# insight-platform/Similari

Hardware: NVIDIA H100
Metric: pair_associations_per_sec (higher is better)
Workload: dtype f32

## Files before the change

similari_b200/csrc/engine.cu:

```cuda
#include <cuda_runtime.h>

#include <algorithm>
#include <chrono>
#include <cmath>
#include <cstdlib>
#include <cstdarg>
#include <cstdio>
#include <cstring>
#include <map>
#include <string>
#include <unordered_map>
#include <vector>

#include "../../include/similari_b200.h"
#include "sb_engine.cuh"

#include <atomic>

namespace sb {
static std::atomic<unsigned long long> g_launches{0};
void note_launch(int n) { g_launches.fetch_add((unsigned long long)n, std::memory_order_relaxed); }
unsigned long long launch_count() { return g_launches.load(std::memory_order_relaxed); }
}

// ... 22 lines not shown
  void* p = nullptr;
  size_t bytes = 0;
  int ensure(size_t need) {
    if (need <= bytes) return 0;
    size_t nb = std::max(need, bytes + bytes / 2);
    void* np = nullptr;
    cudaError_t e = cudaMalloc(&np, nb);
    if (e != cudaSuccess) return fail(SB200_ERR_CUDA, "cudaMalloc(%zu) failed: %s", nb, cudaGetErrorString(e));
    if (p) cudaFree(p);
    p = np;
    bytes = nb;
    return 0;
  }
  void release() {
    if (p) cudaFree(p);
    p = nullptr;
    bytes = 0;
  }
  template <typename T> T* as() const { return reinterpret_cast<T*>(p); }
};

struct HBuf {
  void* p = nullptr;
  void* dp = nullptr;
  size_t bytes = 0;
  int ensure(size_t need) {
    if (need <= bytes) return 0;
    size_t nb = std::max(need, bytes + bytes / 2);
    void* np = nullptr;
    cudaError_t e = cudaHostAlloc(&np, nb, cudaHostAllocMapped);
    if (e != cudaSuccess) return fail(SB200_ERR_CUDA, "cudaHostAlloc(%zu) failed: %s", nb, cudaGetErrorString(e));
    void* ndp = nullptr;
    e = cudaHostGetDevicePointer(&ndp, np, 0);
    if (e != cudaSuccess) { cudaFreeHost(np); return fail(SB200_ERR_CUDA, "cudaHostGetDevicePointer failed: %s", cudaGetErrorString(e)); }
    if (p) cudaFreeHost(p);
    p = np;
    dp = ndp;
    bytes = nb;
    return 0;
  }
  void release() {
    if (p) cudaFreeHost(p);
    p = nullptr;
    dp = nullptr;
    bytes = 0;
  }
  template <typename T> T* as() const { return reinterpret_cast<T*>(p); }
};

int make_params(const sb200_options& o, sb::Params* out) {
  sb::Params p;
  memset(&p, 0, sizeof(p));
  if (o.kind < 0 || o.kind > 3) return fail(SB200_ERR_INVALID, "unknown tracker kind %d", o.kind);
  if (o.positional_kind != SB200_POS_MAHA && o.positional_kind != SB200_POS_IOU)
    return fail(SB200_ERR_INVALID, "unknown positional metric %d", o.positional_kind);
  p.kind = o.kind;
  p.positional_kind = o.positional_kind;
  p.visual_kind = o.visual_kind;
  p.iou_threshold = o.iou_threshold;
  p.min_confidence = o.min_confidence;
  p.pos_weight = o.kalman_position_weight;
  p.vel_weight = o.kalman_velocity_weight;
  p.max_idle_epochs = o.max_idle_epochs;
  if (o.max_idle_epochs < 0) return fail(SB200_ERR_INVALID, "max_idle_epochs must be >= 0");
  if (o.n_constraints < 0 || o.n_constraints > SB200_MAX_CONSTRAINTS)
    return fail(SB200_ERR_INVALID, "at most %d spatio-temporal constraints", SB200_MAX_CONSTRAINTS);
  std::vector<std::pair<int, float>> c;
  for (int i = 0; i < o.n_constraints; ++i) {
    if (!(o.constraint_max_dist[i] > 0.0f))
      return fail(SB200_ERR_INVALID, "The distance is expected to be a positive float");
    c.emplace_back(o.constraint_epochs[i], o.constraint_max_dist[i]);
  }
  std::stable_sort(c.begin(), c.end(), [](const std::pair<int, float>& a, const std::pair<int, float>& b) { return a.first < b.first; });
  c.erase(std::unique(c.begin(), c.end(), [](const std::pair<int, float>& a, const std::pair<int, float>& b) { return a.first == b.first; }), c.end());
  p.n_constraints = (int)c.size();
  for (size_t i = 0; i < c.size(); ++i) { p.constraint_epochs[i] = c[i].first; p.constraint_max_dist[i] = c[i].second; }
  p.is_visual = o.kind == SB200_KIND_VISUAL_SORT || o.kind == SB200_KIND_BATCH_VISUAL_SORT;
  p.is_batch = o.kind == SB200_KIND_BATCH_SORT || o.kind == SB200_KIND_BATCH_VISUAL_SORT;
  if (p.is_visual) {
    if (o.visual_kind != SB200_VIS_EUCLIDEAN && o.visual_kind != SB200_VIS_COSINE)
      return fail(SB200_ERR_INVALID, "unknown visual metric %d", o.visual_kind);
    if (o.feature_dim <= 0) return fail(SB200_ERR_INVALID, "feature_dim must be > 0 for visual trackers");
    if (o.visual_max_observations < 1 || o.visual_max_observations > sb::kMaxObs)
      return fail(SB200_ERR_CAPACITY, "visual_max_observations must be in [1, %d]", sb::kMaxObs);
    p.visual_threshold = o.visual_threshold;
    p.feature_dim = o.feature_dim;
    p.d8 = (o.feature_dim + 7) / 8 * 8;
    p.max_obs = o.visual_max_observations;
    p.min_votes = o.visual_min_votes;
    p.min_track_length = o.visual_minimal_track_length;
    p.min_area = o.visual_minimal_area;
    p.min_quality_use = o.visual_minimal_quality_use;
    p.min_quality_collect = o.visual_minimal_quality_collect;
    p.min_own_use = o.visual_minimal_own_area_percentage_use;
    p.min_own_collect = o.visual_minimal_own_area_percentage_collect;
    p.use_own_area = (o.visual_minimal_own_area_percentage_collect + o.visual_minimal_own_area_percentage_use) > 0.0f;
  } else {
    p.max_obs = 1;
    p.d8 = 8;
  }
  *out = p;
  return 0;
}

}

struct sb200_tracker {
  sb200_options opts{};
  sb::Params P{};
  int device = 0;
  cudaStream_t stream = nullptr;
  bool own_stream = true;
  cudaStream_t user_stream = nullptr;
  bool has_user_stream = false;
  bool join_per_call = true;
  cudaEvent_t ev_join_req = nullptr;
  cudaEvent_t ev_user_in = nullptr, ev_user_out = nullptr;
  cudaStream_t prep_stream = nullptr;
  cudaEvent_t ev_prep_done = nullptr, ev_set_free[2]{}, ev_inputs = nullptr;
  cudaEvent_t ev_cost_done = nullptr;
  bool cost_done_valid = false;
  bool set_busy[2]{};
  bool prep_off = false;
  unsigned long long frame_seq = 0;
  float kernel_ms[2]{};
  bool tc_timed = false;
  cudaStream_t copy_stream = nullptr;
  static constexpr int kDepth = 3;
  struct Pending {
    bool active = false;
    int n_scenes = 0, total = 0;
    std::vector<int> slots, m;
    long long live_ub = 0;
    HBuf h_req;
    HBuf h_out;
    cudaEvent_t done = nullptr;
    cudaEvent_t ev[6]{}, ev_k[3]{}, ev_pos[2]{};
    bool tc_timed = false, pos_forked = false;
    int mode = 0;
  } pend[kDepth];
  int pend_head = 0, pend_count = 0;
  std::vector<int> pending_add;
  long long inflight_live_ub = 0;
  int async_rc = 0;
  std::string async_err;
  unsigned long long acc_units_mn = 0, acc_units_rows = 0, acc_frames = 0;
  double host_ms_total = 0.0, host_ms_blocked = 0.0;
  unsigned long long host_calls = 0;
  double acc_stage_ms[5]{}, acc_kernel_ms[2]{};
  unsigned long long acc_tc_frames = 0;
  cudaStream_t pos_stream = nullptr;
  bool side_off = false;
  cudaEvent_t ev_fork[2]{}, ev_join = nullptr;
  float stage_ms[5]{};
  std::unordered_map<uint64_t, int> slot_of;
  std::vector<uint64_t> scene_of_slot;
  std::vector<uint32_t> epoch;
  std::vector<int> n_tracks;
  std::vector<int> n_hidden;
  std::vector<int> arena_top;
  std::vector<uint64_t> last_req_scenes;
  std::vector<int> last_req_slots;
  int64_t revealed = 0;
  int scene_cap = 0, track_cap = 0;
  DBuf b_idc;
  int auto_waste_counter = 100, auto_waste_periodicity = 100;
  int64_t wasted_count = 0;
  sb::TrackStore ts{};
  DBuf b_id, b_epoch, b_length, b_custom, b_vt, b_pred, b_obs, b_radius, b_kst, b_vert, b_hpred, b_hobs, b_feat, b_feat_bf16, b_fnorm2, b_obs_phys,
      b_obs_hasf, b_obs_q, b_obs_n, b_feat_cnt, b_fblk, b_blk_owner, b_blk_free;
  DBuf b_ntracks, b_cur_epoch, b_scene_ids, b_nfree, b_atop;
  sb::WastedBuf wb{};
  DBuf w_count, w_id, w_scene, w_epoch, w_length, w_pred, w_obs, w_hpred, w_hobs;
  int hist_len = 1;
  struct Staging {
    DBuf boxes, feat, hasf, quality, custom, own;
    const void* key[6] = {nullptr, nullptr, nullptr, nullptr, nullptr, nullptr};
    int total = -1;
    bool pending = false;
    cudaEvent_t ev = nullptr;
    cudaEvent_t ev0 = nullptr;
    cudaEvent_t ev_read = nullptr;
    bool read_pending = false;
  } stg[2];
  int stg_last = 1;
  DBuf f_cbox2[2], f_cradius2[2], f_cconf2[2], f_cvert2[2], f_cflags2[2], f_cnorm22[2], f_cbf162[2], f_decided2[2];
  DBuf f_winner, f_cvt, f_pos, f_vis, f_scenes, f_newcount,
      f_status, f_featdst, f_apprank, f_appmeta, f_posgq, f_frameout, f_excl, f_prewin, f_own, f_ownovf, f_dyn, f_ws, f_tmeta, f_rowinfo, f_slabc, f_slabm, f_slabmask,
      f_dscene, f_maxc, f_maxcval, f_drowb, f_dcolb, f_slabk, f_scene_max, f_tiles, f_pairs, f_colmeta, f_colgeo, f_colb, f_colvalid, f_rowmeta, f_poslist, f_counters, f_visval;
  int num_sms = 132;
  DBuf o_ids, o_epochs, o_lengths, o_vt, o_pred, o_obs;
  HBuf h_small;
  bool adapt_dense = false;
  unsigned long long acc_dense_scenes = 0;
  int last_dense_scenes = 0;
  bool seen_features = false;
  int last_n_scenes = 0;

  ~sb200_tracker() {
    cudaSetDevice(device);
    DBuf* all[] = {&b_id, &b_epoch, &b_length, &b_custom, &b_vt, &b_pred, &b_obs, &b_radius, &b_kst, &b_vert, &b_hpred, &b_hobs, &w_hpred, &w_hobs, &b_feat,
                   &b_feat_bf16, &f_scene_max, &f_tiles, &f_pairs, &f_colmeta, &f_colgeo, &f_colb, &f_colvalid, &f_rowmeta, &f_poslist, &f_counters, &f_visval, &b_fnorm2, &b_obs_phys, &b_obs_hasf, &b_obs_q, &b_obs_n, &b_feat_cnt, &b_ntracks, &b_cur_epoch,
                   &b_fblk, &b_blk_owner, &b_blk_free, &b_nfree, &b_atop, &f_frameout, &f_excl, &f_prewin, &f_own, &f_ownovf, &f_dyn, &b_idc, &f_ws, &f_tmeta, &f_rowinfo, &f_slabc, &f_slabm, &f_slabmask, &f_dscene, &f_maxc, &f_maxcval, &f_drowb, &f_dcolb, &f_slabk,
                   &b_scene_ids, &w_count, &w_id, &w_scene, &w_epoch, &w_length, &w_pred, &w_obs, &f_winner, &f_cvt, &f_pos, &f_vis, &f_scenes, &f_newcount, &f_status,
                   &f_featdst, &f_apprank, &f_appmeta, &f_posgq, &o_ids, &o_epochs, &o_lengths, &o_vt, &o_pred, &o_obs};
    for (DBuf* b : all) b->release();
    for (int k = 0; k < 2; ++k) {
      f_cbox2[k].release(); f_cradius2[k].release(); f_cconf2[k].release(); f_cvert2[k].release(); f_cflags2[k].release();
      f_cnorm22[k].release(); f_cbf162[k].release(); f_decided2[k].release();
    }
    if (stream) cudaStreamSynchronize(stream);
    h_small.release();
    for (auto& g : stg) {
      g.boxes.release(); g.feat.release(); g.hasf.release(); g.quality.release(); g.custom.release(); g.own.release();
      if (g.ev) cudaEventDestroy(g.ev);
      if (g.ev0) cudaEventDestroy(g.ev0);
      if (g.ev_read) cudaEventDestroy(g.ev_read);
    }
    for (auto& q : pend) {
      q.h_req.release(); q.h_out.release();
      if (q.done) cudaEventDestroy(q.done);
      for (auto& e : q.ev) if (e) cudaEventDestroy(e);
      for (auto& e : q.ev_k) if (e) cudaEventDestroy(e);
      for (auto& e : q.ev_pos) if (e) cudaEventDestroy(e);
    }
    if (copy_stream) cudaStreamDestroy(copy_stream);
    if (pos_stream) cudaStreamDestroy(pos_stream);
    if (prep_stream) cudaStreamDestroy(prep_stream);
    for (cudaEvent_t e : {ev_user_in, ev_user_out, ev_prep_done, ev_set_free[0], ev_set_free[1], ev_inputs, ev_join_req, ev_cost_done}) if (e) cudaEventDestroy(e);
    for (auto& e : ev_fork) if (e) cudaEventDestroy(e);
    if (ev_join) cudaEventDestroy(ev_join);
    if (own_stream && stream) cudaStreamDestroy(stream);
  }

  template <typename T>
  int regrow(DBuf& b, T** field, int width, int new_scenes, int new_tracks, bool zero = false) {
    size_t row = (size_t)width * sizeof(T);
    DBuf nb;
    int rc = nb.ensure(std::max<size_t>(1, (size_t)new_scenes * new_tracks * row));
    if (rc) return rc;
    if (zero && cudaMemsetAsync(nb.p, 0, std::max<size_t>(1, (size_t)new_scenes * new_tracks * row), stream) != cudaSuccess)
      return fail(SB200_ERR_CUDA, "store regrow memset failed");
    if (b.p && scene_cap > 0 && track_cap > 0) {
      cudaError_t e = cudaMemcpy2DAsync(nb.p, (size_t)new_tracks * row, b.p, (size_t)track_cap * row,
                                        (size_t)std::min(track_cap, new_tracks) * row, (size_t)scene_cap,
                                        cudaMemcpyDeviceToDevice, stream);
      if (e != cudaSuccess) return fail(SB200_ERR_CUDA, "store regrow copy failed: %s", cudaGetErrorString(e));
      e = cudaStreamSynchronize(stream);
      if (e != cudaSuccess) return fail(SB200_ERR_CUDA, "store regrow sync failed: %s", cudaGetErrorString(e));
    }
    b.release();
    b = nb;
    *field = b.as<T>();
    return 0;
  }

  int ensure_store(int need_scenes, int need_tracks) {
    if (need_scenes <= scene_cap && need_tracks <= track_cap) return 0;
    int ns = scene_cap, nt = track_cap;
    if (need_scenes > ns) ns = std::max(need_scenes, std::max(4, ns * 2));
    if (need_tracks > nt) nt = std::max(need_tracks, std::max(64, nt * 2));
    const int K = P.max_obs;
    int rc = 0;
    if ((rc = regrow(b_id, &ts.id, 1, ns, nt))) return rc;
    if ((rc = regrow(b_epoch, &ts.epoch, 1, ns, nt))) return rc;
    if ((rc = regrow(b_length, &ts.length, 1, ns, nt))) return rc;
    if ((rc = regrow(b_custom, &ts.custom, 1, ns, nt))) return rc;
    if ((rc = regrow(b_vt, &ts.vt, 1, ns, nt))) return rc;
    if ((rc = regrow(b_pred, &ts.pred, 6, ns, nt))) return rc;
    if ((rc = regrow(b_obs, &ts.obs, 6, ns, nt))) return rc;
    if ((rc = regrow(b_radius, &ts.radius, 1, ns, nt))) return rc;
    if ((rc = regrow(b_kst, &ts.kst, sb::kStateStride, ns, nt))) return rc;
    ts.kst_stride = sb::kStateStride;
    if (P.positional_kind == SB200_POS_IOU)
      if ((rc = regrow(b_vert, &ts.vert, 8, ns, nt))) return rc;
    if (hist_len > 1) {
      if ((rc = regrow(b_hpred, &ts.hist_pred, 6 * hist_len, ns, nt, true))) return rc;
      if ((rc = regrow(b_hobs, &ts.hist_obs, 6 * hist_len, ns, nt, true))) return rc;
      ts.hist_len = hist_len;
    }
    if (P.is_visual) {
      if ((rc = regrow(b_feat, &ts.feat, K * P.d8, ns, nt))) return rc;
      {
        unsigned short* tmp = reinterpret_cast<unsigned short*>(ts.feat_bf16);
        if ((rc = regrow(b_feat_bf16, &tmp, K * P.d8, ns, nt))) return rc;
        ts.feat_bf16 = tmp;
      }
      if ((rc = regrow(b_fnorm2, &ts.fnorm2, K, ns, nt))) return rc;
      if ((rc = regrow(b_obs_phys, &ts.obs_phys, K, ns, nt))) return rc;
      if ((rc = regrow(b_obs_hasf, &ts.obs_hasf, K, ns, nt))) return rc;
      if ((rc = regrow(b_obs_q, &ts.obs_q, K, ns, nt))) return rc;
      if ((rc = regrow(b_obs_n, &ts.obs_n, 1, ns, nt))) return rc;
      if ((rc = regrow(b_feat_cnt, &ts.feat_cnt, 1, ns, nt))) return rc;
      if ((rc = regrow(b_fblk, &ts.fblk, 1, ns, nt))) return rc;
      if ((rc = regrow(b_blk_owner, &ts.blk_owner, 1, ns, nt))) return rc;
      if ((rc = regrow(b_blk_free, &ts.blk_free, 1, ns, nt))) return rc;
    }
    if (ns != scene_cap) {
      DBuf n1, n2, n3, n4, n5;
      if ((rc = n1.ensure(sizeof(int) * ns))) return rc;
      if ((rc = n2.ensure(sizeof(unsigned int) * ns))) return rc;
      if ((rc = n3.ensure(sizeof(unsigned long long) * ns))) return rc;
      if ((rc = n4.ensure(sizeof(int) * ns))) return rc;
      if ((rc = n5.ensure(sizeof(int) * ns))) return rc;
      CU(cudaMemsetAsync(n1.p, 0, sizeof(int) * ns, stream));
      CU(cudaMemsetAsync(n4.p, 0, sizeof(int) * ns, stream));
      CU(cudaMemsetAsync(n5.p, 0, sizeof(int) * ns, stream));
      if (b_ntracks.p && scene_cap > 0) {
        CU(cudaMemcpyAsync(n1.p, b_ntracks.p, sizeof(int) * scene_cap, cudaMemcpyDeviceToDevice, stream));
        CU(cudaMemcpyAsync(n4.p, b_nfree.p, sizeof(int) * scene_cap, cudaMemcpyDeviceToDevice, stream));
        CU(cudaMemcpyAsync(n5.p, b_atop.p, sizeof(int) * scene_cap, cudaMemcpyDeviceToDevice, stream));
      }
      CU(cudaStreamSynchronize(stream));
      b_ntracks.release(); b_cur_epoch.release(); b_scene_ids.release(); b_nfree.release(); b_atop.release();
      b_ntracks = n1; b_cur_epoch = n2; b_scene_ids = n3; b_nfree = n4; b_atop = n5;
      ts.n_free = b_nfree.as<int>();
      ts.arena_top = b_atop.as<int>();
    }
    scene_cap = ns;
    track_cap = nt;
    ts.track_cap = nt;
    return 0;
  }

  int slot_for(uint64_t scene_id, bool create) {
    auto it = slot_of.find(scene_id);
    if (it != slot_of.end()) return it->second;
    if (!create) return -1;
    int s = (int)scene_of_slot.size();
    slot_of[scene_id] = s;
    scene_of_slot.push_back(scene_id);
    epoch.push_back(0);
    n_tracks.push_back(0);
    n_hidden.push_back(0);
    arena_top.push_back(0);
    pending_add.push_back(0);
    return s;
  }

  int ensure_wasted(int64_t need) {
    if (need <= wb.cap) return 0;
    int64_t ncap = std::max<int64_t>(need, std::max<int64_t>(1024, (int64_t)wb.cap * 3));
    DBuf nid, nsc, nep, nle, npr, nob, nhp, nho;
    int rc;
    if ((rc = nid.ensure(8 * ncap)) || (rc = nsc.ensure(8 * ncap)) || (rc = nep.ensure(4 * ncap)) ||
        (rc = nle.ensure(4 * ncap)) || (rc = npr.ensure(24 * ncap)) || (rc = nob.ensure(24 * ncap)))
      return rc;
    const size_t hrow = (size_t)24 * hist_len;
    if (hist_len > 1 && ((rc = nhp.ensure(hrow * ncap)) || (rc = nho.ensure(hrow * ncap)))) return rc;
    if (wasted_count > 0) {
      CU(cudaMemcpyAsync(nid.p, w_id.p, 8 * wasted_count, cudaMemcpyDeviceToDevice, stream));
      CU(cudaMemcpyAsync(nsc.p, w_scene.p, 8 * wasted_count, cudaMemcpyDeviceToDevice, stream));
      CU(cudaMemcpyAsync(nep.p, w_epoch.p, 4 * wasted_count, cudaMemcpyDeviceToDevice, stream));
      CU(cudaMemcpyAsync(nle.p, w_length.p, 4 * wasted_count, cudaMemcpyDeviceToDevice, stream));
      CU(cudaMemcpyAsync(npr.p, w_pred.p, 24 * wasted_count, cudaMemcpyDeviceToDevice, stream));
      CU(cudaMemcpyAsync(nob.p, w_obs.p, 24 * wasted_count, cudaMemcpyDeviceToDevice, stream));
      if (hist_len > 1) {
        CU(cudaMemcpyAsync(nhp.p, w_hpred.p, hrow * wasted_count, cudaMemcpyDeviceToDevice, stream));
        CU(cudaMemcpyAsync(nho.p, w_hobs.p, hrow * wasted_count, cudaMemcpyDeviceToDevice, stream));
      }
      CU(cudaStreamSynchronize(stream));
    }
    w_id.release(); w_scene.release(); w_epoch.release(); w_length.release(); w_pred.release(); w_obs.release();
    w_hpred.release(); w_hobs.release();
    w_id = nid; w_scene = nsc; w_epoch = nep; w_length = nle; w_pred = npr; w_obs = nob; w_hpred = nhp; w_hobs = nho;
    wb.hist_pred = w_hpred.as<float>();
    wb.hist_obs = w_hobs.as<float>();
    if (!w_count.p) {
      if ((rc = w_count.ensure(sizeof(int)))) return rc;
      CU(cudaMemsetAsync(w_count.p, 0, sizeof(int), stream));
    }
    wb.cap = (int)ncap;
    wb.count = w_count.as<int>();
    wb.id = w_id.as<unsigned long long>();
    wb.scene = w_scene.as<unsigned long long>();
    wb.epoch = w_epoch.as<unsigned int>();
    wb.length = w_length.as<unsigned int>();
    wb.pred = w_pred.as<float>();
    wb.obs = w_obs.as<float>();
    return 0;
// ... 187 lines not shown
  auto since = [&](std::chrono::steady_clock::time_point a) { return std::chrono::duration<double, std::milli>(tnow() - a).count(); };
  if (n_scenes < 0) return fail(SB200_ERR_INVALID, "n_scenes must be >= 0");
  if (n_scenes > 0 && (!scene_ids || !det_offsets)) return fail(SB200_ERR_INVALID, "scene_ids / det_offsets are NULL");
  const int total = n_scenes > 0 ? det_offsets[n_scenes] : 0;
  if (n_scenes > 0 && det_offsets[0] != 0) return fail(SB200_ERR_INVALID, "det_offsets[0] must be 0");
  for (int s = 0; s < n_scenes; ++s)
    if (det_offsets[s + 1] < det_offsets[s]) return fail(SB200_ERR_INVALID, "det_offsets must be non-decreasing");
  if (total > 0 && !boxes) return fail(SB200_ERR_INVALID, "boxes is NULL");
  if (!P.is_visual) { features = nullptr; has_feature = nullptr; quality = nullptr; own_area = nullptr; }
  int rc = 0;
  poll();
  if (async_rc) { if ((rc = drain("error of an earlier frame"))) return rc; }
  const bool same_req = (int)last_req_scenes.size() == n_scenes && n_scenes > 0 &&
                        memcmp(last_req_scenes.data(), scene_ids, sizeof(uint64_t) * (size_t)n_scenes) == 0;
  if (!same_req && n_scenes > 0) {
    std::unordered_map<uint64_t, int> seen;
    for (int s = 0; s < n_scenes; ++s)
      if (!seen.emplace(scene_ids[s], s).second) return fail(SB200_ERR_INVALID, "scene %llu appears twice in one request", (unsigned long long)scene_ids[s]);
  }
  {
    int max_m0 = 0, max_n0 = 0;
    for (int s = 0; s < n_scenes; ++s) {
      const int m = det_offsets[s + 1] - det_offsets[s];
      int slot = -1;
      if (same_req) slot = last_req_slots[s];
      else { auto it = slot_of.find(scene_ids[s]); if (it != slot_of.end()) slot = it->second; }
      const int nub = slot >= 0 ? n_tracks[slot] + pending_add[slot] : 0;
      max_m0 = std::max(max_m0, m);
      max_n0 = std::max(max_n0, nub);
    }
    const int cap0 = P.is_visual ? kDenseVoteCap : 0;
    if (sb::voting_smem_need(max_m0, max_n0, cap0) > sb::kVotingSmemLimit) {
      if (pend_count > 0) {
        if ((rc = drain("assignment solver bound"))) return rc;
        max_n0 = 0;
        for (int s = 0; s < n_scenes; ++s) {
          auto it = slot_of.find(scene_ids[s]);
          if (it != slot_of.end()) max_n0 = std::max(max_n0, n_tracks[it->second]);
        }
      }
      if (sb::voting_smem_need(max_m0, max_n0, cap0) > sb::kVotingSmemLimit)
        return fail(SB200_ERR_CAPACITY, "scene too large for the on-chip assignment solver (m=%d, n=%d)", max_m0, max_n0);
    }
  }
  if (auto_waste_counter == 0) {
    if ((rc = drain("auto-waste tick"))) return rc;
    if ((rc = run_waste())) return rc;
    auto_waste_counter = auto_waste_periodicity;
  } else auto_waste_counter -= 1;
  if (n_scenes == 0) return wait ? drain() : 0;

  if (!same_req) {
    last_req_slots.resize(n_scenes);
    for (int s = 0; s < n_scenes; ++s) last_req_slots[s] = slot_for(scene_ids[s], true);
    last_req_scenes.assign(scene_ids, scene_ids + n_scenes);
  }
  if (pend_count == kDepth) {
    if (trace) fprintf(stderr, "[sb200] predict waits: ring of %d frames full\n", kDepth);
    absorb_oldest(true);
  }

  const int K = P.max_obs;
  std::vector<int> n_ub(n_scenes), nb_ub(n_scenes), m_of(n_scenes);
  int max_m = 0, max_n = 0, max_nb = 0, need_tracks = 0;
  long long live_ub = 0, pos_total = 0, vis_total = 0, col_total = 0, posl_total = 0, visl_total = 0, work = 0;
  auto bounds = [&]() {
    max_m = max_n = max_nb = need_tracks = 0;
    live_ub = pos_total = vis_total = col_total = work = 0;
    for (int s = 0; s < n_scenes; ++s) {
      const int slot = last_req_slots[s];
      const int m = det_offsets[s + 1] - det_offsets[s];
      m_of[s] = m;
      n_ub[s] = n_tracks[slot] + pending_add[slot];
      nb_ub[s] = P.is_visual ? arena_top[slot] + pending_add[slot] : 0;
      live_ub += n_ub[s];
      pos_total += (long long)m * n_ub[s];
      if (P.is_visual) vis_total += (long long)m * n_ub[s] * K;
      col_total += ((long long)nb_ub[s] * K + 127) / 128 * 128;
      work += (long long)m * n_ub[s] * K;
      max_m = std::max(max_m, m);
      max_n = std::max(max_n, n_ub[s]);
      max_nb = std::max(max_nb, nb_ub[s]);
      need_tracks = std::max(need_tracks, n_ub[s] + m);
    }
  };
  bounds();
  {
    const int pipe_room = kDepth * std::max(max_m, opts.max_dets_per_scene_hint);
    int hint_s = std::max((int)scene_of_slot.size(), opts.max_scenes_hint);
    if (hint_s > scene_cap || need_tracks > track_cap) {
      if ((rc = drain("track store bound"))) return rc;
      bounds();
      const int want_t = std::max(need_tracks, opts.max_tracks_per_scene_hint) + pipe_room;
      if (hint_s > scene_cap || need_tracks > track_cap)
        if ((rc = ensure_store(hint_s, std::max(want_t, track_cap + track_cap / 2)))) return rc;
    }
    if (wasted_count + inflight_live_ub + live_ub + 1 > wb.cap) {
      const long long pipe_need = inflight_live_ub + live_ub;
      if ((rc = drain("wasted buffer bound"))) return rc;
      bounds();
      const long long dets = std::max<long long>(total, (long long)std::max(opts.max_scenes_hint, n_scenes) * opts.max_dets_per_scene_hint);
      const long long ring_need = (long long)(kDepth + 1) * (live_ub + (long long)kDepth * dets);
      const long long rec_bytes = 72 + (hist_len > 1 ? 48ll * hist_len : 0);
      const long long base_need = std::max<long long>(ring_need, 2 * pipe_need);
      const long long mult = std::max<long long>(1, std::min<long long>(8, (2ll << 30) / std::max<long long>(1, base_need * rec_bytes)));
      if ((rc = ensure_wasted(2 * wasted_count + mult * base_need + 1))) return rc;
    }
    if (!b_idc.p) {
      if ((rc = b_idc.ensure(8))) return rc;
      CU(cudaMemsetAsync(b_idc.p, 0, 8, stream));
    }
  }
  Pending& q = pend[(pend_head + pend_count) % kDepth];
  if (!q.done) {
    CU(cudaEventCreateWithFlags(&q.done, cudaEventDisableTiming));
    for (auto& e : q.ev) CU(cudaEventCreate(&e));
    for (auto& e : q.ev_k) CU(cudaEventCreate(&e));
    for (auto& e : q.ev_pos) CU(cudaEventCreate(&e));
  }
  if ((rc = q.h_req.ensure(sizeof(sb::SceneReq) * (size_t)n_scenes)) ||
      (rc = q.h_out.ensure(dyn_offset(n_scenes) + sizeof(sb::FrameDyn) + 16)))
    return rc;
  bool want_tc = false, want_dense = false;
  if (P.is_visual && features != nullptr && total > 0) {
    const bool selective = P.visual_kind == SB200_VIS_EUCLIDEAN ? (P.visual_threshold < 1e18f) : (P.visual_threshold > -1.0f);
    const bool big = P.d8 >= 64 && work * P.d8 >= (1ll << 28);
    const bool dense_ok = P.n_constraints == 0;
    want_tc = selective && big;
    want_dense = big && dense_ok && (!selective || adapt_dense);
    if (want_dense) want_tc = false;
    if (const char* e = getenv("SB200_VIS_KERNEL")) {
      if (!strcmp(e, "simt")) { want_tc = false; want_dense = false; }
      else if (!strcmp(e, "tc")) { want_tc = work > 0; want_dense = false; }
      else if (!strcmp(e, "dense")) { want_dense = work > 0 && dense_ok; want_tc = work > 0 && !want_dense; }
    }
  }
  const int vote_cap = want_dense ? kDenseVoteCap : sb::kVoteVisCap;
  sb::Params Pf = P;
  Pf.vote_vis_cap = vote_cap;
  sb::SceneReq* hreq = q.h_req.as<sb::SceneReq>();
  for (int s = 0; s < n_scenes; ++s) {
    sb::SceneReq& r = hreq[s];
    r.slot = last_req_slots[s];
    r.m = m_of[s];
    r.det_base = det_offsets[s];
    r.epoch = epoch[r.slot] + 1;
    r.scene_id = scene_ids[s];
    r.pos_lbase = (int)posl_total;
    r.pos_lcap = (int)std::min<long long>((long long)r.m * 32, (long long)sb::kVotePosCap * 2);
    posl_total += r.pos_lcap;
    r.vis_lbase = (int)visl_total;
    r.vis_lcap = P.is_visual ? (int)std::min<long long>((long long)r.m * 64, (long long)vote_cap * 4) : 0;
    visl_total += r.vis_lcap;
  }
  const long long hint_dets = (long long)std::max(opts.max_scenes_hint, n_scenes) * opts.max_dets_per_scene_hint;
  const size_t T = (size_t)std::max<long long>(std::max(total, 1), hint_dets);
  const int hint_tracks = opts.max_tracks_per_scene_hint > 0 ? track_cap : 0;
  const long long hint_cols = (long long)std::max(opts.max_scenes_hint, n_scenes) * (((long long)hint_tracks * K + 127) / 128 * 128);
  const long long pos_ub = pos_total;
  {
    const long long hint_pos = hint_dets * hint_tracks;
    pos_total = std::max(pos_total, hint_pos);
    if (P.is_visual) vis_total = std::max(vis_total, hint_pos * K);
  }
  const int cset = (int)(frame_seq & 1);
  DBuf &f_cbox = f_cbox2[cset], &f_cradius = f_cradius2[cset], &f_cconf = f_cconf2[cset], &f_cvert = f_cvert2[cset],
       &f_cflags = f_cflags2[cset], &f_cnorm2 = f_cnorm22[cset], &f_cbf16 = f_cbf162[cset], &f_decided = f_decided2[cset];
  if ((rc = ENS(f_cbox, T * 24)) || (rc = ENS(f_cradius, T * 4)) || (rc = ENS(f_cconf, T * 4)) ||
      (rc = ENS(f_winner, T * 4)) || (rc = ENS(f_cvt, T)) || (rc = ENS(f_scenes, sizeof(sb::SceneDesc) * n_scenes)) ||
      (rc = ENS(f_newcount, 4 * (size_t)n_scenes)) || (rc = ENS(f_dyn, sizeof(sb::FrameDyn))) ||
      (rc = ENS(f_apprank, T * 8)) || (rc = ENS(f_appmeta, 16 * (size_t)n_scenes)) ||
      (rc = ENS(f_pos, std::max<size_t>(4, (size_t)pos_total * 4))))
    return rc;
  if (P.positional_kind == SB200_POS_IOU && (rc = ENS(f_cvert, T * 64))) return rc;
  if (P.is_visual) {
    if ((rc = ENS(f_cflags, T)) || (rc = ENS(f_cnorm2, T * 4)) || (rc = ENS(f_featdst, T * 4)) ||
        (rc = ENS(f_vis, std::max<size_t>(4, (size_t)vis_total * 4))) || (rc = ENS(f_scene_max, 4 * (size_t)n_scenes)))
      return rc;
  }
  sb::TcArgs tc;
  memset(&tc, 0, sizeof(tc));
  tc.num_sms = num_sms;
  int mstep = 0, cstep = 256;
  const long long visl_alloc = std::max(visl_total, hint_dets * 64);
  if (want_tc || want_dense) {
    tc.use_tc = true;
    tc.dense = want_dense;
    mstep = 256;
    cstep = want_dense ? (256 / K) * K : sb::vis_screen_ucols(P.d8, num_sms, n_scenes, m_of.data(), nb_ub.data(), K);
    tc.cstep = cstep;
    long long tiles_ub = 0, slabs_ub = 0, ws_ub = 0, blk_ub = 0;
    for (int s = 0; s < n_scenes; ++s) {
      const long long ct = ((long long)nb_ub[s] * K + cstep - 1) / cstep;
      tiles_ub += (long long)((m_of[s] + mstep - 1) / mstep) * ct;
      slabs_ub += ct;
      ws_ub += ct * (cstep / K) * ((m_of[s] + 127) / 128 * 128);
      blk_ub += ct * (cstep / K);
    }
    tc.n_tiles = (int)tiles_ub;
    long long tiles_alloc = tiles_ub;
    {
      const long long hs = std::max(opts.max_scenes_hint, n_scenes), hd = std::max(opts.max_dets_per_scene_hint, max_m);
      const long long ht = std::max(hint_tracks, max_nb);
      tiles_alloc = std::max(tiles_alloc, hs * ((hd + mstep - 1) / mstep) * ((ht * K + cstep - 1) / cstep + 1));
      if (f_tiles.bytes > 0 && sizeof(sb::TcTile) * (size_t)tiles_alloc > f_tiles.bytes) tiles_alloc += tiles_alloc / 2;
    }
    if ((rc = ENS(f_cbf16, T * P.d8 * 2)) || (rc = ENS(f_tiles, sizeof(sb::TcTile) * (size_t)std::max<long long>(1, tiles_alloc))) ||
        (rc = ENS(f_rowmeta, sizeof(sb::VisRowMeta) * (T + 256))))
      return rc;
    tc.rowmeta = f_rowmeta.as<sb::VisRowMeta>();
    tc.max_rows = max_nb * K;
    tc.d_tiles = f_tiles.as<sb::TcTile>();
    tc.d_n_tiles = &f_dyn.as<sb::FrameDyn>()->n_tiles;
    tc.a_rows = total;
    tc.b_rows = (long long)scene_cap * track_cap * K;
    if (!want_dense) {
      if ((rc = ENS(f_colmeta, sizeof(sb::VisColMeta) * (size_t)(std::max(col_total, hint_cols) + 256))) ||
          (rc = ENS(f_colb, 4 * (size_t)(std::max(col_total, hint_cols) + 256))) ||
          (rc = ENS(f_colvalid, (size_t)(std::max(col_total, hint_cols) + 256) / 8 + 16)) ||
          (rc = ENS(f_colgeo, sizeof(sb::VisColGeo) * (size_t)std::max<long long>(1, P.n_constraints > 0 ? std::max(col_total, hint_cols) : 1))))
        return rc;
      tc.colmeta = f_colmeta.as<sb::VisColMeta>();
      tc.colgeo = f_colgeo.as<sb::VisColGeo>();
      tc.colb = f_colb.as<float>();
      tc.colvalid = f_colvalid.as<unsigned int>();
      tc.total_cols = (int)col_total;
    } else {
      const long long hs = std::max(opts.max_scenes_hint, n_scenes), ht = hint_tracks;
      const long long hd = std::max(opts.max_dets_per_scene_hint, 0);
      ws_ub = std::max(ws_ub, hs * (ht + 256) * ((hd + 127) / 128 * 128));
      blk_ub = std::max(blk_ub, hs * (ht + 256));
      slabs_ub = std::max(slabs_ub, hs * ((ht * K + cstep - 1) / cstep + 1));
      if ((rc = ENS(f_drowb, 4 * 5 * T)) || (rc = ENS(f_dcolb, 4 * (size_t)std::max<long long>(1, blk_ub))) ||
          (rc = ENS(f_slabk, 4 * 256 * (size_t)std::max<long long>(1, slabs_ub))))
        return rc;
      if ((rc = ENS(f_ws, 4 * (size_t)std::max<long long>(1, ws_ub))) || (rc = ENS(f_tmeta, sizeof(sb::DenseTrackMeta) * (size_t)std::max<long long>(1, blk_ub))) ||
          (rc = ENS(f_rowinfo, 8 * (size_t)std::max<long long>(1, blk_ub * K))) || (rc = ENS(f_slabc, 4 * 256 * (size_t)std::max<long long>(1, slabs_ub))) ||
          (rc = ENS(f_slabm, 4 * 256 * (size_t)std::max<long long>(1, slabs_ub))) || (rc = ENS(f_slabmask, 2 * 32 * (size_t)std::max<long long>(1, slabs_ub))) ||
          (rc = ENS(f_dscene, 4 * 6 * (size_t)n_scenes + 128)) || (rc = ENS(f_maxc, sizeof(sb::VisPair) * (size_t)std::max<long long>(1, visl_alloc))) ||
          (rc = ENS(f_maxcval, 4 * (size_t)std::max<long long>(1, visl_alloc))))
        return rc;
      tc.max_blocks = max_nb;
      tc.n_slabs_ub = (int)slabs_ub;
      tc.ws = f_ws.p;
      tc.d_rowb = f_drowb.as<unsigned int>();
      tc.d_colb = f_dcolb.as<unsigned int>();
      tc.blk_ub = blk_ub;
      tc.slab_ktf = f_slabk.as<float>();
      tc.tmeta = f_tmeta.as<sb::DenseTrackMeta>();
      tc.rowinfo = f_rowinfo.as<int2>();
      tc.slab_colc = f_slabc.as<float>();
      tc.slab_cmax = f_slabm.as<float>();
      tc.slab_vmask = f_slabmask.as<unsigned int>();
      tc.slab_bmask = tc.slab_vmask + (size_t)slabs_ub * 8;
      tc.maxc_cnt = f_dscene.as<int>();
      tc.maxc_next = tc.maxc_cnt + n_scenes;
      tc.dense_bad = tc.maxc_cnt + 2 * n_scenes;
      tc.zeros = tc.maxc_cnt + 3 * n_scenes;
      tc.scene_l0 = reinterpret_cast<float*>(tc.maxc_cnt + 4 * n_scenes);
      tc.scene_cmax = tc.scene_l0 + n_scenes;
      tc.dbg_counts = reinterpret_cast<int*>(tc.scene_cmax + n_scenes) + 4;
      tc.maxc = f_maxc.as<sb::VisPair>();
      tc.maxc_val = f_maxcval.as<float>();
    }
  }
  sb::Frame f;
  memset(&f, 0, sizeof(f));
  f.total = total;
  f.pos_total = pos_ub;
  f.dyn = f_dyn.as<sb::FrameDyn>();
  f.id_counter = b_idc.as<unsigned long long>();
  f.id_add = P.is_batch ? (long long)total : -1;
  f.dense_bad = tc.dense ? tc.dense_bad : nullptr;
  f.pos_dense_all = getenv("SB200_FULL_COSTS") != nullptr || getenv("SB200_NO_FORK") != nullptr;
  bool prefetched = false;
  Staging* sin = nullptr;
  if (device_io) {
    f.in_boxes = boxes; f.in_feat = features; f.in_hasf = has_feature; f.in_quality = quality;
    f.in_custom = reinterpret_cast<const long long*>(custom_ids); f.in_own = own_area;
  } else {
    const void* key[6] = {boxes, features, features ? has_feature : nullptr, quality, custom_ids, own_area};
    int use = -1;
    for (int k = 0; k < 2; ++k)
      if (stg[k].pending && stg[k].total == total && memcmp(stg[k].key, key, sizeof(key)) == 0) use = k;
    if (use >= 0) {
      prefetched = true;
      stg[use].pending = false;
      CU(cudaStreamWaitEvent(stream, stg[use].ev, 0));
    } else {
      use = stg[0].pending ? 1 : (stg[1].pending ? 0 : 1 - stg_last);
      stg[use].pending = false;
    }
    stg_last = use;
    Staging& S = stg[use];
    sin = &S;
    if (prefetched && (S.boxes.bytes < T * 24 || (features && S.feat.bytes < T * (size_t)P.feature_dim * 4))) {
      prefetched = false;
    }
    if ((rc = ENS(S.boxes, T * 24))) return rc;
    f.in_boxes = S.boxes.as<float>();
    if (features && total > 0) {
      if ((rc = ENS(S.feat, T * (size_t)P.feature_dim * 4))) return rc;
      f.in_feat = S.feat.as<float>();
      if (has_feature) {
        if ((rc = ENS(S.hasf, T))) return rc;
        f.in_hasf = S.hasf.as<unsigned char>();
      }
    }
    if (quality && total > 0) { if ((rc = ENS(S.quality, T * 4))) return rc; f.in_quality = S.quality.as<float>(); }
    if (custom_ids && total > 0) { if ((rc = ENS(S.custom, T * 8))) return rc; f.in_custom = S.custom.as<long long>(); }
    if (own_area && total > 0) { if ((rc = ENS(S.own, T * 4))) return rc; f.in_own = S.own.as<float>(); }
  }
  f.c_box = f_cbox.as<float>(); f.c_radius = f_cradius.as<float>(); f.c_conf = f_cconf.as<float>();
  f.c_vert = f_cvert.as<double>(); f.c_flags = f_cflags.as<unsigned char>(); f.c_norm2 = f_cnorm2.as<float>();
  f.winner = f_winner.as<int>(); f.c_vt = f_cvt.as<unsigned char>(); f.pos = f_pos.as<float>(); f.vis = f_vis.as<float>();
  f.scenes = f_scenes.as<sb::SceneDesc>(); f.new_count = f_newcount.as<int>();
  f.new_count_all = f.new_count;
  f.feat_dst = P.is_visual ? f_featdst.as<int>() : nullptr;
  f.app_rank = f_apprank.as<int2>(); f.app_meta = f_appmeta.as<int4>();
  if ((rc = ENS(f_frameout, sizeof(int) * 3 * (size_t)n_scenes))) return rc;
  f.frame_out = f_frameout.as<int>();
  f.c_bf16 = tc.use_tc ? f_cbf16.p : nullptr; f.scene_max = f_scene_max.as<unsigned int>();
  const size_t n_counters = 6 * (size_t)n_scenes + 4;
  if ((rc = ENS(f_poslist, sizeof(sb::PosEntry) * (size_t)std::max<long long>(1, std::max(posl_total, hint_dets * 32)))) ||
      (rc = ENS(f_counters, sizeof(int) * n_counters)))
    return rc;
  if (P.is_visual && ((rc = ENS(f_pairs, sizeof(sb::VisPair) * (size_t)std::max<long long>(1, visl_alloc))) ||
                      (rc = ENS(f_visval, sizeof(float) * (size_t)std::max<long long>(1, visl_alloc)))))
    return rc;
  f.pos_list = f_poslist.as<sb::PosEntry>();
  f.pos_cnt = f_counters.as<int>();
  f.vis_cnt = f.pos_cnt + n_scenes;
  f.scene_mode = f.pos_cnt + 2 * n_scenes;
  f.vis_mode = f.pos_cnt + 3 * n_scenes;
  f.refine_next = f.pos_cnt + 4 * n_scenes;
  f.status = f.pos_cnt + 5 * n_scenes;
  f.dense_cnt = f.pos_cnt + 6 * n_scenes;
  if (getenv("SB200_POS_GQ") != nullptr) {
    size_t gq_cap = (size_t)std::min<long long>(std::max<long long>(1, std::max<long long>(total, hint_dets) * 24), 1ll << 26);
    if (const char* e = getenv("SB200_POS_GQ_CAP")) gq_cap = (size_t)std::max(1, atoi(e));
    if ((rc = ENS(f_posgq, 8 * gq_cap))) return rc;
    f.pos_gq = f_posgq.as<int2>();
    f.pos_gq_cnt = f.pos_cnt + 6 * n_scenes + 1;
    f.pos_gq_cap = (int)gq_cap;
  }
  f.vis_pairs = f_pairs.as<sb::VisPair>();
  f.vis_val = f_visval.as<float>();
  sb200_predict_out o{};
  if (out) o = *out;
  if (device_io) {
    f.o_ids = reinterpret_cast<unsigned long long*>(o.ids); f.o_epochs = o.epochs; f.o_lengths = o.lengths;
    f.o_vt = o.voting_types; f.o_pred = o.predicted_boxes; f.o_obs = o.observed_boxes;
  } else {
    if (o.ids) { if ((rc = ENS(o_ids, T * 8))) return rc; f.o_ids = o_ids.as<unsigned long long>(); }
    if (o.epochs) { if ((rc = ENS(o_epochs, T * 4))) return rc; f.o_epochs = o_epochs.as<unsigned int>(); }
    if (o.lengths) { if ((rc = ENS(o_lengths, T * 4))) return rc; f.o_lengths = o_lengths.as<unsigned int>(); }
    if (o.voting_types) { if ((rc = ENS(o_vt, T))) return rc; f.o_vt = o_vt.as<unsigned char>(); }
    if (o.predicted_boxes) { if ((rc = ENS(o_pred, T * 24))) return rc; f.o_pred = o_pred.as<float>(); }
    if (o.observed_boxes) { if ((rc = ENS(o_obs, T * 24))) return rc; f.o_obs = o_obs.as<float>(); }
  }
  const bool full_costs = getenv("SB200_FULL_COSTS") != nullptr || getenv("SB200_NO_FORK") != nullptr;
  const bool fork = P.is_visual && tc.use_tc && tc.n_tiles > 0 && !full_costs;
  if (fork) {
    if ((rc = ENS(f_decided, T)) || (rc = ENS(f_excl, (size_t)scene_cap * track_cap + 16)) || (rc = ENS(f_prewin, T * 4))) return rc;
    f.decided = f_decided.as<unsigned char>();
    f.excl = f_excl.as<unsigned char>();
    f.pre_winner = f_prewin.as<int>();
  }
  const bool derive_own = P.is_visual && P.use_own_area && f.in_own == nullptr && total > 0;
  if (derive_own && ((rc = ENS(f_own, T * 4)) || (rc = ENS(f_ownovf, 16 + T * sizeof(int2))))) return rc;

  for (int s = 0; s < n_scenes; ++s) epoch[last_req_slots[s]] += 1;
  if (features != nullptr && total > 0) seen_features = true;
  frame_seq += 1;
  q.active = true;
  q.n_scenes = n_scenes;
  q.total = total;
  q.slots.assign(last_req_slots.begin(), last_req_slots.end());
  q.m = m_of;
  q.live_ub = live_ub;
  q.tc_timed = false;
  q.pos_forked = false;
  q.mode = tc.dense ? 2 : (tc.use_tc ? 1 : 0);
  for (int s = 0; s < n_scenes; ++s) pending_add[last_req_slots[s]] += m_of[s];
  inflight_live_ub += live_ub;
  pend_count += 1;
  last_n_scenes = n_scenes;
  struct Rollback {
    sb200_tracker* t; Pending* q; bool armed;
    ~Rollback() {
      if (!armed) return;
      for (int s = 0; s < q->n_scenes; ++s) t->pending_add[q->slots[s]] -= q->m[s];
      t->inflight_live_ub -= q->live_ub;
      q->active = false;
      t->pend_count -= 1;
    }
  } rollback{this, &q, true};

  const double ms_setup = since(t_begin);
  if (has_user_stream) {
    if (!ev_user_in) { CU(cudaEventCreateWithFlags(&ev_user_in, cudaEventDisableTiming)); CU(cudaEventCreateWithFlags(&ev_user_out, cudaEventDisableTiming)); }
    CU(cudaEventRecord(ev_user_in, user_stream));
    CU(cudaStreamWaitEvent(stream, ev_user_in, 0));
  }
  if (!device_io && !prefetched && total > 0) {
    const size_t n = (size_t)total;
    CU(cudaMemcpyAsync(sin->boxes.p, boxes, n * 24, cudaMemcpyHostToDevice, stream));
    if (f.in_feat) {
      CU(cudaMemcpyAsync(sin->feat.p, features, n * (size_t)P.feature_dim * 4, cudaMemcpyHostToDevice, stream));
      if (f.in_hasf) CU(cudaMemcpyAsync(sin->hasf.p, has_feature, n, cudaMemcpyHostToDevice, stream));
    }
    if (f.in_quality) CU(cudaMemcpyAsync(sin->quality.p, quality, n * 4, cudaMemcpyHostToDevice, stream));
    if (f.in_custom) CU(cudaMemcpyAsync(sin->custom.p, custom_ids, n * 8, cudaMemcpyHostToDevice, stream));
    if (f.in_own) CU(cudaMemcpyAsync(sin->own.p, own_area, n * 4, cudaMemcpyHostToDevice, stream));
  }
  if (!pos_stream && !side_off) {
    static const bool off = [] { const char* e = getenv("SB200_SIDE_STREAM"); return e && e[0] == '0'; }();
    side_off = off;
    if (!side_off) {
      int lo = 0, hi = 0;
      CU(cudaDeviceGetStreamPriorityRange(&lo, &hi));
      CU(cudaStreamCreateWithPriority(&pos_stream, cudaStreamNonBlocking, hi));
      for (auto& e : ev_fork) CU(cudaEventCreateWithFlags(&e, cudaEventDisableTiming));
      CU(cudaEventCreateWithFlags(&ev_join, cudaEventDisableTiming));
    }
  }
  const bool side_ok = pos_stream != nullptr;
  if (!prep_stream && !prep_off) {
    static const bool off = [] { const char* e = getenv("SB200_PREP_AHEAD"); return e && e[0] == '0'; }();
    prep_off = off;
    if (!prep_off) {
      int lo = 0, hi = 0;
      CU(cudaDeviceGetStreamPriorityRange(&lo, &hi));
      CU(cudaStreamCreateWithPriority(&prep_stream, cudaStreamNonBlocking, lo));
      CU(cudaEventCreateWithFlags(&ev_prep_done, cudaEventDisableTiming));
      CU(cudaEventCreateWithFlags(&ev_inputs, cudaEventDisableTiming));
    }
  }
  const bool prep_ahead = prep_stream != nullptr && !derive_own && total > 0;
  const bool side_setup = side_ok && !derive_own && total > 0;
  cudaStream_t s_setup = stream;
  if (side_setup) {
    CU(cudaEventRecord(ev_fork[0], stream));
    CU(cudaStreamWaitEvent(pos_stream, ev_fork[0], 0));
    s_setup = pos_stream;
  }
  sb::launch_frame_setup(P, ts, f, reinterpret_cast<const sb::SceneReq*>(q.h_req.dp), n_scenes, b_ntracks.as<int>(), mstep,
                         cstep, tc.dense, f_tiles.as<sb::TcTile>(), f_dyn.as<sb::FrameDyn>(), f_counters.as<int>(), (int)n_counters, s_setup);
  tc.max_init_done = 1;
  if (side_setup && Pf.is_visual && tc.use_tc && !tc.dense && tc.n_tiles > 0 && max_m > 0 && max_n > 0 && f.in_feat) {
    sb::launch_vis_colmeta(Pf, ts, f, n_scenes, max_n, tc, pos_stream);
    tc.colmeta_done = 1;
  }
  if (side_setup) CU(cudaEventRecord(ev_join, pos_stream));
  CU(cudaEventRecord(q.ev[0], stream));
  if (derive_own) {
    sb::launch_own_area(f, n_scenes, max_m, f.in_boxes, f_own.as<float>(), f_ownovf.as<int>(),
                        reinterpret_cast<int2*>(f_ownovf.as<char>() + 16), stream);
    f.in_own = f_own.as<float>();
  }
  if (prep_ahead) {
    if (has_user_stream) CU(cudaStreamWaitEvent(prep_stream, ev_user_in, 0));
    if (!device_io) {
      if (prefetched) CU(cudaStreamWaitEvent(prep_stream, sin->ev, 0));
      else { CU(cudaEventRecord(ev_inputs, stream)); CU(cudaStreamWaitEvent(prep_stream, ev_inputs, 0)); }
    }
    if (set_busy[cset]) CU(cudaStreamWaitEvent(prep_stream, ev_set_free[cset], 0));
    static const bool after_cost = [] { const char* e = getenv("SB200_PREP_AFTER"); return !(e && !strcmp(e, "none")); }();
    if (after_cost && cost_done_valid) CU(cudaStreamWaitEvent(prep_stream, ev_cost_done, 0));
    sb::launch_prep(Pf, f, n_scenes, max_m, prep_stream);
    CU(cudaEventRecord(ev_prep_done, prep_stream));
    CU(cudaStreamWaitEvent(stream, ev_prep_done, 0));
  } else {
    sb::launch_prep(Pf, f, n_scenes, max_m, stream);
  }
  if (side_setup) CU(cudaStreamWaitEvent(stream, ev_join, 0));
  CU(cudaEventRecord(q.ev[1], stream));
  sb::TcArgs tcc = tc;
  if (tc.use_tc && tc.n_tiles > 0) { tcc.ev_screen0 = q.ev_k[0]; tcc.ev_screen1 = q.ev_k[1]; tcc.ev_refine1 = q.ev_k[2]; q.tc_timed = true; }
  if (!fork) {
    sb::launch_pos_cost(Pf, ts, f, n_scenes, max_m, max_n, stream);
    CU(cudaEventRecord(q.ev[2], stream));
    int vr0 = sb::launch_vis_cost(Pf, ts, f, n_scenes, max_m, max_n, tcc, stream);
    if (vr0 != 0) return fail(SB200_ERR_CUDA, "visual cost launch failed (%d)", vr0);
    if (!f.pos_dense_all) sb::launch_pos_scan_lazy(Pf, ts, f, n_scenes, max_m, max_n, 1, stream);
  } else {
    CU(cudaEventRecord(q.ev[2], stream));
    {
      int vr0 = sb::launch_vis_cost_a(Pf, ts, f, n_scenes, max_m, max_n, tcc, stream);
      if (vr0 != 0) return fail(SB200_ERR_CUDA, "visual cost launch failed (%d)", vr0);
      vr0 = sb::launch_vote_masks(Pf, ts, f, n_scenes, max_m, max_n, stream);
      if (vr0 != 0) return fail(SB200_ERR_CUDA, "voting launch failed: %s", cudaGetErrorString((cudaError_t)vr0));
    }
    CU(cudaEventRecord(q.ev_pos[0], stream));
    sb::launch_pos_scan_lazy(Pf, ts, f, n_scenes, max_m, max_n, 0, stream);
    CU(cudaEventRecord(q.ev_pos[1], stream));
    int vr1 = sb::launch_vis_cost_b(Pf, ts, f, n_scenes, max_m, max_n, tcc, stream);
    if (vr1 != 0) return fail(SB200_ERR_CUDA, "visual cost launch failed (%d)", vr1);
    sb::launch_pos_scan_lazy(Pf, ts, f, n_scenes, max_m, max_n, 1, stream);
    q.pos_forked = true;
  }
  CU(cudaEventRecord(q.ev[3], stream));
  if (prep_stream) {
    if (!ev_cost_done) CU(cudaEventCreateWithFlags(&ev_cost_done, cudaEventDisableTiming));
    CU(cudaEventRecord(ev_cost_done, stream));
    cost_done_valid = true;
  }
  int vr = sb::launch_voting(Pf, ts, f, n_scenes, max_m, max_n, stream);
  if (vr != 0) return fail(SB200_ERR_CUDA, "voting launch failed: %s", cudaGetErrorString((cudaError_t)vr));
  CU(cudaEventRecord(q.ev[4], stream));
  sb::launch_apply(Pf, ts, f, n_scenes, max_m, 0ull, b_ntracks.as<int>(), stream);
  const bool side_sweep = side_ok && Pf.is_visual && f.in_feat && total > 0;
  if (side_sweep) {
    CU(cudaEventRecord(ev_fork[1], stream));
    CU(cudaStreamWaitEvent(pos_stream, ev_fork[1], 0));
    sb::launch_frame_sweep(Pf, ts, f, n_scenes, b_ntracks.as<int>(), wb, pos_stream);
    CU(cudaEventRecord(ev_join, pos_stream));
    sb::launch_feat_store(Pf, ts, f, stream);
    CU(cudaStreamWaitEvent(stream, ev_join, 0));
  } else {
    sb::launch_feat_store(Pf, ts, f, stream);
    sb::launch_frame_sweep(Pf, ts, f, n_scenes, b_ntracks.as<int>(), wb, stream);
  }
  CU(cudaEventRecord(q.ev[5], stream));
  CU(cudaGetLastError());

  if (!device_io && total > 0) {
    if (o.ids) CU(cudaMemcpyAsync(o.ids, f.o_ids, (size_t)total * 8, cudaMemcpyDeviceToHost, stream));
    if (o.epochs) CU(cudaMemcpyAsync(o.epochs, f.o_epochs, (size_t)total * 4, cudaMemcpyDeviceToHost, stream));
    if (o.lengths) CU(cudaMemcpyAsync(o.lengths, f.o_lengths, (size_t)total * 4, cudaMemcpyDeviceToHost, stream));
    if (o.voting_types) CU(cudaMemcpyAsync(o.voting_types, f.o_vt, (size_t)total, cudaMemcpyDeviceToHost, stream));
    if (o.predicted_boxes) CU(cudaMemcpyAsync(o.predicted_boxes, f.o_pred, (size_t)total * 24, cudaMemcpyDeviceToHost, stream));
    if (o.observed_boxes) CU(cudaMemcpyAsync(o.observed_boxes, f.o_obs, (size_t)total * 24, cudaMemcpyDeviceToHost, stream));
  }
  {
    char* ho = reinterpret_cast<char*>(q.h_out.p);
    CU(cudaMemcpyAsync(ho, f.frame_out, 12 * (size_t)n_scenes, cudaMemcpyDeviceToHost, stream));
    CU(cudaMemcpyAsync(ho + 12 * (size_t)n_scenes, f.status, 4 * (size_t)n_scenes, cudaMemcpyDeviceToHost, stream));
    CU(cudaMemcpyAsync(ho + dyn_offset(n_scenes), f_dyn.p, sizeof(sb::FrameDyn), cudaMemcpyDeviceToHost, stream));
    CU(cudaMemcpyAsync(ho + dyn_offset(n_scenes) + sizeof(sb::FrameDyn), f.dense_cnt, 4, cudaMemcpyDeviceToHost, stream));
  }
  static const bool trace_dense = trace && atoi(getenv("SB200_TRACE")) >= 2;
  if (trace_dense && tc.dense && tc.n_tiles > 0) {
    int hc[8] = {0};
    int vc = 0;
    CU(cudaMemcpyAsync(hc, tc.dbg_counts, sizeof(hc), cudaMemcpyDeviceToHost, stream));
    CU(cudaStreamSynchronize(stream));
    std::vector<int> vcnt((size_t)n_scenes);
    CU(cudaMemcpy(vcnt.data(), f.vis_cnt, 4 * (size_t)n_scenes, cudaMemcpyDeviceToHost));
    long long tot = 0; int mx = 0;
    for (int v : vcnt) { tot += v; mx = std::max(mx, v); }
    (void)vc;
    fprintf(stderr, "[sb200] dense frame: fallback reasons threshold %d, max-list overflow %d, no maximum %d; max candidates %d; pairs to refine %lld (largest scene %d)\n",
            hc[0], hc[1], hc[2], hc[3], tot, mx);
  }
  CU(cudaEventRecord(q.done, stream));
  if (!ev_set_free[cset]) CU(cudaEventCreateWithFlags(&ev_set_free[cset], cudaEventDisableTiming));
  CU(cudaEventRecord(ev_set_free[cset], stream));
  set_busy[cset] = true;
  if (has_user_stream && join_per_call) {
    CU(cudaEventRecord(ev_user_out, stream));
    CU(cudaStreamWaitEvent(user_stream, ev_user_out, 0));
  }
  rollback.armed = false;
  if (sin) { CU(cudaEventRecord(sin->ev_read, stream)); sin->read_pending = true; }
  const double ms_launch = since(t_begin);
  if (wait) rc = drain();
  host_ms_total += since(t_begin);
  host_calls += 1;
  if (trace && prefetched && sin && wait) {
    float cms = 0.0f;
    if (cudaEventElapsedTime(&cms, sin->ev0, sin->ev) == cudaSuccess)
      fprintf(stderr, "[sb200] prefetch copy of this frame took %.3f ms on the copy stream\n", cms);
  }
  if (trace) fprintf(stderr, "[sb200] predict: setup %.3f ms, launched at %.3f ms, returned at %.3f ms (total dets %d, %d in flight)\n", ms_setup, ms_launch, since(t_begin), total, pend_count);
  return rc;
}

#undef ENS
extern "C" {

const char* sb200_last_error(void) { return g_err.c_str(); }
void sb200__set_error(const char* msg) { g_err = msg ? msg : ""; }

int sb200_device_count(void) {
  int n = 0;
  if (cudaGetDeviceCount(&n) != cudaSuccess) { cudaGetLastError(); return 0; }
  return n;
}

void sb200_options_default(sb200_options* o) {
  if (!o) return;
  memset(o, 0, sizeof(*o));
  o->kind = SB200_KIND_SORT;
  o->positional_kind = SB200_POS_MAHA;
  o->iou_threshold = 0.3f;
  o->min_confidence = 0.05f;
  o->max_idle_epochs = 5;
  o->history_length = 1;
  o->kalman_position_weight = 1.0f / 20.0f;
  o->kalman_velocity_weight = 1.0f / 160.0f;
  o->visual_kind = SB200_VIS_EUCLIDEAN;
  o->visual_threshold = 3.402823466e+38f;
  o->visual_max_observations = 5;
  o->visual_min_votes = 1;
  o->visual_minimal_track_length = 3;
}

int sb200_tracker_create(const sb200_options* opts, sb200_tracker** out) {
  if (!opts || !out) return fail(SB200_ERR_INVALID, "opts / out is NULL");
  *out = nullptr;
  int ndev = sb200_device_count();
  if (ndev <= 0) return fail(SB200_ERR_CUDA, "no CUDA device available (this library has no CPU execution path)");
  if (opts->device < 0 || opts->device >= ndev) return fail(SB200_ERR_INVALID, "device %d out of range (%d devices)", opts->device, ndev);
  sb::Params P;
  int rc = make_params(*opts, &P);
  if (rc) return rc;
  CU(cudaSetDevice(opts->device));
  sb200_tracker* t = new sb200_tracker();
  t->opts = *opts;
  t->P = P;
// ... 449 lines not shown
```

similari_b200/csrc/kernels_assign.cu:

```cuda
#include <algorithm>

#include "sb_engine.cuh"

namespace sb {

constexpr int VT_THREADS = 512;
constexpr int NWARPS = VT_THREADS / 32;
constexpr int kNone = -1, kSelf = -2;

struct MinPair { long long v; int y; };

__device__ __forceinline__ MinPair min_pair(MinPair a, MinPair b) {
  return (b.v < a.v || (b.v == a.v && b.y < a.y)) ? b : a;
}
__device__ __forceinline__ MinPair warp_min(MinPair a) {
#pragma unroll
  for (int o = 16; o > 0; o >>= 1) {
    MinPair b;
    b.v = __shfl_xor_sync(0xffffffffu, a.v, o);
    b.y = __shfl_xor_sync(0xffffffffu, a.y, o);
    a = min_pair(a, b);
  }
  return a;
}
// ... 742 lines not shown
    }
    for (int y = tid; y < ny; y += VT_THREADS) { s.ly[y] = 0; s.yx[y] = -1; }
    __syncthreads();

    int parity = 0;
    int root = 0;
    while (root < nrows) {
      {
        int* cand = s.alt;
        int* cfirst = s.slackx;
        for (int y = tid; y < ny; y += VT_THREADS) cfirst[y] = 0x7fffffff;
        if (tid == 0) s_misc[2] = nrows;
        __syncthreads();
        for (int r = root + tid; r < nrows; r += VT_THREADS) {
          int besty = -1;
          if (thr > 0) {
            const long long lxr = s.lx[r];
            MinPair best; best.v = lxr + s.ly[r] - thr; best.y = r;
            if (r < n_seen_rows) {
              const int m = s.row_cand[r];
              for (int q = s.row_ptr[m]; q < s.row_ptr[m + 1]; ++q) {
                const int y = nrows + s.col_rank[s.csr_n[q]];
                MinPair c; c.v = lxr + s.ly[y] - weight_i64(s.csr_v[q]); c.y = y;
                best = min_pair(best, c);
              }
            }
            if (best.v == 0 && lxr > 0) besty = best.y;
          }
          cand[r] = besty;
          if (besty >= 0) atomicMin(&cfirst[besty], r);
        }
        __syncthreads();
        for (int r = root + tid; r < nrows; r += VT_THREADS) {
          const int y = cand[r];
          if (y < 0 || cfirst[y] != r || s.yx[y] >= 0) atomicMin(&s_misc[2], r);
        }
        __syncthreads();
        const int first_fail = s_misc[2];
        for (int r = root + tid; r < first_fail; r += VT_THREADS) {
          const int y = cand[r];
          s.xy[r] = y; s.yx[y] = r;
        }
      }
      __syncthreads();
      root = s_misc[2];
      if (root >= nrows) break;
      const long long lxr = s.lx[root];
      MinPair best; best.v = 9223372036854775807LL; best.y = 0x7fffffff;
      for (int y = tid; y < ny; y += VT_THREADS) {
        long long sl = lxr + s.ly[y] - wgt(root, y);
        s.slack[y] = sl; s.slackx[y] = root; s.alt[y] = -1;
        MinPair c; c.v = sl; c.y = y;
        best = min_pair(best, c);
      }
      for (int x = tid; x < nrows; x += VT_THREADS) s.inS[x] = x == root;
      best = warp_min(best);
      if (lane == 0) s_red[parity][wid] = best;
      __syncthreads();
      int y_end = -1, x_end = -1;
      for (;;) {
        MinPair g = s_red[parity][0];
#pragma unroll
        for (int w = 1; w < NWARPS; ++w) g = min_pair(g, s_red[parity][w]);
        parity ^= 1;
        const long long delta = g.v;
        const int ystar = g.y;
        const int xstar = s.slackx[ystar];
        const int x2 = s.yx[ystar];
        for (int x = tid; x < nrows; x += VT_THREADS) {
          if (s.inS[x]) { if (delta > 0) s.lx[x] -= delta; }
          else if (x == x2) s.inS[x] = 1;
        }
        if (x2 < 0) {
          if (delta > 0)
            for (int y = tid; y < ny; y += VT_THREADS) {
              if (s.alt[y] >= 0) s.ly[y] += delta;
              else s.slack[y] -= delta;
            }
          y_end = ystar; x_end = xstar;
          break;
        }
        const long long lx2 = s.lx[x2];
        MinPair nb; nb.v = 9223372036854775807LL; nb.y = 0x7fffffff;
        for (int y = tid; y < ny; y += VT_THREADS) {
          if (s.alt[y] >= 0) { if (delta > 0) s.ly[y] += delta; continue; }
          long long sl = s.slack[y] - delta;
          if (y == ystar) { s.alt[y] = xstar; s.slack[y] = sl; continue; }
          long long a = lx2 + s.ly[y] - wgt(x2, y);
          if (sl > a) { sl = a; s.slackx[y] = x2; }
          s.slack[y] = sl;
          MinPair c; c.v = sl; c.y = y;
          nb = min_pair(nb, c);
        }
        nb = warp_min(nb);
        if (lane == 0) s_red[parity][wid] = nb;
        __syncthreads();
      }
      __syncthreads();
      if (tid == 0) {
        int y = y_end, x = x_end;
        for (;;) {
          int prec = s.xy[x];
          s.yx[y] = x;
          s.xy[x] = y;
          y = prec;
          if (y < 0) break;
          x = s.alt[y];
        }
      }
      __syncthreads();
      ++root;
    }
    for (int r = tid; r < n_seen_rows; r += VT_THREADS) {
      int y = s.xy[r];
      int m = s.row_cand[r];
      if (y >= nrows && (y - nrows) < n_seen_cols) {
        winner[m] = s.col_trk[y - nrows];
        cvt[m] = (unsigned char)1;
      }
    }
  }
  __syncthreads();
  int c = 0;
  for (int m = tid; m < M; m += VT_THREADS) c += winner[m] < 0;
#pragma unroll
  for (int o = 16; o > 0; o >>= 1) c += __shfl_xor_sync(0xffffffffu, c, o);
  if (lane == 0) s_warp[wid] = c;
  __syncthreads();
  if (tid == 0) {
    int t = 0;
    for (int w = 0; w < NWARPS; ++w) t += s_warp[w];
    f.new_count[sidx] = t;
  }
}

__device__ __forceinline__ int vis_side_mode(const Params& p, const Frame& f, const SceneDesc& sc, int s, int tc_used) {
  if (sc.m >= 65535 || sc.n >= 65535) return 1;
  if (p.is_visual) {
    if (!tc_used) return 1;
    if (f.vis_cnt[s] > sc.vis_lcap || f.vis_cnt[s] > vote_cap(p)) return 1;
    if (f.dense_bad && f.dense_bad[s]) return 1;
  }
  return 0;
}
__global__ void scene_mode_kernel(Params p, Frame f, int n_scenes, int tc_used) {
  int s = blockIdx.x * blockDim.x + threadIdx.x;
  if (s >= n_scenes) return;
  const SceneDesc sc = f.scenes[s];
  int mode = vis_side_mode(p, f, sc, s, tc_used);
  if (f.pos_cnt[s] > sc.pos_lcap || f.pos_cnt[s] > kVotePosCap) mode = 1;
  f.scene_mode[s] = mode;
  if (mode != 0 && f.dense_cnt) atomicAdd(f.dense_cnt, 1);
}
__global__ void vis_mode_kernel(Params p, Frame f, int n_scenes, int tc_used) {
  int s = blockIdx.x * blockDim.x + threadIdx.x;
  if (s >= n_scenes) return;
  f.vis_mode[s] = vis_side_mode(p, f, f.scenes[s], s, tc_used);
}

void launch_scene_mode(const Params& p, const Frame& f, int n_scenes, bool tc_used, cudaStream_t st) {
  if (n_scenes == 0) return;
  scene_mode_kernel<<<(n_scenes + 127) / 128, 128, 0, st>>>(p, f, n_scenes, tc_used ? 1 : 0);
  note_launch();
}

void launch_vis_mode(const Params& p, const Frame& f, int n_scenes, bool tc_used, cudaStream_t st) {
  if (n_scenes == 0 || !f.vis_mode) return;
  vis_mode_kernel<<<(n_scenes + 127) / 128, 128, 0, st>>>(p, f, n_scenes, tc_used ? 1 : 0);
  note_launch();
}

void launch_scene_max(const Params& p, const Frame& f, int n_scenes, bool init_only, cudaStream_t st) {
  if (n_scenes == 0 || !f.scene_max) return;
  if (init_only) {
    vis_max_init_kernel<<<(n_scenes + 255) / 256, 256, 0, st>>>(f.scene_max, n_scenes);
  } else {
    dim3 grid(32, n_scenes);
    vis_max_kernel<<<grid, 256, 0, st>>>(p, f, f.scene_max);
  }
  note_launch();
}

size_t voting_smem_need(int max_m, int max_n, int viscap) {
  return std::max(vote_smem_bytes(max_m, max_n), sparse_smem_bytes(max_m, max_n, viscap > 0 ? viscap : kVoteVisCap));
}

int launch_voting(const Params& p, const TrackStore& ts, const Frame& f, int n_scenes, int max_m, int max_n,
                  cudaStream_t st) {
  if (n_scenes == 0) return 0;
  const size_t smem_d = vote_smem_bytes(max_m, max_n);
  const size_t smem_s = sparse_smem_bytes(max_m, max_n, vote_cap(p));
  if (smem_d > kVotingSmemLimit || smem_s > kVotingSmemLimit) return -3;
  cudaError_t e;
  if (p.is_visual) {
    if ((e = cudaFuncSetAttribute(voting_sparse_kernel<true, false>, cudaFuncAttributeMaxDynamicSharedMemorySize, (int)smem_s)) != cudaSuccess) return (int)e;
    if ((e = cudaFuncSetAttribute(voting_kernel<true>, cudaFuncAttributeMaxDynamicSharedMemorySize, (int)smem_d)) != cudaSuccess) return (int)e;
    voting_sparse_kernel<true, false><<<n_scenes, VT_THREADS, smem_s, st>>>(p, ts, f);
    voting_kernel<true><<<n_scenes, VT_THREADS, smem_d, st>>>(p, f);
    note_launch(2);
  } else {
    if ((e = cudaFuncSetAttribute(voting_sparse_kernel<false, false>, cudaFuncAttributeMaxDynamicSharedMemorySize, (int)smem_s)) != cudaSuccess) return (int)e;
    if ((e = cudaFuncSetAttribute(voting_kernel<false>, cudaFuncAttributeMaxDynamicSharedMemorySize, (int)smem_d)) != cudaSuccess) return (int)e;
    voting_sparse_kernel<false, false><<<n_scenes, VT_THREADS, smem_s, st>>>(p, ts, f);
    voting_kernel<false><<<n_scenes, VT_THREADS, smem_d, st>>>(p, f);
    note_launch(2);
  }
  return 0;
}

int launch_vote_masks(const Params& p, const TrackStore& ts, const Frame& f, int n_scenes, int max_m, int max_n,
                      cudaStream_t st) {
  if (n_scenes == 0 || !p.is_visual || !f.decided || !f.excl) return 0;
  const size_t smem_s = sparse_smem_bytes(max_m, max_n, vote_cap(p));
  if (smem_s > kVotingSmemLimit) return -3;
  cudaError_t e = cudaFuncSetAttribute(voting_sparse_kernel<true, true>, cudaFuncAttributeMaxDynamicSharedMemorySize, (int)smem_s);
  if (e != cudaSuccess) return (int)e;
  voting_sparse_kernel<true, true><<<n_scenes, VT_THREADS, smem_s, st>>>(p, ts, f);
  note_launch();
  return 0;
}

}
```

similari_b200/csrc/kernels_cost.cu:

```cuda
#include <cuda_bf16.h>

#include <algorithm>
#include <cstdlib>

#include "sb_engine.cuh"

namespace sb {

__global__ void prep_kernel(Params p, Frame f) {
  int i = blockIdx.x * blockDim.x + threadIdx.x;
  if (i >= f.total) return;
  i += f.det0;
  if (f.decided) f.decided[i] = 0;
  const float* b = f.in_boxes + (size_t)i * 6;
  float xc = b[0], yc = b[1], ang = b[2], asp = b[3], h = b[4], conf = b[5];
  if (ang == 0.0f) ang = nanf("");
  float* cb = f.c_box + (size_t)i * 6;
  cb[0] = xc; cb[1] = yc; cb[2] = ang; cb[3] = asp; cb[4] = h; cb[5] = conf;
  f.c_radius[i] = box_radius(asp, h);
  f.c_conf[i] = conf < p.min_confidence ? p.min_confidence : conf;
  if (p.positional_kind == 1) box_vertices(xc, yc, ang, asp, h, f.c_vert + (size_t)i * 8);
  if (p.is_visual) {
    bool hasf = f.in_feat != nullptr && (f.in_hasf == nullptr || f.in_hasf[i] != 0);
    float q = f.in_quality ? f.in_quality[i] : 1.0f;
// ... 484 lines not shown
__device__ void vis_cost_tile(const Params& p, const TrackStore& ts, const Frame& f, int scene, int bx, int by);

__global__ void __launch_bounds__(VT) vis_cost_kernel(Params p, TrackStore ts, Frame f, int n_scenes, int tiles_x, int tiles_y) {
  if (f.dense_cnt && *f.dense_cnt == 0) return;
  const long long per_scene = (long long)tiles_x * tiles_y;
  for (int scene = 0; scene < n_scenes; ++scene) {
    if (f.scene_mode[scene] == 0) continue;
    for (long long t = blockIdx.x; t < per_scene; t += gridDim.x) {
      vis_cost_tile(p, ts, f, scene, (int)(t % tiles_x), (int)(t / tiles_x));
      __syncthreads();
    }
  }
}

__device__ void vis_cost_tile(const Params& p, const TrackStore& ts, const Frame& f, int scene, int bx, int by) {
  const SceneDesc sc = f.scenes[scene];
  const int K = p.max_obs;
  const int ncols = sc.n * K;
  const int c0 = bx * VN, m0 = by * VM;
  if (c0 >= ncols || m0 >= sc.m) return;
  __shared__ float sa[VM][VK + 1];
  __shared__ float sb_[VN][VK + 1];
  __shared__ int col_row[VN];
  __shared__ float col_norm[VN];
  __shared__ unsigned char col_ok[VN];
  __shared__ unsigned char row_ok[VM];
  __shared__ float row_norm[VM];
  const int tid = threadIdx.x;
  const bool cosine = p.visual_kind == 1;
  if (tid < VN) {
    int c = c0 + tid;
    int row = -1; float nrm = 0.0f; unsigned char ok = 0;
    if (c < ncols) {
      int n = c / K, k = c % K;
      size_t ti = (size_t)sc.slot * ts.track_cap + n;
      if (k < ts.obs_n[ti] && ts.obs_hasf[ti * K + k] && ts.feat_cnt[ti] >= p.min_track_length) {
        int phys = ts.obs_phys[ti * K + k];
        row = (int)(feat_block(ts, sc.slot, ti) * K + phys);
        nrm = cosine ? ts.fnorm2[row] : 0.0f;
        ok = 1;
      }
    }
    col_row[tid] = row; col_norm[tid] = nrm; col_ok[tid] = ok;
  }
  if (tid >= 64 && tid < 64 + VM) {
    int i = tid - 64;
    int m = m0 + i;
    unsigned char ok = 0; float nrm = 0.0f;
    if (m < sc.m) {
      int g = sc.det_base + m;
      ok = (f.c_flags[g] & 2) ? 1 : 0;
      nrm = cosine ? f.c_norm2[g] : 0.0f;
    }
    row_ok[i] = ok; row_norm[i] = nrm;
  }
  __syncthreads();
  const int tx = tid % 16, ty = tid / 16;
  float acc[4][4];
#pragma unroll
  for (int a = 0; a < 4; ++a)
#pragma unroll
    for (int b = 0; b < 4; ++b) acc[a][b] = 0.0f;
  const int D = p.feature_dim, D8 = p.d8;
  for (int k0 = 0; k0 < D8; k0 += VK) {
    for (int e = tid; e < VM * VK; e += VT) {
      int r = e / VK, c = e % VK;
      int m = m0 + r, d = k0 + c;
      float v = 0.0f;
      if (m < sc.m && d < D && row_ok[r]) v = f.in_feat[(size_t)(sc.det_base + m) * D + d];
      sa[r][c] = v;
    }
    for (int e = tid; e < VN * VK; e += VT) {
      int r = e / VK, c = e % VK;
      int d = k0 + c;
      float v = 0.0f;
      int row = col_row[r];
      if (row >= 0 && d < D8) v = ts.feat[(size_t)row * D8 + d];
      sb_[r][c] = v;
    }
    __syncthreads();
#pragma unroll
    for (int blk = 0; blk < VK / 8; ++blk) {
      float av[4][8], bv[4][8];
#pragma unroll
      for (int a = 0; a < 4; ++a)
#pragma unroll
        for (int l = 0; l < 8; ++l) av[a][l] = sa[ty * 4 + a][blk * 8 + l];
#pragma unroll
      for (int b = 0; b < 4; ++b)
#pragma unroll
        for (int l = 0; l < 8; ++l) bv[b][l] = sb_[tx * 4 + b][blk * 8 + l];
#pragma unroll
      for (int a = 0; a < 4; ++a)
#pragma unroll
        for (int b = 0; b < 4; ++b) {
          float t[8];
          if (cosine) {
#pragma unroll
            for (int l = 0; l < 8; ++l) t[l] = av[a][l] * bv[b][l];
          } else {
#pragma unroll
            for (int l = 0; l < 8; ++l) { float df = av[a][l] - bv[b][l]; t[l] = df * df; }
          }
          acc[a][b] = acc[a][b] + reduce_add8(t);
        }
    }
    __syncthreads();
  }
  float* out = f.vis + sc.vis_off;
  const float qnan = nanf("");
#pragma unroll
  for (int a = 0; a < 4; ++a) {
    int r = ty * 4 + a, m = m0 + r;
    if (m >= sc.m) continue;
    int g = sc.det_base + m;
    const float cx = f.c_box[(size_t)g * 6], cy = f.c_box[(size_t)g * 6 + 1], cr = f.c_radius[g];
#pragma unroll
    for (int b = 0; b < 4; ++b) {
      int cc = tx * 4 + b, c = c0 + cc;
      if (c >= ncols) continue;
      float v = qnan;
      if (row_ok[r] && col_ok[cc]) {
        int n = c / K;
        size_t ti = (size_t)sc.slot * ts.track_cap + n;
        const float* tb = ts.pred + ti * 6;
        if (compat_ok(p, sc.epoch, ts.epoch[ti], cx, cy, cr, tb[0], tb[1], ts.radius[ti])) {
          if (cosine) {
            float d = acc[a][b] / sqrtf(row_norm[r] * col_norm[cc]);
            if (d >= p.visual_threshold) v = 1.0f - d;
          } else {
            float d = sqrtf(acc[a][b]);
            if (d <= p.visual_threshold) v = d;
          }
        }
      }
      out[(size_t)m * ncols + c] = v;
    }
  }
}

int launch_vis_cost_a(const Params& p, const TrackStore& ts, const Frame& f, int n_scenes, int max_m, int max_n,
                      const TcArgs& tc, cudaStream_t st) {
  if (n_scenes == 0 || !p.is_visual) return 0;
  const bool any = max_m > 0 && max_n > 0 && f.in_feat != nullptr;
  const bool use_tc = tc.use_tc && any;
  if (!tc.max_init_done) launch_scene_max(p, f, n_scenes, true, st);
  if (use_tc && tc.dense) {
    int rc = launch_vis_dense(p, ts, f, n_scenes, max_m, tc, st);
    if (rc != 0) return rc;
  } else if (use_tc) {
    int rc = launch_vis_cost_tc(p, ts, f, n_scenes, max_n, tc, 0, st);
    if (rc != 0) return rc;
  }
  launch_vis_mode(p, f, n_scenes, use_tc, st);
  if (use_tc) {
    int rc = launch_vis_cost_tc(p, ts, f, n_scenes, max_n, tc, 1, st);
    if (rc != 0) return rc;
  }
  return 0;
}

int launch_vis_cost_b(const Params& p, const TrackStore& ts, const Frame& f, int n_scenes, int max_m, int max_n,
                      const TcArgs& tc, cudaStream_t st) {
  if (n_scenes == 0) return 0;
  if (!p.is_visual) {
    launch_scene_mode(p, f, n_scenes, false, st);
    return 0;
  }
  const bool any = max_m > 0 && max_n > 0 && f.in_feat != nullptr;
  const bool use_tc = tc.use_tc && any;
  launch_scene_mode(p, f, n_scenes, use_tc, st);
  if (max_m > 0 && max_n > 0) {
    const int tx = (max_n * p.max_obs + VN - 1) / VN, ty = (max_m + VM - 1) / VM;
    const long long want = (long long)tx * ty * (use_tc ? 1 : n_scenes);
    const int grid = (int)std::min<long long>(want, kNumSms * 8);
    vis_cost_kernel<<<grid, VT, 0, st>>>(p, ts, f, n_scenes, tx, ty);
    note_launch();
    launch_scene_max(p, f, n_scenes, false, st);
  }
  return 0;
}

int launch_vis_cost(const Params& p, const TrackStore& ts, const Frame& f, int n_scenes, int max_m, int max_n,
                    const TcArgs& tc, cudaStream_t st) {
  int rc = launch_vis_cost_a(p, ts, f, n_scenes, max_m, max_n, tc, st);
  if (rc != 0) return rc;
  return launch_vis_cost_b(p, ts, f, n_scenes, max_m, max_n, tc, st);
}

}
```

similari_b200/csrc/kernels_feat_dense.cu:

```cuda
#include <cuda.h>
#include <cuda_bf16.h>
#include <cuda_fp16.h>
#include <cuda_runtime.h>
#include <stdint.h>

#include <algorithm>
#include <cstdlib>
#include <cstring>

#include "sb_engine.cuh"
#include "sb_tc.cuh"

namespace sb {

constexpr float kDenseErrE = kScreenRelErr + 2e-4f;
constexpr float kDenseErrC = kScreenRelErr + 2e-4f;

constexpr int DS_STAGES = 4;
constexpr int DS_STAGE_BYTES = TC_A_BYTES + TC_B_BYTES;
constexpr int DS_CH = 16;
constexpr int DS_PITCH = DS_CH + 1;

struct DsHdr {
  int scene, m0, m, det_base;
// ... 397 lines not shown
    else v = (na + nb2 - 2.0f * dot) - 1e-4f * (na + nb2);
    best = fmaxf(best, v);
  }
  if (lane == 0) s_w[wid] = best;
  __syncthreads();
  if (tid == 0) {
    for (int w = 1; w < 8; ++w) best = fmaxf(best, s_w[w]);
    scene_l0[s] = best;
  }
}

constexpr int SEL_T = 512;
__global__ void __launch_bounds__(SEL_T) vis_dense_select_kernel(Params p, Frame f, const __half2* ws, const DenseTrackMeta* tmeta,
                                                                 const int2* rowinfo, const int* maxc_cnt, const int* max_nan,
                                                                 int* dense_bad, int* dbg_counts, const unsigned int* rowb,
                                                                 const unsigned int* colb, int fused) {
  extern __shared__ unsigned char sel_smem[];
  const int s = blockIdx.x;
  const SceneDesc sc = f.scenes[s];
  const int tid = threadIdx.x, lane = tid & 31;
  const int K = p.max_obs;
  const int nb = sc.nb, M = sc.m;
  if (M == 0 || nb == 0) return;
  const unsigned int um = f.scene_max[s];
  const float maxd = __uint_as_float((um & 0x80000000u) ? (um & 0x7fffffffu) : ~um);
  const int reason = (max_nan[s] != 0 ? 1 : 0) | (maxc_cnt[s] > sc.vis_lcap ? 2 : 0) | (!(maxd >= 0.0f) ? 4 : 0);
  if (tid == 0) {
    if (reason & 1) atomicAdd(&dbg_counts[0], 1);
    if (reason & 2) atomicAdd(&dbg_counts[1], 1);
    if (reason & 4) atomicAdd(&dbg_counts[2], 1);
    atomicAdd(&dbg_counts[3], maxc_cnt[s]);
  }
  if (reason) { if (tid == 0) dense_bad[s] = reason; return; }
  unsigned int* lcol = reinterpret_cast<unsigned int*>(sel_smem);
  short* kt = reinterpret_cast<short*>(lcol + nb);
  const int need_votes = p.min_votes > 1 ? p.min_votes : 1;
  for (int b = tid; b < nb; b += SEL_T) {
    const DenseTrackMeta tm = tmeta[sc.blk_off + b];
    const int kb = (tm.n >= 0 && tm.kt >= need_votes) ? tm.kt : 0;
    kt[b] = (short)kb;
    unsigned int u = 0x00800000u;
    if (fused && kb > 0) {
      const unsigned int cb = colb[sc.blk_off + b];
      if (cb != 0u) u = enc_ord(((float)kb * maxd * (1.0f - 2e-6f) - 1e-7f) + dec_ord(cb));
    }
    lcol[b] = u;
  }
  __syncthreads();
  const int mpad = (M + 127) / 128 * 128;
  const __half2* w0 = ws + sc.ws_off;
  const float fneg = -3.0e38f;
  for (int pass = fused ? 1 : 0; pass < 2; ++pass) {
    for (int m0 = 0; m0 < mpad; m0 += SEL_T) {
      const int m = m0 + tid;
      const bool row_ok = m < M && (f.c_flags[sc.det_base + m] & 2);
      float lrow = fneg;
      if (pass == 1 && row_ok) {
        if (!fused) lrow = f.vis_val[sc.vis_lbase + m];
        else {
          const unsigned int* rb = rowb + (size_t)(sc.det_base + m) * kDenseKClasses;
#pragma unroll
          for (int kc = 0; kc < kDenseKClasses; ++kc) {
            const unsigned int u = rb[kc];
            if (u != 0u) lrow = fmaxf(lrow, ((float)(kc + 1) * maxd * (1.0f - 2e-6f) - 1e-7f) + dec_ord(u));
          }
        }
      }
      const __half2* wrow = w0 + m;
      constexpr int UB = 8;
      for (int b0 = 0; b0 < nb; b0 += UB) {
        int kk[UB];
        float2 ee[UB];
#pragma unroll
        for (int u = 0; u < UB; ++u) {
          kk[u] = b0 + u < nb ? (int)kt[b0 + u] : 0;
          ee[u] = make_float2(0.0f, 0.0f);
          if (row_ok && kk[u] != 0) {
            const unsigned int raw = __ldcs(reinterpret_cast<const unsigned int*>(wrow + (size_t)(b0 + u) * mpad));
            const float2 v = __half22float2(*reinterpret_cast<const __half2*>(&raw));
            ee[u] = make_float2(v.x, v.y + (v.x * kHalfRel) / (float)kk[u]);
          }
        }
#pragma unroll
        for (int u = 0; u < UB; ++u) {
          const int k = kk[u], b = b0 + u;
          if (k == 0) continue;
          const float fk = (float)k, a = fk * maxd;
          const float2 e = ee[u];
          if (pass == 0) {
            float wlo = fneg;
            if (row_ok) wlo = (a * (1.0f - 2e-6f) - 1e-7f) - (e.x * (1.0f + 2e-6f) + fk * e.y);
            lrow = fmaxf(lrow, wlo);
            unsigned int uu = __float_as_uint(wlo);
            uu = (uu & 0x80000000u) ? ~uu : (uu | 0x80000000u);
            uu = __reduce_max_sync(0xffffffffu, uu);
            if (lane == 0 && uu > lcol[b]) atomicMax(&lcol[b], uu);
          } else if (row_ok) {
            float whi = (a * (1.0f + 2e-6f) + 1e-7f) - (e.x * (1.0f - 2e-6f) - fk * e.y);
            if (!(e.x < 6.0e4f)) whi = 3.0e38f;
            const unsigned int uu = lcol[b];
            const float lc = __uint_as_float((uu & 0x80000000u) ? (uu & 0x7fffffffu) : ~uu);
            if (whi >= lrow || whi >= lc) {
              const int g = sc.det_base + m;
              int cnt = 0;
              int2 ri[kMaxObs];
              for (int ph = 0; ph < K; ++ph) {
                ri[ph] = rowinfo[(size_t)sc.blk_off * K + (size_t)b * K + ph];
                cnt += ri[ph].y >= 0;
              }
              int pos = atomicAdd(&f.vis_cnt[s], cnt);
              for (int ph = 0; ph < K; ++ph) {
                if (ri[ph].y < 0) continue;
                if (pos < sc.vis_lcap) {
                  VisPair vp;
                  vp.g = g; vp.row = ri[ph].y; vp.scene = s; vp.outcol = ri[ph].x;
                  f.vis_pairs[sc.vis_lbase + pos] = vp;
                }
                ++pos;
              }
            }
          }
        }
      }
      if (pass == 0 && m < M) f.vis_val[sc.vis_lbase + m] = lrow;
    }
    __syncthreads();
  }
}

typedef CUresult (*EncodeTiledFnD)(CUtensorMap*, CUtensorMapDataType, cuuint32_t, void*, const cuuint64_t*, const cuuint64_t*,
                                   const cuuint32_t*, const cuuint32_t*, CUtensorMapInterleave, CUtensorMapSwizzle,
                                   CUtensorMapL2promotion, CUtensorMapFloatOOBfill);
static EncodeTiledFnD get_encode_d() {
  static EncodeTiledFnD fn = nullptr;
  if (!fn) {
    void* q = nullptr;
    cudaDriverEntryPointQueryResult qr;
    if (cudaGetDriverEntryPoint("cuTensorMapEncodeTiled", &q, cudaEnableDefault, &qr) == cudaSuccess && q) fn = (EncodeTiledFnD)q;
  }
  return fn;
}
static int make_map_d(CUtensorMap* m, const void* base, long long rows, int d8, int box_rows) {
  EncodeTiledFnD enc = get_encode_d();
  if (!enc) return -1;
  cuuint64_t dims[2] = {(cuuint64_t)d8, (cuuint64_t)rows};
  cuuint64_t strides[1] = {(cuuint64_t)d8 * 2};
  cuuint32_t box[2] = {(cuuint32_t)TC_BK, (cuuint32_t)box_rows};
  cuuint32_t estr[2] = {1, 1};
  CUresult r = enc(m, CU_TENSOR_MAP_DATA_TYPE_BFLOAT16, 2, (void*)base, dims, strides, box, estr, CU_TENSOR_MAP_INTERLEAVE_NONE,
                   CU_TENSOR_MAP_SWIZZLE_128B, CU_TENSOR_MAP_L2_PROMOTION_L2_256B, CU_TENSOR_MAP_FLOAT_OOB_FILL_NONE);
  return r == CUDA_SUCCESS ? 0 : -2;
}

int launch_vis_refine(const Params& p, const TrackStore& ts, const Frame& f, int n_scenes, int* nan_flag, cudaStream_t st);

int launch_vis_dense(const Params& p, const TrackStore& ts, const Frame& f, int n_scenes, int max_m, const TcArgs& tc,
                     cudaStream_t st) {
  if (n_scenes == 0) return 0;
  cudaMemsetAsync(tc.maxc_cnt, 0, (size_t)n_scenes * 4 * 4, st);
  cudaMemsetAsync(tc.dbg_counts, 0, 8 * 4, st);
  if (tc.n_tiles == 0 || max_m == 0) return 0;
  CUtensorMap mA, mB;
  if (make_map_d(&mA, f.c_bf16, tc.a_rows, p.d8, TC_BM) || make_map_d(&mB, ts.feat_bf16, tc.b_rows, p.d8, TC_BN / 2)) return -1;
  const bool cosine = p.visual_kind == 1;
  cudaMemsetAsync(tc.slab_vmask, 0, (size_t)tc.n_slabs_ub * (TC_BN / 32) * 4, st);
  cudaMemsetAsync(tc.slab_bmask, 0, (size_t)tc.n_slabs_ub * (TC_BN / 32) * 4, st);
  cudaMemsetAsync(tc.scene_cmax, 0, (size_t)n_scenes * 4, st);
  cudaMemsetAsync(tc.slab_ktf, 0, (size_t)tc.n_slabs_ub * TC_BN * 4, st);
  const bool fused = p.max_obs <= kDenseKClasses && getenv("SB200_DENSE_GENERIC") == nullptr;
  if (fused) {
    cudaMemsetAsync(tc.d_rowb, 0, (size_t)f.total * kDenseKClasses * 4, st);
    cudaMemsetAsync(tc.d_colb, 0, (size_t)tc.blk_ub * 4, st);
  }
  if (tc.max_blocks > 0) {
    dim3 grid((tc.max_blocks + 127) / 128, n_scenes);
    vis_dense_meta_kernel<<<grid, 128, 0, st>>>(p, ts, f, tc.max_blocks, tc.cstep, tc.tmeta, tc.rowinfo, tc.slab_colc, tc.slab_cmax,
                                                tc.slab_ktf, tc.slab_vmask, tc.slab_bmask, tc.scene_cmax);
    note_launch();
  }
  vis_dense_rowmeta_kernel<<<(f.total + 255) / 256, 256, 0, st>>>(p, f, tc.rowmeta);
  vis_dense_sample_kernel<<<n_scenes, 256, 0, st>>>(p, ts, f, tc.rowinfo, tc.scene_l0);
  note_launch(2);
  if (tc.ev_screen0) cudaEventRecord(tc.ev_screen0, st);
  {
    const size_t smem = sizeof(DsSmem) + 1024;
    const void* fn = nullptr;
#define SB_WSUM(KT) (cosine ? (const void*)vis_wsum_kernel<true, KT> : (const void*)vis_wsum_kernel<false, KT>)
    switch (p.max_obs) {
      case 1: fn = SB_WSUM(1); break;
      case 2: fn = SB_WSUM(2); break;
      case 3: fn = SB_WSUM(3); break;
      case 4: fn = SB_WSUM(4); break;
      case 5: fn = SB_WSUM(5); break;
      default: fn = SB_WSUM(0); break;
    }
    if (getenv("SB200_DENSE_GENERIC")) fn = SB_WSUM(0);
#undef SB_WSUM
    cudaError_t e = cudaFuncSetAttribute(fn, cudaFuncAttributeMaxDynamicSharedMemorySize, (int)smem);
    if (e != cudaSuccess) return (int)e;
    const int ncta = 2 * std::min(tc.n_tiles, tc.num_sms / 2);
    cudaLaunchConfig_t cfg;
    memset(&cfg, 0, sizeof(cfg));
    cfg.gridDim = dim3(ncta);
    cfg.blockDim = dim3(TC_THREADS);
    cfg.dynamicSmemBytes = smem;
    cfg.stream = st;
    cudaLaunchAttribute attr[1];
    attr[0].id = cudaLaunchAttributeClusterDimension;
    attr[0].val.clusterDim.x = 2; attr[0].val.clusterDim.y = 1; attr[0].val.clusterDim.z = 1;
    cfg.attrs = attr;
    cfg.numAttrs = 1;
    DenseDev dd;
    dd.ws = reinterpret_cast<__half2*>(tc.ws); dd.rowb = tc.d_rowb; dd.colb = tc.d_colb; dd.slab_ktf = tc.slab_ktf;
    dd.slab_colc = tc.slab_colc; dd.slab_cmax = tc.slab_cmax; dd.slab_vmask = tc.slab_vmask;
    dd.slab_bmask = tc.slab_bmask; dd.scene_l0 = tc.scene_l0; dd.scene_cmax = tc.scene_cmax; dd.maxc = tc.maxc;
    dd.maxc_cnt = tc.maxc_cnt; dd.rowmeta = tc.rowmeta;
    static const int dbg = getenv("SB200_DENSE_DBG") ? atoi(getenv("SB200_DENSE_DBG")) : 0;
    dd.dbg = dbg;
    const TcTile* d_tiles = tc.d_tiles;
    const int* d_n_tiles = tc.d_n_tiles;
    void* args[] = {(void*)&mA, (void*)&mB, (void*)&p, (void*)&ts, (void*)&f, (void*)&d_tiles, (void*)&d_n_tiles, (void*)&dd};
    e = cudaLaunchKernelExC(&cfg, fn, args);
    if (e != cudaSuccess) return (int)e;
    note_launch();
  }
  if (tc.ev_screen1) cudaEventRecord(tc.ev_screen1, st);
  {
    Frame fm = f;
    fm.vis_pairs = tc.maxc; fm.vis_val = tc.maxc_val; fm.vis_cnt = tc.maxc_cnt; fm.refine_next = tc.maxc_next;
    fm.vis_mode = tc.zeros;
    int rc = launch_vis_refine(p, ts, fm, n_scenes, tc.dense_bad, st);
    if (rc != 0) return rc;
  }
  {
    const size_t smem = (size_t)std::max(1, tc.max_blocks) * 6 + 64;
    if (smem > 48 * 1024) cudaFuncSetAttribute(vis_dense_select_kernel, cudaFuncAttributeMaxDynamicSharedMemorySize, (int)smem);
    vis_dense_select_kernel<<<n_scenes, SEL_T, smem, st>>>(p, f, reinterpret_cast<const __half2*>(tc.ws), tc.tmeta, tc.rowinfo,
                                                           tc.maxc_cnt, tc.dense_bad, tc.dense_bad, tc.dbg_counts, tc.d_rowb,
                                                           tc.d_colb, fused ? 1 : 0);
    note_launch();
  }
  return 0;
}

}
```

similari_b200/csrc/kernels_feat_tc.cu:

```cuda
#include <cuda.h>
#include <cuda_bf16.h>
#include <cuda_runtime.h>
#include <stdint.h>

#include <algorithm>
#include <cstdlib>
#include <cstring>

#include "sb_engine.cuh"
#include "sb_tc.cuh"

namespace sb {

constexpr int TC_STAGES = 4;
constexpr int TC_STAGE_BYTES = TC_A_BYTES + TC_B_BYTES;

struct TcHdr { int scene, m0, ncols_left, m, det_base, col0, epoch, vis_lbase, vis_lcap, pad; };
struct TcSmem {
  unsigned char stage[TC_STAGES][TC_STAGE_BYTES];
  VisColMeta meta[4][TC_BN];
  VisRowMeta rowm[4][TC_BM];
  float colb[4][TC_BN];
  unsigned int colvalid[4][TC_BN / 32];
  TcHdr hdr[4];
// ... 56 lines not shown
          h.scene = tl.scene; h.m0 = m0; h.ncols_left = sc.nb * K - tl.c0; h.m = sc.m; h.det_base = sc.det_base;
          h.col0 = sc.col_off + tl.c0; h.epoch = (int)sc.epoch; h.vis_lbase = sc.vis_lbase; h.vis_lcap = sc.vis_lcap; h.pad = 0;
          S.hdr[g] = h;
          mbar_expect_tx(&S.meta_full[g], (uint32_t)(sizeof(VisColMeta) * TC_BN + sizeof(VisRowMeta) * TC_BM +
                                                    4 * TC_BN + TC_BN / 8));
          bulk_load(S.meta[g], colmeta + h.col0, (uint32_t)(sizeof(VisColMeta) * TC_BN), &S.meta_full[g]);
          bulk_load(S.rowm[g], rowmeta + rowA, (uint32_t)(sizeof(VisRowMeta) * TC_BM), &S.meta_full[g]);
          bulk_load(S.colb[g], colb + h.col0, 4 * TC_BN, &S.meta_full[g]);
          bulk_load(S.colvalid[g], colvalid + (h.col0 >> 5), TC_BN / 8, &S.meta_full[g]);
        }
        for (int kb = 0; kb < KB; ++kb) {
          mbar_wait(&S.empty_bar[stage], phase ^ 1);
          unsigned char* base = stage_base + stage * TC_STAGE_BYTES;
          mbar_expect_tx(&S.full_bar[stage], TC_STAGE_BYTES);
          tma_load_2d(base, &mapA, kb * TC_BK, rowA, &S.full_bar[stage]);
          tma_load_2d_mc(base + TC_A_BYTES + crank * (TC_B_BYTES / 2), &mapB, kb * TC_BK, rowB + (int)crank * (TC_BN / 2),
                         &S.full_bar[stage], (uint16_t)0x3);
          if (++stage == TC_STAGES) { stage = 0; phase ^= 1; }
        }
      }
    }
  } else {
    asm volatile("setmaxnreg.inc.sync.aligned.u32 232;");
    const int wg = (warp >> 2) - 1;
    const int rr[2] = {wg * TC_WG_ROWS + (warp & 3) * 16 + (lane >> 2), wg * TC_WG_ROWS + (warp & 3) * 16 + (lane >> 2) + 8};
    const int q2 = 2 * (lane & 3);
    const bool geo = p.n_constraints > 0;
    int stage = 0;
    uint32_t phase = 0;
    int it = 0;
    for (int t = cta_first; t < n_tiles; t += cta_step, ++it) {
      float acc[128];
      tc_consume_tile<2, TC_STAGES, TC_STAGE_BYTES>(acc, stage_base, S.full_bar, S.empty_bar, KB, wg, stage, phase);
      const int ms = it & 3;
      mbar_wait(&S.meta_full[ms], (it >> 2) & 1);
      const VisColMeta* gmeta = S.meta[ms];
      const TcHdr h = S.hdr[ms];
      const float* gcolb = S.colb[ms];
      float rowk[2];
      bool row_ok[2];
      int g[2];
#pragma unroll
      for (int hr = 0; hr < 2; ++hr) {
        const VisRowMeta rm = S.rowm[ms][rr[hr]];
        const int m = h.m0 + rr[hr];
        row_ok[hr] = m < h.m && rm.ok;
        g[hr] = h.det_base + m;
        rowk[hr] = rm.rowk;
      }
      unsigned int keep[4] = {0u, 0u, 0u, 0u};
#pragma unroll
      for (int j = 0; j < TC_BN / 8; ++j) {
        const int c0 = 8 * j + q2;
        const float2 cb = *reinterpret_cast<const float2*>(gcolb + c0);
        const unsigned int vw = S.colvalid[ms][c0 >> 5] >> (c0 & 31);
#pragma unroll
        for (int e = 0; e < 4; ++e) {
          const int hr = e >> 1, cl = e & 1;
          const float b = COSINE ? rowk[hr] * (cl ? cb.y : cb.x) : rowk[hr] + (cl ? cb.y : cb.x);
          const bool k = !(acc[4 * j + e] < b) && ((vw >> cl) & 1u) && c0 + cl < h.ncols_left && row_ok[hr];
          if (k) keep[j >> 3] |= 1u << (((4 * j) & 31) + e);
        }
      }
      if (geo) {
        float cx[2], cy[2], cr[2];
#pragma unroll
        for (int hr = 0; hr < 2; ++hr) {
          cx[hr] = 0.0f; cy[hr] = 0.0f; cr[hr] = 0.0f;
          if (row_ok[hr]) { cx[hr] = f.c_box[(size_t)g[hr] * 6]; cy[hr] = f.c_box[(size_t)g[hr] * 6 + 1]; cr[hr] = f.c_radius[g[hr]]; }
        }
#pragma unroll
        for (int w = 0; w < 4; ++w) {
          unsigned int kk = keep[w];
          while (kk) {
            const int b = __ffs(kk) - 1;
            kk &= kk - 1;
            const int i = w * 32 + b, hr = (i >> 1) & 1;
            const int col = 8 * (i >> 2) + q2 + (i & 1);
            const VisColGeo cg = colgeo[h.col0 + col];
            if (!compat_ok(p, (unsigned int)h.epoch, cg.tep, cx[hr], cy[hr], cr[hr], cg.tx, cg.ty, cg.tr)) keep[w] &= ~(1u << b);
          }
        }
      }
      int cnt = 0;
#pragma unroll
      for (int w = 0; w < 4; ++w) cnt += __popc(keep[w]);
      if (__any_sync(0xffffffffu, cnt != 0)) {
        int incl = cnt;
#pragma unroll
        for (int o = 1; o < 32; o <<= 1) {
          int tt = __shfl_up_sync(0xffffffffu, incl, o);
          if (lane >= o) incl += tt;
        }
        const int total = __shfl_sync(0xffffffffu, incl, 31);
        int base = 0;
        if (lane == 31) base = atomicAdd(&f.vis_cnt[h.scene], total);
        base = __shfl_sync(0xffffffffu, base, 31);
        int pos = base + incl - cnt;
#pragma unroll
        for (int hr = 0; hr < 2; ++hr) {
#pragma unroll
          for (int w = 0; w < 4; ++w) {
            unsigned int kk = keep[w] & (hr ? 0xccccccccu : 0x33333333u);
            while (kk) {
              const int b = __ffs(kk) - 1;
              kk &= kk - 1;
              if (pos < h.vis_lcap) {
                const int i = w * 32 + b;
                const VisColMeta cm = gmeta[8 * (i >> 2) + q2 + (i & 1)];
                VisPair vp;
                vp.g = g[hr]; vp.row = cm.row; vp.scene = h.scene; vp.outcol = cm.outcol;
                f.vis_pairs[h.vis_lbase + pos] = vp;
              }
              ++pos;
            }
          }
        }
      }
      __syncwarp();
      if (lane == 0) mbar_arrive(&S.meta_empty[ms]);
    }
  }
  __syncthreads();
  cluster_sync_all();
}

constexpr int SA_BN = 128;
constexpr int SA_KMAX = 8;
constexpr int SA_A_BLOCK = TC_BM * TC_BK * 2;
constexpr int SA_B_STAGE = SA_BN * TC_BK * 2;
constexpr int SA_STAGES = 5;
constexpr int SA_SLABS = 4;
struct SaHdr { int scene, m0, ncols, m, det_base, col0, epoch, vis_lbase, vis_lcap, unit, last, pad; };
struct SaSmem {
  unsigned char a[SA_KMAX][SA_A_BLOCK];
  unsigned char b[SA_STAGES][SA_B_STAGE];
  VisColMeta meta[SA_SLABS][SA_BN];
  float colb[SA_SLABS][SA_BN];
  unsigned int colvalid[SA_SLABS][SA_BN / 32];
  SaHdr hdr[SA_SLABS];
  unsigned long long a_full[SA_KMAX];
  unsigned long long a_empty;
  unsigned long long full_bar[SA_STAGES];
  unsigned long long empty_bar[SA_STAGES];
  unsigned long long meta_full[SA_SLABS];
  unsigned long long meta_empty[SA_SLABS];
};
static_assert(sizeof(SaSmem) + 1024 <= 227 * 1024, "A-stationary screen kernel exceeds the shared memory of an SM");
constexpr int kScreenStationaryMaxD8 = SA_KMAX * TC_BK;

template <bool COSINE>
__global__ void __launch_bounds__(TC_THREADS, 1)
vis_screen_sa_kernel(const __grid_constant__ CUtensorMap mapA, const __grid_constant__ CUtensorMap mapB, Params p,
                     TrackStore ts, Frame f, const TcTile* units, int n_units_host, const int* n_units_dev, int ucols,
                     const VisColMeta* colmeta, const VisColGeo* colgeo, const VisRowMeta* rowmeta, const float* colb,
                     const unsigned int* colvalid) {
  const int n_units = n_units_dev ? *n_units_dev : n_units_host;
  extern __shared__ unsigned char smem_raw_[];
  SaSmem& S = *reinterpret_cast<SaSmem*>(smem_raw_ + ((1024u - (smem_u32(smem_raw_) & 1023u)) & 1023u));
  const int warp = threadIdx.x >> 5, lane = threadIdx.x & 31;
  const int K = p.max_obs;
  const int KB = (p.d8 + TC_BK - 1) / TC_BK;
  const uint32_t crank = cluster_rank();
  if (threadIdx.x == 0) {
    for (int kb = 0; kb < SA_KMAX; ++kb) mbar_init(&S.a_full[kb], 1);
    mbar_init(&S.a_empty, 2);
    for (int s = 0; s < SA_STAGES; ++s) { mbar_init(&S.full_bar[s], 1); mbar_init(&S.empty_bar[s], 2); }
    for (int b = 0; b < SA_SLABS; ++b) { mbar_init(&S.meta_full[b], 1); mbar_init(&S.meta_empty[b], 4); }
    asm volatile("fence.mbarrier_init.release.cluster;" ::: "memory");
  }
  __syncthreads();
  cluster_sync_all();

  if (warp < 4) {
    asm volatile("setmaxnreg.dec.sync.aligned.u32 40;");
    if (warp == 0 && lane == 0) {
      asm volatile("prefetch.tensormap [%0];" ::"l"((uint64_t)&mapA) : "memory");
      asm volatile("prefetch.tensormap [%0];" ::"l"((uint64_t)&mapB) : "memory");
      int seq = 0, gk = 0, unit = 0;
      for (int u = (int)(blockIdx.x >> 1); u < n_units; u += (int)(gridDim.x >> 1), ++unit) {
        const TcTile tl = units[u];
        const SceneDesc sc = f.scenes[tl.scene];
        const int m0 = tl.m0 + (int)crank * TC_BM;
        const int rowA = sc.det_base + m0;
        const int cols = min(ucols, sc.nb * K - tl.c0);
        const int nct = (cols + SA_BN - 1) / SA_BN;
        const int rowB = sc.slot * ts.track_cap * K + tl.c0;
        if (unit > 0) mbar_wait(&S.a_empty, (unit - 1) & 1);
        if (nct == 1) mbar_arrive(&S.a_empty);
        for (int ct = 0; ct < nct; ++ct, ++seq) {
          const int g = seq % SA_SLABS;
          mbar_wait(&S.meta_empty[g], ((seq / SA_SLABS) & 1) ^ 1);
          SaHdr h;
          h.scene = tl.scene; h.m0 = m0; h.ncols = min(SA_BN, cols - ct * SA_BN); h.m = sc.m; h.det_base = sc.det_base;
          h.col0 = sc.col_off + tl.c0 + ct * SA_BN; h.epoch = (int)sc.epoch; h.vis_lbase = sc.vis_lbase;
          h.vis_lcap = sc.vis_lcap; h.unit = unit; h.last = ct + 2 >= nct; h.pad = 0;
          S.hdr[g] = h;
          mbar_expect_tx(&S.meta_full[g], (uint32_t)(sizeof(VisColMeta) * SA_BN + 4 * SA_BN + SA_BN / 8));
          bulk_load(S.meta[g], colmeta + h.col0, (uint32_t)(sizeof(VisColMeta) * SA_BN), &S.meta_full[g]);
          bulk_load(S.colb[g], colb + h.col0, 4 * SA_BN, &S.meta_full[g]);
          bulk_load(S.colvalid[g], colvalid + (h.col0 >> 5), SA_BN / 8, &S.meta_full[g]);
          for (int kb = 0; kb < KB; ++kb, ++gk) {
            if (ct == 0) {
              mbar_expect_tx(&S.a_full[kb], SA_A_BLOCK);
              tma_load_2d(S.a[kb], &mapA, kb * TC_BK, rowA, &S.a_full[kb]);
            }
            const int s = gk % SA_STAGES;
            mbar_wait(&S.empty_bar[s], ((gk / SA_STAGES) & 1) ^ 1);
            mbar_expect_tx(&S.full_bar[s], SA_B_STAGE);
            tma_load_2d_mc(S.b[s] + crank * (SA_B_STAGE / 2), &mapB, kb * TC_BK, rowB + ct * SA_BN + (int)crank * (SA_BN / 2),
                           &S.full_bar[s], (uint16_t)0x3);
          }
        }
      }
      for (int e = 0; e < 2; ++e, ++seq) {
        const int g = seq % SA_SLABS;
        mbar_wait(&S.meta_empty[g], ((seq / SA_SLABS) & 1) ^ 1);
        S.hdr[g].scene = -1 - e;
        mbar_arrive(&S.meta_full[g]);
      }
    }
  } else {
    asm volatile("setmaxnreg.inc.sync.aligned.u32 232;");
    const int wg = (warp >> 2) - 1;
    const int rr[2] = {(warp & 3) * 16 + (lane >> 2), (warp & 3) * 16 + (lane >> 2) + 8};
    const int q2 = 2 * (lane & 3);
    const bool geo = p.n_constraints > 0;
    const bool elected = (threadIdx.x & 127) == 0;
    for (int pos = wg;; pos += 2) {
      const int ms = pos % SA_SLABS;
      mbar_wait(&S.meta_full[ms], (pos / SA_SLABS) & 1);
      const SaHdr h = S.hdr[ms];
      if (pos > 0) wg2_bar_sync(1 + (pos & 1));
      if (h.scene < 0) {
        if (h.scene == -1) wg2_bar_arrive(1 + ((pos + 1) & 1));
        break;
      }
      float rowk[2][2];
      bool row_ok[2][2];
#pragma unroll
      for (int hh = 0; hh < 2; ++hh)
#pragma unroll
        for (int hr = 0; hr < 2; ++hr) {
          const int m = h.m0 + 64 * hh + rr[hr];
          const VisRowMeta rm = rowmeta[h.det_base + m];
          rowk[hh][hr] = rm.rowk;
          row_ok[hh][hr] = m < h.m && rm.ok;
        }

      float acc[128];
      {
        const int g0 = pos * KB;
        int stage = g0 % SA_STAGES;
        uint32_t phase = (g0 / SA_STAGES) & 1;
        int prev = -1;
        auto release = [&](int s) {
          if (elected)
            for (uint32_t r = 0; r < 2; ++r) mbar_arrive_cluster(cluster_addr(&S.empty_bar[s], r));
        };
        for (int kb = 0; kb < KB; ++kb) {
          mbar_wait(&S.a_full[kb], (uint32_t)h.unit & 1u);
          mbar_wait(&S.full_bar[stage], phase);
          const uint32_t a0 = smem_u32(S.a[kb]);
          const uint32_t b0 = smem_u32(S.b[stage]);
          wgmma_fence();
#pragma unroll
          for (int k = 0; k < TC_BK / 16; ++k) {
            const uint32_t acc_on = (kb | k) != 0 ? 1u : 0u;
            wgmma_bf16_m64n128(acc, wgmma_desc(a0 + k * 32), wgmma_desc(b0 + k * 32), acc_on);
            wgmma_bf16_m64n128(acc + 64, wgmma_desc(a0 + 64 * 128 + k * 32), wgmma_desc(b0 + k * 32), acc_on);
          }
          wgmma_commit();
          wgmma_wait<1>();
          if (prev >= 0) release(prev);
          prev = stage;
          if (++stage == SA_STAGES) { stage = 0; phase ^= 1; }
        }
        wg2_bar_arrive(1 + ((pos + 1) & 1));
        wgmma_wait<0>();
        wgmma_fence_acc(acc);
        release(prev);
        if (h.last && elected) mbar_arrive(&S.a_empty);
      }

      const VisColMeta* gmeta = S.meta[ms];
      const float* gcolb = S.colb[ms];
      unsigned int colm[2] = {0u, 0u};
#pragma unroll
      for (int j = 0; j < SA_BN / 8; ++j) {
        const int c0 = 8 * j + q2;
        unsigned int m2 = (S.colvalid[ms][c0 >> 5] >> (c0 & 31)) & 3u;
        m2 &= (c0 < h.ncols ? 1u : 0u) | (c0 + 1 < h.ncols ? 2u : 0u);
        colm[j >> 3] |= (m2 | (m2 << 2)) << ((4 * j) & 31);
      }
      unsigned int keep[4];
#pragma unroll
      for (int hh = 0; hh < 2; ++hh) {
        const unsigned int rowm = (row_ok[hh][0] ? 0x33333333u : 0u) | (row_ok[hh][1] ? 0xccccccccu : 0u);
        keep[2 * hh] = 0u;
        keep[2 * hh + 1] = 0u;
#pragma unroll
        for (int j = 0; j < SA_BN / 8; ++j) {
          const float2 cb = *reinterpret_cast<const float2*>(gcolb + 8 * j + q2);
#pragma unroll
          for (int e = 0; e < 4; ++e) {
            const float rk = rowk[hh][e >> 1], c = (e & 1) ? cb.y : cb.x;
            const float b = COSINE ? rk * c : rk + c;
            if (!(acc[64 * hh + 4 * j + e] < b)) keep[2 * hh + (j >> 3)] |= 1u << ((4 * j + e) & 31);
          }
        }
        keep[2 * hh] &= colm[0] & rowm;
        keep[2 * hh + 1] &= colm[1] & rowm;
      }
      if (geo) {
        float cx[2][2], cy[2][2], cr[2][2];
#pragma unroll
        for (int hh = 0; hh < 2; ++hh)
#pragma unroll
          for (int hr = 0; hr < 2; ++hr) {
            cx[hh][hr] = 0.0f; cy[hh][hr] = 0.0f; cr[hh][hr] = 0.0f;
            if (row_ok[hh][hr]) {
              const size_t g = (size_t)h.det_base + h.m0 + 64 * hh + rr[hr];
              cx[hh][hr] = f.c_box[g * 6]; cy[hh][hr] = f.c_box[g * 6 + 1]; cr[hh][hr] = f.c_radius[g];
            }
          }
#pragma unroll
        for (int w = 0; w < 4; ++w) {
          unsigned int kk = keep[w];
          while (kk) {
            const int b = __ffs(kk) - 1;
            kk &= kk - 1;
            const int i = (w & 1) * 32 + b, hh = w >> 1;
            const bool r8 = (i >> 1) & 1;
            const int col = 8 * (i >> 2) + q2 + (i & 1);
            const VisColGeo cg = colgeo[h.col0 + col];
            if (!compat_ok(p, (unsigned int)h.epoch, cg.tep, r8 ? cx[hh][1] : cx[hh][0], r8 ? cy[hh][1] : cy[hh][0],
                           r8 ? cr[hh][1] : cr[hh][0], cg.tx, cg.ty, cg.tr))
              keep[w] &= ~(1u << b);
          }
        }
      }
      int cnt = 0;
#pragma unroll
      for (int w = 0; w < 4; ++w) cnt += __popc(keep[w]);
      if (__any_sync(0xffffffffu, cnt != 0)) {
        int incl = cnt;
#pragma unroll
        for (int o = 1; o < 32; o <<= 1) {
          int tt = __shfl_up_sync(0xffffffffu, incl, o);
          if (lane >= o) incl += tt;
        }
        const int total = __shfl_sync(0xffffffffu, incl, 31);
        int base = 0;
        if (lane == 31) base = atomicAdd(&f.vis_cnt[h.scene], total);
        base = __shfl_sync(0xffffffffu, base, 31);
        int at = base + incl - cnt;
#pragma unroll
        for (int hh = 0; hh < 2; ++hh) {
#pragma unroll
          for (int hr = 0; hr < 2; ++hr) {
            const int g = h.det_base + h.m0 + 64 * hh + rr[hr];
#pragma unroll
            for (int w = 0; w < 2; ++w) {
              unsigned int kk = keep[2 * hh + w] & (hr ? 0xccccccccu : 0x33333333u);
              while (kk) {
                const int b = __ffs(kk) - 1;
                kk &= kk - 1;
                if (at < h.vis_lcap) {
                  const int i = w * 32 + b;
                  const VisColMeta cm = gmeta[8 * (i >> 2) + q2 + (i & 1)];
                  VisPair vp;
                  vp.g = g; vp.row = cm.row; vp.scene = h.scene; vp.outcol = cm.outcol;
                  f.vis_pairs[h.vis_lbase + at] = vp;
                }
                ++at;
              }
            }
          }
        }
      }
      __syncwarp();
      if (lane == 0) mbar_arrive(&S.meta_empty[ms]);
    }
  }
  __syncthreads();
  cluster_sync_all();
}

__device__ __forceinline__ float reduce_add8_tc(const float* t) {
  float q0 = t[0] + t[4], q1 = t[1] + t[5], q2 = t[2] + t[6], q3 = t[3] + t[7];
  float d0 = q0 + q2, d1 = q1 + q3;
  return d0 + d1;
}

constexpr int RF_WARPS = 4;
constexpr int RF_SEG = 64;
constexpr int RF_PITCH = RF_SEG + 1;

template <bool TAIL>
__device__ __forceinline__ void refine_load_a(const float* __restrict__ a, int blk, int D, float* av) {
  if (!TAIL) {
    const float4 a0 = *reinterpret_cast<const float4*>(a + blk * 8);
    const float4 a1 = *reinterpret_cast<const float4*>(a + blk * 8 + 4);
    av[0] = a0.x; av[1] = a0.y; av[2] = a0.z; av[3] = a0.w; av[4] = a1.x; av[5] = a1.y; av[6] = a1.z; av[7] = a1.w;
  } else {
#pragma unroll
    for (int l = 0; l < 8; ++l) av[l] = blk * 8 + l < D ? a[blk * 8 + l] : 0.0f;
  }
}
template <bool COSINE>
__device__ __forceinline__ float refine_block_sum(const float* av, const float* __restrict__ b, int blk) {
  const float4 b0 = *reinterpret_cast<const float4*>(b + blk * 8);
  const float4 b1 = *reinterpret_cast<const float4*>(b + blk * 8 + 4);
  const float bb[8] = {b0.x, b0.y, b0.z, b0.w, b1.x, b1.y, b1.z, b1.w};
  float t[8];
#pragma unroll
  for (int l = 0; l < 8; ++l) {
    if (COSINE) t[l] = av[l] * bb[l];
    else { const float df = av[l] - bb[l]; t[l] = df * df; }
  }
  return reduce_add8_tc(t);
}

template <bool COSINE, bool TAIL, int RP>
__global__ void __launch_bounds__(RF_WARPS * 32, RP == 32 ? 6 : 8) vis_refine_kernel(Params p, TrackStore ts, Frame f, int* nan_flag) {
  __shared__ float s_bs[RF_WARPS][RP][RF_PITCH];
  const int scene = blockIdx.y;
  if (f.vis_mode[scene] != 0) return;
  const SceneDesc sc = f.scenes[scene];
  const int lane = threadIdx.x & 31, w = threadIdx.x >> 5;
  const int n_pairs = min(f.vis_cnt[scene], sc.vis_lcap);
  const int nblk = p.d8 / 8;
  const int D = p.feature_dim;
  float (*bs)[RF_PITCH] = s_bs[w];
  float vmax = nanf("");
  for (;;) {
    int i0 = 0;
    if (lane == 0) i0 = atomicAdd(f.refine_next + scene, RP);
    i0 = __shfl_sync(0xffffffffu, i0, 0);
    if (i0 >= n_pairs) break;
    const int npair = min(RP, n_pairs - i0);
    VisPair mine;
    mine.g = 0; mine.row = 0; mine.scene = 0; mine.outcol = 0;
    if (lane < npair) mine = f.vis_pairs[sc.vis_lbase + i0 + lane];
    float acc = 0.0f;
    for (int seg0 = 0; seg0 < nblk; seg0 += RF_SEG) {
      const int segn = min(RF_SEG, nblk - seg0);
      int g_prev = -1;
      float av[RF_SEG / 32][8];
#pragma unroll 4
      for (int pp = 0; pp < npair; ++pp) {
        const int g = __shfl_sync(0xffffffffu, mine.g, pp);
        const int row = __shfl_sync(0xffffffffu, mine.row, pp);
        const float* b = ts.feat + (size_t)row * p.d8;
        if (g != g_prev) {
          const float* a = f.in_feat + (size_t)g * D;
#pragma unroll
          for (int h = 0; h < RF_SEG / 32; ++h)
            if (h * 32 + lane < segn) refine_load_a<TAIL>(a, seg0 + h * 32 + lane, D, av[h]);
          g_prev = g;
        }
#pragma unroll
        for (int h = 0; h < RF_SEG / 32; ++h) {
          const int j = h * 32 + lane;
          if (j < segn) bs[pp][j] = refine_block_sum<COSINE>(av[h], b, seg0 + j);
        }
      }
      __syncwarp();
      if (lane < npair)
        for (int j = 0; j < segn; ++j) acc = acc + bs[lane][j];
      __syncwarp();
    }
    if (lane < npair) {
      float v = nanf("");
      if (COSINE) {
        const float d = acc / sqrtf(f.c_norm2[mine.g] * ts.fnorm2[mine.row]);
        if (d >= p.visual_threshold) v = 1.0f - d;
      } else {
        const float d = sqrtf(acc);
        if (d <= p.visual_threshold) v = d;
      }
      f.vis_val[sc.vis_lbase + i0 + lane] = v;
      if (!is_nan(v) && !(v <= vmax)) vmax = v;
      if (nan_flag && is_nan(v)) nan_flag[scene] = 1;
    }
  }
  unsigned int u = 0u;
  if (!is_nan(vmax)) {
    u = __float_as_uint(vmax);
    u = (u & 0x80000000u) ? ~u : (u | 0x80000000u);
  }
#pragma unroll
  for (int o = 16; o > 0; o >>= 1) u = max(u, __shfl_xor_sync(0xffffffffu, u, o));
  if (lane == 0 && u != 0u) atomicMax(f.scene_max + scene, u);
}

constexpr int RA_WARPS = 6;
constexpr int RA_STAGES = 3;
constexpr int RA_PAIRS = 2;
constexpr int RA_SEGF = RF_SEG * 8;
constexpr int RA_STAGE_FLOATS = RA_PAIRS * 2 * RA_SEGF;

__device__ __forceinline__ void cp_async16(void* smem_dst, const void* gsrc) {
  asm volatile("cp.async.cg.shared.global [%0], [%1], 16;" ::"r"(smem_u32(smem_dst)), "l"(gsrc) : "memory");
}
__device__ __forceinline__ void cp_async_commit() { asm volatile("cp.async.commit_group;" ::: "memory"); }
template <int N>
__device__ __forceinline__ void cp_async_wait() { asm volatile("cp.async.wait_group %0;" ::"n"(N) : "memory"); }

template <bool COSINE>
__global__ void __launch_bounds__(RA_WARPS * 32) vis_refine_async_kernel(Params p, TrackStore ts, Frame f, int* nan_flag) {
  extern __shared__ __align__(16) unsigned char ra_smem[];
  const int scene = blockIdx.y;
  if (f.vis_mode[scene] != 0) return;
  const SceneDesc sc = f.scenes[scene];
  const int lane = threadIdx.x & 31, w = threadIdx.x >> 5;
  float* stage0 = reinterpret_cast<float*>(ra_smem) + (size_t)w * (RA_STAGES * RA_STAGE_FLOATS + 32 * RF_PITCH);
  float (*bs)[RF_PITCH] = reinterpret_cast<float (*)[RF_PITCH]>(stage0 + RA_STAGES * RA_STAGE_FLOATS);
  const int n_pairs = min(f.vis_cnt[scene], sc.vis_lcap);
  const int nblk = p.d8 / 8;
  const int D = p.feature_dim;
  float vmax = nanf("");
  for (;;) {
    int i0 = 0;
    if (lane == 0) i0 = atomicAdd(f.refine_next + scene, 32);
    i0 = __shfl_sync(0xffffffffu, i0, 0);
    if (i0 >= n_pairs) break;
    const int npair = min(32, n_pairs - i0);
    VisPair mine;
    mine.g = 0; mine.row = 0; mine.scene = 0; mine.outcol = 0;
    if (lane < npair) mine = f.vis_pairs[sc.vis_lbase + i0 + lane];
    float acc = 0.0f;
    const int nst = (npair + RA_PAIRS - 1) / RA_PAIRS;
    for (int seg0 = 0; seg0 < nblk; seg0 += RF_SEG) {
      const int segn = min(RF_SEG, nblk - seg0);
      const int nchunk = segn * 2;
      auto issue = [&](int st) {
        if (st < nst) {
          float* dst = stage0 + (st % RA_STAGES) * RA_STAGE_FLOATS;
#pragma unroll
          for (int pi = 0; pi < RA_PAIRS; ++pi) {
            const int pp = st * RA_PAIRS + pi;
            const int g = __shfl_sync(0xffffffffu, mine.g, pp & 31);
            const int row = __shfl_sync(0xffffffffu, mine.row, pp & 31);
            if (pp < npair) {
              const float* a = f.in_feat + (size_t)g * D + seg0 * 8;
              const float* b = ts.feat + (size_t)row * p.d8 + seg0 * 8;
              float* da = dst + (pi * 2) * RA_SEGF;
              float* db = da + RA_SEGF;
#pragma unroll
              for (int c = 0; c < RA_SEGF / 4 / 32; ++c) {
                const int q = c * 32 + lane;
                if (q < nchunk) {
                  const int pos = ((q & 1) * RF_SEG + (q >> 1)) * 4;
                  cp_async16(da + pos, a + q * 4);
                  cp_async16(db + pos, b + q * 4);
                }
              }
            }
          }
        }
        cp_async_commit();
      };
      issue(0);
      issue(1);
      for (int st = 0; st < nst; ++st) {
        issue(st + 2);
        cp_async_wait<2>();
        __syncwarp();
        const float* src = stage0 + (st % RA_STAGES) * RA_STAGE_FLOATS;
#pragma unroll
        for (int pi = 0; pi < RA_PAIRS; ++pi) {
          const int pp = st * RA_PAIRS + pi;
          if (pp < npair) {
            const float* sa = src + (pi * 2) * RA_SEGF;
            const float* sb2 = sa + RA_SEGF;
#pragma unroll
            for (int h = 0; h < RF_SEG / 32; ++h) {
              const int j = h * 32 + lane;
              if (j < segn) {
                const float4 a0 = *reinterpret_cast<const float4*>(sa + j * 4);
                const float4 a1 = *reinterpret_cast<const float4*>(sa + (RF_SEG + j) * 4);
                const float4 b0 = *reinterpret_cast<const float4*>(sb2 + j * 4);
                const float4 b1 = *reinterpret_cast<const float4*>(sb2 + (RF_SEG + j) * 4);
                const float av[8] = {a0.x, a0.y, a0.z, a0.w, a1.x, a1.y, a1.z, a1.w};
                const float bv[8] = {b0.x, b0.y, b0.z, b0.w, b1.x, b1.y, b1.z, b1.w};
                float t[8];
#pragma unroll
                for (int l = 0; l < 8; ++l) {
                  if (COSINE) t[l] = av[l] * bv[l];
                  else { const float df = av[l] - bv[l]; t[l] = df * df; }
                }
                bs[pp][j] = reduce_add8_tc(t);
              }
            }
          }
        }
        __syncwarp();
      }
      cp_async_wait<0>();
      if (lane < npair)
        for (int j = 0; j < segn; ++j) acc = acc + bs[lane][j];
      __syncwarp();
    }
    if (lane < npair) {
      float v = nanf("");
      if (COSINE) {
        const float d = acc / sqrtf(f.c_norm2[mine.g] * ts.fnorm2[mine.row]);
        if (d >= p.visual_threshold) v = 1.0f - d;
      } else {
        const float d = sqrtf(acc);
        if (d <= p.visual_threshold) v = d;
      }
      f.vis_val[sc.vis_lbase + i0 + lane] = v;
      if (!is_nan(v) && !(v <= vmax)) vmax = v;
      if (nan_flag && is_nan(v)) nan_flag[scene] = 1;
    }
  }
  unsigned int u = 0u;
  if (!is_nan(vmax)) {
    u = __float_as_uint(vmax);
    u = (u & 0x80000000u) ? ~u : (u | 0x80000000u);
  }
#pragma unroll
  for (int o = 16; o > 0; o >>= 1) u = max(u, __shfl_xor_sync(0xffffffffu, u, o));
  if (lane == 0 && u != 0u) atomicMax(f.scene_max + scene, u);
}

__global__ void vis_fill_none_kernel(Params p, Frame f) {
  const int scene = blockIdx.y;
  if (f.scene_mode[scene] != 0) return;
  const SceneDesc sc = f.scenes[scene];
  const long long cnt = (long long)sc.m * sc.n * p.max_obs;
  float* out = f.vis + sc.vis_off;
  const float qnan = nanf("");
  for (long long i = (long long)blockIdx.x * blockDim.x + threadIdx.x; i < cnt; i += (long long)gridDim.x * blockDim.x) out[i] = qnan;
}
__global__ void vis_scatter_kernel(Params p, Frame f) {
  const int scene = blockIdx.y;
  if (f.scene_mode[scene] != 0) return;
  const SceneDesc sc = f.scenes[scene];
  const int n_pairs = min(f.vis_cnt[scene], sc.vis_lcap);
  float* out = f.vis + sc.vis_off;
  for (int i = blockIdx.x * blockDim.x + threadIdx.x; i < n_pairs; i += gridDim.x * blockDim.x) {
    const VisPair vp = f.vis_pairs[sc.vis_lbase + i];
    out[(size_t)(vp.g - sc.det_base) * (sc.n * p.max_obs) + vp.outcol] = f.vis_val[sc.vis_lbase + i];
  }
}
void launch_vis_densify(const Params& p, const Frame& f, int n_scenes, cudaStream_t st) {
  if (n_scenes == 0) return;
  dim3 grid(64, n_scenes);
  vis_fill_none_kernel<<<grid, 256, 0, st>>>(p, f);
  vis_scatter_kernel<<<grid, 256, 0, st>>>(p, f);
  note_launch(2);
}

__global__ void to_bf16_kernel(const float* src, int src_pitch, int d, int d8, long long rows, __nv_bfloat16* dst) {
  long long i = (long long)blockIdx.x * blockDim.x + threadIdx.x;
  if (i >= rows * d8) return;
  long long r = i / d8;
  int c = (int)(i - r * d8);
  float x = c < d ? src[r * src_pitch + c] : 0.0f;
  dst[i] = __float2bfloat16_rn(x);
}

void launch_to_bf16(const float* src, int src_pitch, int d, int d8, long long rows, void* dst, cudaStream_t st) {
  if (rows == 0) return;
  long long n = rows * d8;
  to_bf16_kernel<<<(unsigned)((n + 255) / 256), 256, 0, st>>>(src, src_pitch, d, d8, rows, (__nv_bfloat16*)dst);
  note_launch();
}

typedef CUresult (*EncodeTiledFn)(CUtensorMap*, CUtensorMapDataType, cuuint32_t, void*, const cuuint64_t*, const cuuint64_t*,
                                  const cuuint32_t*, const cuuint32_t*, CUtensorMapInterleave, CUtensorMapSwizzle,
                                  CUtensorMapL2promotion, CUtensorMapFloatOOBfill);

static EncodeTiledFn get_encode() {
  static EncodeTiledFn fn = nullptr;
  if (!fn) {
    void* p = nullptr;
    cudaDriverEntryPointQueryResult qr;
    if (cudaGetDriverEntryPoint("cuTensorMapEncodeTiled", &p, cudaEnableDefault, &qr) == cudaSuccess && p) fn = (EncodeTiledFn)p;
  }
  return fn;
}

static int make_map(CUtensorMap* m, const void* base, long long rows, int d8, int box_rows) {
  EncodeTiledFn enc = get_encode();
  if (!enc) return -1;
  cuuint64_t dims[2] = {(cuuint64_t)d8, (cuuint64_t)rows};
  cuuint64_t strides[1] = {(cuuint64_t)d8 * 2};
  cuuint32_t box[2] = {(cuuint32_t)TC_BK, (cuuint32_t)box_rows};
  cuuint32_t estr[2] = {1, 1};
  CUresult r = enc(m, CU_TENSOR_MAP_DATA_TYPE_BFLOAT16, 2, (void*)base, dims, strides, box, estr, CU_TENSOR_MAP_INTERLEAVE_NONE,
                   CU_TENSOR_MAP_SWIZZLE_128B, CU_TENSOR_MAP_L2_PROMOTION_L2_256B, CU_TENSOR_MAP_FLOAT_OOB_FILL_NONE);
  return r == CUDA_SUCCESS ? 0 : -2;
}

__global__ void vis_meta_kernel(Params p, TrackStore ts, Frame f, int n_scenes, int max_rows, VisColMeta* colmeta,
                                VisColGeo* colgeo, float* colb, unsigned int* colvalid) {
  const int s = blockIdx.y;
  const SceneDesc sc = f.scenes[s];
  const int K = p.max_obs;
  const int prow = blockIdx.x * blockDim.x + threadIdx.x;
  const bool in = prow < sc.nb * K && prow < max_rows;
  VisColMeta cm;
  cm.colb = 0.0f; cm.colc = 0.0f; cm.outcol = -1; cm.row = -1;
  if (in) {
    const int b = prow / K, ph = prow - b * K;
    const size_t sbase = (size_t)sc.slot * ts.track_cap;
    const int n = ts.blk_owner ? ts.blk_owner[sbase + b] : b;
    const size_t ti = sbase + (n >= 0 ? n : 0);
    const size_t frow = (sbase + b) * K + ph;
    unsigned int tep = 0u;
    if (n >= 0) {
      const int on = ts.obs_n[ti];
      int k_of = -1, live_mask = 0;
      for (int k = 0; k < K; ++k) {
        if (k < on && ts.obs_hasf[ti * K + k]) {
          int pp = ts.obs_phys[ti * K + k];
          live_mask |= 1 << pp;
          if (pp == ph) k_of = k;
        }
      }
      tep = ts.epoch[ti];
      if (k_of >= 0) {
        const unsigned int delta = sc.epoch > tep ? sc.epoch - tep : tep - sc.epoch;
        cm.outcol = n * K + k_of;
        const bool valid = (ts.feat_cnt[ti] >= p.min_track_length) && ((unsigned int)p.max_idle_epochs >= delta);
        const float nb = ts.fnorm2[frow];
        cm.colb = p.visual_kind == 1 ? sqrtf(nb) : 0.5f * nb * (1.0f - 1e-5f - kScreenRelErr);
        cm.row = valid ? (int)frow : -1;
      } else {
        int dead_rank = 0;
        for (int pp = 0; pp < ph; ++pp) dead_rank += ((live_mask >> pp) & 1) ? 0 : 1;
        int seen = 0;
        for (int k = 0; k < K; ++k) {
          bool lv = k < on && ts.obs_hasf[ti * K + k];
          if (!lv) { if (seen == dead_rank) { cm.outcol = n * K + k; break; } ++seen; }
        }
      }
    }
    colmeta[sc.col_off + prow] = cm;
    colb[sc.col_off + prow] = cm.colb;
    if (p.n_constraints > 0) {
      VisColGeo cg;
      cg.tx = 0.0f; cg.ty = 0.0f; cg.tr = 0.0f; cg.tep = tep;
      if (n >= 0) { const float* tb = ts.pred + ti * 6; cg.tx = tb[0]; cg.ty = tb[1]; cg.tr = ts.radius[ti]; }
      colgeo[sc.col_off + prow] = cg;
    }
  }
  const unsigned int vb = __ballot_sync(0xffffffffu, cm.row >= 0);
  if ((threadIdx.x & 31) == 0 && vb != 0) colvalid[(sc.col_off + prow) >> 5] = vb;
  else if ((threadIdx.x & 31) == 0 && in) colvalid[(sc.col_off + prow) >> 5] = 0u;
}

__global__ void vis_rowmeta_kernel(Params p, Frame f, VisRowMeta* rowmeta) {
  int g = blockIdx.x * blockDim.x + threadIdx.x;
  if (g >= f.total) return;
  g += f.det0;
  const float na = f.c_norm2[g];
  VisRowMeta rm;
  rm.ok = (f.c_flags[g] & 2) ? 1 : 0;
  const float thr = p.visual_threshold;
  if (p.visual_kind == 1) rm.rowk = (thr - 1e-5f - kScreenRelErr) * sqrtf(na);
  else rm.rowk = 0.5f * (na * (1.0f - 1e-5f - kScreenRelErr) - thr * thr * (1.0f + 1e-5f));
  rowmeta[g] = rm;
}

int launch_vis_refine(const Params& p, const TrackStore& ts, const Frame& f, int n_scenes, int* nan_flag, cudaStream_t st) {
  if (n_scenes == 0) return 0;
  dim3 grid(16, n_scenes);
  const bool tail = p.feature_dim != p.d8 || (reinterpret_cast<uintptr_t>(f.in_feat) & 15) != 0;
  static const bool async_copy = getenv("SB200_REFINE") != nullptr && !strcmp(getenv("SB200_REFINE"), "async");
  if (!tail && async_copy) {
    const size_t smem = (size_t)RA_WARPS * (RA_STAGES * RA_STAGE_FLOATS + 32 * RF_PITCH) * sizeof(float);
    const void* fn = p.visual_kind == 1 ? (const void*)vis_refine_async_kernel<true> : (const void*)vis_refine_async_kernel<false>;
    cudaError_t e = cudaFuncSetAttribute(fn, cudaFuncAttributeMaxDynamicSharedMemorySize, (int)smem);
    if (e != cudaSuccess) return (int)e;
    dim3 grid2(8, n_scenes);
    if (p.visual_kind == 1) vis_refine_async_kernel<true><<<grid2, RA_WARPS * 32, smem, st>>>(p, ts, f, nan_flag);
    else vis_refine_async_kernel<false><<<grid2, RA_WARPS * 32, smem, st>>>(p, ts, f, nan_flag);
    note_launch();
    return 0;
  }
  static const bool rp16 = !(getenv("SB200_REFINE_PAIRS") != nullptr && atoi(getenv("SB200_REFINE_PAIRS")) == 32);
#define SB_RF(C, T)                                                                        \
  do {                                                                                     \
    if (rp16) vis_refine_kernel<C, T, 16><<<grid, RF_WARPS * 32, 0, st>>>(p, ts, f, nan_flag); \
    else vis_refine_kernel<C, T, 32><<<grid, RF_WARPS * 32, 0, st>>>(p, ts, f, nan_flag);      \
  } while (0)
  if (p.visual_kind == 1) {
    if (tail) SB_RF(true, true); else SB_RF(true, false);
  } else {
    if (tail) SB_RF(false, true); else SB_RF(false, false);
  }
#undef SB_RF
  note_launch();
  return 0;
}

void launch_vis_colmeta(const Params& p, const TrackStore& ts, const Frame& f, int n_scenes, int max_n, const TcArgs& tc,
                        cudaStream_t st) {
  const int max_rows = tc.max_rows > 0 ? tc.max_rows : max_n * p.max_obs;
  if (tc.n_tiles == 0 || max_rows <= 0) return;
  dim3 grid((max_rows + 255) / 256, n_scenes);
  vis_meta_kernel<<<grid, 256, 0, st>>>(p, ts, f, n_scenes, max_rows, tc.colmeta, tc.colgeo, tc.colb, tc.colvalid);
  note_launch();
}

int vis_screen_ucols(int d8, int num_sms, int n_scenes, const int* m, const int* nb, int K) {
  if (d8 > kScreenStationaryMaxD8) return TC_BN;
  long long pairs = 0, pair_tiles = 0;
  int max_ct = 1;
  for (int s = 0; s < n_scenes; ++s) {
    const int ct = (nb[s] * K + SA_BN - 1) / SA_BN, rp = (m[s] + 2 * TC_BM - 1) / (2 * TC_BM);
    pairs += rp;
    pair_tiles += (long long)rp * ct;
    max_ct = std::max(max_ct, ct);
  }
  const long long units = 2ll * std::max(1, num_sms / 2);
  if (pairs >= units) return max_ct * SA_BN;
  const long long per = (pair_tiles + units - 1) / units;
  return (int)std::max<long long>(2, std::min<long long>(per, max_ct)) * SA_BN;
}

int launch_vis_cost_tc(const Params& p, const TrackStore& ts, const Frame& f, int n_scenes, int max_n, const TcArgs& tc,
                       int phase, cudaStream_t st) {
  if (tc.n_tiles == 0) return 0;
  if (phase == 1) {
    int rc = launch_vis_refine(p, ts, f, n_scenes, nullptr, st);
    if (tc.ev_refine1) cudaEventRecord(tc.ev_refine1, st);
    return rc;
  }
  const bool stationary = p.d8 <= kScreenStationaryMaxD8;
  CUtensorMap mA, mB;
  if (make_map(&mA, f.c_bf16, tc.a_rows, p.d8, TC_BM) ||
      make_map(&mB, ts.feat_bf16, tc.b_rows, p.d8, stationary ? SA_BN / 2 : TC_BN / 2))
    return -1;
  const size_t smem = (stationary ? sizeof(SaSmem) : sizeof(TcSmem)) + 1024;
  const bool cosine = p.visual_kind == 1;
  cudaError_t e = cudaSuccess;
  const void* fn = stationary ? (cosine ? (const void*)vis_screen_sa_kernel<true> : (const void*)vis_screen_sa_kernel<false>)
                              : (cosine ? (const void*)vis_screen_kernel<true> : (const void*)vis_screen_kernel<false>);
  e = cudaFuncSetAttribute(fn, cudaFuncAttributeMaxDynamicSharedMemorySize, (int)smem);
  if (e != cudaSuccess) return (int)e;
  if (!tc.colmeta_done) launch_vis_colmeta(p, ts, f, n_scenes, max_n, tc, st);
  vis_rowmeta_kernel<<<(f.total + 255) / 256, 256, 0, st>>>(p, f, tc.rowmeta);
  note_launch();
  if (tc.ev_screen0) cudaEventRecord(tc.ev_screen0, st);
  {
    const int ncta = 2 * std::min(tc.n_tiles, tc.num_sms / 2);
    cudaLaunchConfig_t cfg;
    memset(&cfg, 0, sizeof(cfg));
    cfg.gridDim = dim3(ncta);
    cfg.blockDim = dim3(TC_THREADS);
    cfg.dynamicSmemBytes = smem;
    cfg.stream = st;
    cudaLaunchAttribute attr[1];
    attr[0].id = cudaLaunchAttributeClusterDimension;
    attr[0].val.clusterDim.x = 2; attr[0].val.clusterDim.y = 1; attr[0].val.clusterDim.z = 1;
    cfg.attrs = attr;
    cfg.numAttrs = 1;
    const TcTile* d_tiles = tc.d_tiles;
    int n_tiles = tc.n_tiles;
    const int* d_n_tiles = tc.d_n_tiles;
    const VisColMeta* cmeta = tc.colmeta;
    const VisColGeo* cgeo = tc.colgeo;
    const VisRowMeta* rmeta = tc.rowmeta;
    const float* cb = tc.colb;
    const unsigned int* cv = tc.colvalid;
    int ucols = tc.cstep;
    void* args[] = {(void*)&mA, (void*)&mB, (void*)&p, (void*)&ts, (void*)&f, (void*)&d_tiles, (void*)&n_tiles,
                    (void*)&d_n_tiles, (void*)&cmeta, (void*)&cgeo, (void*)&rmeta, (void*)&cb, (void*)&cv};
    void* args_sa[] = {(void*)&mA, (void*)&mB, (void*)&p, (void*)&ts, (void*)&f, (void*)&d_tiles, (void*)&n_tiles,
                       (void*)&d_n_tiles, (void*)&ucols, (void*)&cmeta, (void*)&cgeo, (void*)&rmeta, (void*)&cb, (void*)&cv};
    e = cudaLaunchKernelExC(&cfg, fn, stationary ? args_sa : args);
    if (e != cudaSuccess) return (int)e;
    note_launch();
  }
  if (tc.ev_screen1) cudaEventRecord(tc.ev_screen1, st);
  return 0;
}

}
```

similari_b200/csrc/kernels_state.cu:

```cuda
#include <cuda_bf16.h>

#include <algorithm>

#include "sb_engine.cuh"

namespace sb {

constexpr int AT = 512;

__device__ __forceinline__ void write_box(float* dst, const Box& b) {
  dst[0] = b.xc; dst[1] = b.yc; dst[2] = b.angle; dst[3] = b.aspect; dst[4] = b.height; dst[5] = b.conf;
}
__device__ __forceinline__ void write_box_row(float* dst, const Box& b) {
  float2* d2 = reinterpret_cast<float2*>(dst);
  d2[0] = make_float2(b.xc, b.yc); d2[1] = make_float2(b.angle, b.aspect); d2[2] = make_float2(b.height, b.conf);
}

__global__ void __launch_bounds__(AT) apply_rank_kernel(Params p, TrackStore ts, Frame f, int n_scenes, int* n_tracks) {
  __shared__ int s_warp[AT / 32];
  __shared__ int s_carry;
  __shared__ int s_newbefore;
  const int sidx = blockIdx.x;
  const SceneDesc sc = f.scenes[sidx];
  const int tid = threadIdx.x, lane = tid & 31, wid = tid >> 5;
// ... 379 lines not shown
    s_wbase = seen > 0 ? atomicAdd(wb.count, seen) : 0;
  }
  __syncthreads();
  const int wcount = s_wcount;
  if (frame_out && tid == 0) {
    frame_out[blockIdx.x * 3] = n - wcount;
    frame_out[blockIdx.x * 3 + 1] = arena ? ts.arena_top[slot] : 0;
    frame_out[blockIdx.x * 3 + 2] = wcount;
  }
  if (wcount == 0) return;
  const int first = s_first;
  const int nfree0 = arena ? ts.n_free[slot] : 0;
  for (int j = first + tid; j < n; j += WT) {
    const int d = s_dst[j];
    if (d >= 0) continue;
    const int wrank = -1 - d;
    const int o = s_wbase + wrank;
    if (o < wb.cap) {
      wb.id[o] = ts.id[base + j]; wb.scene[o] = scene_id; wb.epoch[o] = ts.epoch[base + j];
      wb.length[o] = ts.length[base + j];
      for (int c = 0; c < 6; ++c) { wb.pred[(size_t)o * 6 + c] = ts.pred[(base + j) * 6 + c]; wb.obs[(size_t)o * 6 + c] = ts.obs[(base + j) * 6 + c]; }
      if (ts.hist_len > 1) {
        const int hw = ts.hist_len * 6;
        const int hv = (int)min((unsigned int)ts.hist_len, ts.length[base + j]) * 6;
        for (int c = 0; c < hv; ++c) {
          wb.hist_pred[(size_t)o * hw + c] = ts.hist_pred[(base + j) * hw + c];
          wb.hist_obs[(size_t)o * hw + c] = ts.hist_obs[(base + j) * hw + c];
        }
      }
    }
    if (arena) {
      const int b = ts.fblk[base + j];
      ts.blk_free[base + nfree0 + wrank] = b;
      ts.blk_owner[base + b] = -1;
    }
  }
  __syncthreads();
  for (int j0 = first; j0 < n; j0 += WT) {
    const int j = j0 + tid;
    int d = -1;
    unsigned long long v_id = 0; unsigned int v_ep = 0, v_len = 0; long long v_cu = 0; signed char v_vt = 0; float v_r = 0.0f;
    unsigned char v_on = 0, v_fc = 0, v_ph[kMaxObs], v_hf[kMaxObs]; float v_q[kMaxObs]; int v_fb = 0;
    if (j < n) {
      d = s_dst[j];
      if (d >= 0 && d != j) {
        const size_t t = base + j;
        v_id = ts.id[t]; v_ep = ts.epoch[t]; v_len = ts.length[t]; v_cu = ts.custom[t]; v_vt = ts.vt[t]; v_r = ts.radius[t];
        if (p.is_visual) {
          v_on = ts.obs_n[t]; v_fc = ts.feat_cnt[t];
          if (arena) v_fb = ts.fblk[t];
          for (int k = 0; k < K; ++k) {
            const bool have = k < (int)v_on;
            v_ph[k] = have ? ts.obs_phys[t * K + k] : (unsigned char)0; v_hf[k] = have ? ts.obs_hasf[t * K + k] : (unsigned char)0;
            v_q[k] = have ? ts.obs_q[t * K + k] : 0.0f;
          }
        }
      } else d = -1;
    }
    __syncthreads();
    if (d >= 0) {
      const size_t t = base + d;
      ts.id[t] = v_id; ts.epoch[t] = v_ep; ts.length[t] = v_len; ts.custom[t] = v_cu; ts.vt[t] = v_vt; ts.radius[t] = v_r;
      if (p.is_visual) {
        ts.obs_n[t] = v_on; ts.feat_cnt[t] = v_fc;
        if (arena) ts.fblk[t] = v_fb;
        for (int k = 0; k < K; ++k) { ts.obs_phys[t * K + k] = v_ph[k]; ts.obs_hasf[t * K + k] = v_hf[k]; ts.obs_q[t * K + k] = v_q[k]; }
      }
    }
    __syncthreads();
  }
  compact_rows(ts.pred, base, 6, s_dst, first, n);
  compact_rows(ts.obs, base, 6, s_dst, first, n);
  compact_rows(ts.kst, base, ts.kst_stride, s_dst, first, n);
  if (p.positional_kind == 1) compact_rows(ts.vert, base, 8, s_dst, first, n);
  if (ts.hist_len > 1) {
    compact_rows(ts.hist_pred, base, ts.hist_len * 6, s_dst, first, n);
    compact_rows(ts.hist_obs, base, ts.hist_len * 6, s_dst, first, n);
  }
  const int kept = n - wcount;
  if (arena) {
    for (int j = first + tid; j < kept; j += WT) ts.blk_owner[base + ts.fblk[base + j]] = j;
    if (tid == 0) ts.n_free[slot] = nfree0 + wcount;
  }
  if (tid == 0) n_tracks[slot] = kept;
}

static void launch_waste_kernel(const Params& p, const TrackStore& ts, int n_ctas, const unsigned int* d_cur_epoch,
                                const unsigned long long* d_scene_ids, int* d_n_tracks, const WastedBuf& wb,
                                const SceneDesc* scenes, int* frame_out, unsigned long long* id_counter, long long id_add,
                                const int* new_count, cudaStream_t st) {
  const size_t smem = (size_t)std::max(1, ts.track_cap) * sizeof(int);
  if (smem > 48 * 1024) cudaFuncSetAttribute(waste_kernel, cudaFuncAttributeMaxDynamicSharedMemorySize, (int)smem);
  waste_kernel<<<n_ctas, WT, smem, st>>>(p, ts, d_cur_epoch, d_scene_ids, d_n_tracks, wb, scenes, frame_out, id_counter,
                                         id_add, new_count, n_ctas);
  note_launch();
}

void launch_waste(const Params& p, const TrackStore& ts, int n_slots, const unsigned int* d_cur_epoch,
                  const unsigned long long* d_scene_ids, int* d_n_tracks, const WastedBuf& wb, int max_n,
                  cudaStream_t st) {
  (void)max_n;
  if (n_slots == 0) return;
  launch_waste_kernel(p, ts, n_slots, d_cur_epoch, d_scene_ids, d_n_tracks, wb, nullptr, nullptr, nullptr, 0, nullptr, st);
}

void launch_frame_sweep(const Params& p, const TrackStore& ts, const Frame& f, int n_scenes, int* d_n_tracks,
                        const WastedBuf& wb, cudaStream_t st) {
  if (n_scenes == 0) return;
  launch_waste_kernel(p, ts, n_scenes, nullptr, nullptr, d_n_tracks, wb, f.scenes, f.frame_out, f.id_counter, f.id_add,
                      f.new_count, st);
}

__global__ void kalman_ops_kernel(int op, float pw, float vw, const float* in30, const float* boxes, int n, float* out30) {
  int i = blockIdx.x * blockDim.x + threadIdx.x;
  if (i >= n) return;
  float a[kStateFloats], b[kStateFloats];
  Box bx{};
  if (boxes) { const float* q = boxes + (size_t)i * 6; bx = Box{q[0], q[1], q[2], q[3], q[4], q[5]}; }
  if (op == 0) kalman_initiate(pw, vw, bx, b);
  else {
    for (int k = 0; k < kStateFloats; ++k) a[k] = in30[(size_t)i * kStateFloats + k];
    if (op == 1) kalman_predict(pw, vw, a, b);
    else kalman_update(pw, a, bx, b);
  }
  for (int k = 0; k < kStateFloats; ++k) out30[(size_t)i * kStateFloats + k] = b[k];
}

void launch_kalman_ops(int op, float pw, float vw, const float* in30, const float* boxes, int n, float* out30,
                       cudaStream_t st) {
  if (n == 0) return;
  kalman_ops_kernel<<<(n + 127) / 128, 128, 0, st>>>(op, pw, vw, in30, boxes, n, out30);
  note_launch();
}

__global__ void pull_kernel(unsigned int* __restrict__ dst, const unsigned int* __restrict__ src, size_t n4, size_t n1) {
  const size_t i = (size_t)blockIdx.x * blockDim.x + threadIdx.x;
  if (i < n4) reinterpret_cast<uint4*>(dst)[i] = reinterpret_cast<const uint4*>(src)[i];
  if (i < n1) dst[n4 * 4 + i] = src[n4 * 4 + i];
}

void launch_pull(void* dst, const void* src, size_t bytes, cudaStream_t st) {
  if (bytes == 0) return;
  const size_t words = bytes / 4, n4 = words / 4, n1 = words - n4 * 4;
  const size_t threads = n4 > n1 ? n4 : n1;
  pull_kernel<<<(unsigned int)((threads + 255) / 256), 256, 0, st>>>(reinterpret_cast<unsigned int*>(dst),
                                                                    reinterpret_cast<const unsigned int*>(src), n4, n1);
  note_launch();
}

constexpr int FS_T = 1024;

__global__ void __launch_bounds__(FS_T) frame_setup_kernel(Params p, TrackStore ts, Frame f, const SceneReq* req, int n_scenes,
                                                           const int* n_tracks, int mstep, int cstep, int dense_i,
                                                           TcTile* tiles, FrameDyn* dyn, int* zero, int n_zero) {
  constexpr int NQ = 6;
  __shared__ long long s_w[NQ][FS_T / 32];
  __shared__ long long s_carry[NQ];
  __shared__ unsigned long long s_red[3][FS_T / 32];
  __shared__ int s_maxn, s_maxrows;
  const int tid = threadIdx.x, lane = tid & 31, wid = tid >> 5;
  for (int i = tid; i < n_zero; i += FS_T) zero[i] = 0;
  if (f.scene_max) for (int i = tid; i < n_scenes; i += FS_T) f.scene_max[i] = ~__float_as_uint(-1.0f);
  if (tid < NQ) s_carry[tid] = 0;
  if (tid == 0) { s_maxn = 0; s_maxrows = 0; }
  const bool dense = dense_i != 0;
  __syncthreads();
  const int K = p.max_obs;
  unsigned long long u_mn = 0, u_rows = 0, live = 0;
  for (int base = 0; base < n_scenes; base += FS_T) {
    const int s = base + tid;
    SceneReq r;
    r.slot = 0; r.m = 0; r.det_base = 0; r.epoch = 0; r.scene_id = 0; r.pos_lbase = r.pos_lcap = r.vis_lbase = r.vis_lcap = 0;
    int n = 0, nb = 0, rows = 0;
    long long v[NQ] = {0, 0, 0, 0, 0, 0};
    int ctiles = 0;
    if (s < n_scenes) {
      r = req[s];
      n = n_tracks[r.slot];
      nb = (p.is_visual && ts.arena_top) ? ts.arena_top[r.slot] : 0;
      rows = nb * K;
      v[0] = (long long)r.m * n;
      v[1] = p.is_visual ? (long long)r.m * n * K : 0;
      ctiles = (rows + cstep - 1) / cstep;
      v[2] = dense ? (long long)ctiles * 256 : ((long long)rows + 127) / 128 * 128;
      v[3] = mstep > 0 ? (long long)((r.m + mstep - 1) / mstep) * ctiles : 0;
      const int nbpad = dense ? ctiles * (cstep / (K > 0 ? K : 1)) : nb;
      v[4] = dense ? (long long)nbpad * ((r.m + 127) / 128 * 128) : 0;
      v[5] = nbpad;
      u_mn += (unsigned long long)v[0];
      u_rows += (unsigned long long)r.m * (unsigned long long)rows;
      live += (unsigned long long)n;
      atomicMax(&s_maxn, n);
      atomicMax(&s_maxrows, rows);
    }
    long long x[NQ];
#pragma unroll
    for (int q = 0; q < NQ; ++q) {
      x[q] = v[q];
#pragma unroll
      for (int o = 1; o < 32; o <<= 1) {
        const long long t = __shfl_up_sync(0xffffffffu, x[q], o);
        if (lane >= o) x[q] += t;
      }
      if (lane == 31) s_w[q][wid] = x[q];
    }
    __syncthreads();
    long long ex[NQ];
#pragma unroll
    for (int q = 0; q < NQ; ++q) {
      long long woff = 0;
      for (int w = 0; w < wid; ++w) woff += s_w[q][w];
      ex[q] = s_carry[q] + woff + x[q] - v[q];
    }
    __syncthreads();
    if (tid == FS_T - 1) {
#pragma unroll
      for (int q = 0; q < NQ; ++q) s_carry[q] = ex[q] + v[q];
    }
    if (s < n_scenes) {
      SceneDesc d;
      d.slot = r.slot; d.m = r.m; d.n = n; d.det_base = r.det_base;
      d.pos_off = ex[0]; d.vis_off = ex[1];
      d.epoch = r.epoch; d.col_off = (int)ex[2]; d.scene_id = r.scene_id;
      d.pos_lbase = r.pos_lbase; d.pos_lcap = r.pos_lcap; d.vis_lbase = r.vis_lbase; d.vis_lcap = r.vis_lcap;
      d.nb = nb; d.pad0 = 0;
      d.ws_off = ex[4]; d.blk_off = (int)ex[5]; d.slab_off = dense ? (int)(ex[2] / 256) : 0;
      f.scenes[s] = d;
      if (mstep > 0 && tiles) {
        int k = (int)ex[3];
        for (int m0 = 0; m0 < r.m; m0 += mstep)
          for (int j = 0; j < ctiles; ++j) { TcTile t; t.scene = s; t.m0 = m0; t.c0 = j * cstep; t.pad = j; tiles[k++] = t; }
      }
    }
    __syncthreads();
  }
#pragma unroll
  for (int o = 16; o > 0; o >>= 1) {
    u_mn += __shfl_xor_sync(0xffffffffu, u_mn, o);
    u_rows += __shfl_xor_sync(0xffffffffu, u_rows, o);
    live += __shfl_xor_sync(0xffffffffu, live, o);
  }
  if (lane == 0) { s_red[0][wid] = u_mn; s_red[1][wid] = u_rows; s_red[2][wid] = live; }
  __syncthreads();
  if (tid == 0) {
    unsigned long long a = 0, b = 0, c = 0;
    for (int w = 0; w < FS_T / 32; ++w) { a += s_red[0][w]; b += s_red[1][w]; c += s_red[2][w]; }
    FrameDyn d;
    d.n_tiles = (int)s_carry[3]; d.total_cols = (int)s_carry[2]; d.max_rows = s_maxrows; d.max_n = s_maxn;
    d.pos_total = s_carry[0]; d.vis_total = s_carry[1];
    d.units_mn = a; d.units_rows = b; d.live_total = (long long)c;
    d.ws_total = s_carry[4]; d.blk_total = (int)s_carry[5]; d.dense_scenes = 0;
    *dyn = d;
  }
}

void launch_frame_setup(const Params& p, const TrackStore& ts, const Frame& f, const SceneReq* req, int n_scenes,
                        const int* d_n_tracks, int mstep, int cstep, bool dense, TcTile* tiles, FrameDyn* dyn, int* zero,
                        int n_zero, cudaStream_t st) {
  frame_setup_kernel<<<1, FS_T, 0, st>>>(p, ts, f, req, n_scenes, d_n_tracks, mstep, cstep > 0 ? cstep : 256, dense ? 1 : 0, tiles,
                                         dyn, zero, n_zero);
  note_launch();
}

}
```

similari_b200/csrc/sb_engine.cuh:

```cuda
#pragma once
#include <cuda_runtime.h>
#include <stdint.h>

#include "sb_math.cuh"

namespace sb {

constexpr int kMaxConstraints = 8;
constexpr int kNumSms = 132;
constexpr int kMaxObs = 8;
constexpr int kStateStride = 32;
constexpr int kMaxHist = 64;

struct Params {
  int kind, positional_kind, visual_kind;
  float iou_threshold, min_confidence, pos_weight, vel_weight;
  int max_idle_epochs;
  int n_constraints;
  int constraint_epochs[kMaxConstraints];
  float constraint_max_dist[kMaxConstraints];
  float visual_threshold;
  int feature_dim, d8, max_obs, min_votes, min_track_length;
  int vote_vis_cap;
  float min_area, min_quality_use, min_quality_collect, min_own_use, min_own_collect;
  bool is_visual, is_batch, use_own_area;
};

struct SceneDesc {
  int slot;
  int m;
  int n;
  int det_base;
  long long pos_off;
  long long vis_off;
  unsigned int epoch;
  int col_off;
  unsigned long long scene_id;
  int pos_lbase, pos_lcap;
  int vis_lbase, vis_lcap;
  int nb;
  int pad0;
  long long ws_off;
  int blk_off;
  int slab_off;
};

struct SceneReq {
  int slot, m, det_base;
  unsigned int epoch;
  unsigned long long scene_id;
  int pos_lbase, pos_lcap, vis_lbase, vis_lcap;
};
struct FrameDyn {
  int n_tiles;
  int total_cols;
  int max_rows;
  int max_n;
  long long pos_total;
  long long vis_total;
  unsigned long long units_mn;
  unsigned long long units_rows;
  long long live_total;
  long long ws_total;
  int blk_total;
  int dense_scenes;
};

struct VisPair { int g, row, scene, outcol; };
struct PosEntry { unsigned short m, n; float v; };
constexpr int kVotePosCap = 3072;
constexpr int kVoteVisCap = 4096;

struct TrackStore {
  int track_cap;
  unsigned long long* id;
  unsigned int* epoch;
  unsigned int* length;
  long long* custom;
  signed char* vt;
  float* pred;
  float* obs;
  float* radius;
  float* kst;
  int kst_stride;
  double* vert;
  int hist_len;
  float* hist_pred;
  float* hist_obs;
  float* feat;
  void* feat_bf16;
  float* fnorm2;
  unsigned char* obs_phys;
  unsigned char* obs_hasf;
  float* obs_q;
  unsigned char* obs_n;
  unsigned char* feat_cnt;
  int* fblk;
  int* blk_owner;
  int* blk_free;
  int* n_free;
  int* arena_top;
};

__device__ __forceinline__ size_t feat_block(const TrackStore& ts, int slot, size_t ti) {
  return ts.fblk ? (size_t)slot * ts.track_cap + (size_t)ts.fblk[ti] : ti;
}

struct Frame {
  int total;
  int det0;
  int scene0;
  const int* new_count_all;
  long long pos_fill_off;
  const float* in_boxes;
  const float* in_feat;
  const unsigned char* in_hasf;
  const float* in_quality;
  const long long* in_custom;
  const float* in_own;
  float* c_box;
  float* c_radius;
  float* c_conf;
  double* c_vert;
  unsigned char* c_flags;
  float* c_norm2;
  void* c_bf16;
  unsigned int* scene_max;
  int* winner;
  unsigned char* c_vt;
  float* pos;
  bool pos_dense_all;
  long long pos_total;
  float* vis;
  SceneDesc* scenes;
  int* new_count;
  int* status;
  int* feat_dst;
  int2* app_rank;
  int4* app_meta;
  int* frame_out;
  const FrameDyn* dyn;
  unsigned long long* id_counter;
  long long id_add;
  PosEntry* pos_list;
  int* pos_cnt;
  VisPair* vis_pairs;
  float* vis_val;
  int* vis_cnt;
  int* scene_mode;
  int* vis_mode;
  unsigned char* decided;
  unsigned char* excl;
  int* pre_winner;
  int* dense_cnt;
  int2* pos_gq;
  int* pos_gq_cnt;
  int pos_gq_cap;
  int* refine_next;
  const int* dense_bad;
  unsigned long long* o_ids;
  unsigned int* o_epochs;
  unsigned int* o_lengths;
  unsigned char* o_vt;
  float* o_pred;
  float* o_obs;
};

struct TcTile { int scene, m0, c0, pad; };
struct VisColMeta {
  float colb;
  float colc;
  int outcol;
  int row;
};
struct VisColGeo { float tx, ty, tr; unsigned int tep; };
struct VisRowMeta { float rowk; int ok, pad0, pad1; };
struct DenseTrackMeta { int n; int kt; float cmax; int pad; };

void launch_prep(const Params& p, const Frame& f, int n_scenes, int max_m, cudaStream_t st);
void launch_own_area(const Frame& f, int n_scenes, int max_m, const float* d_boxes, float* d_out, int* d_ovf_cnt,
                     int2* d_ovf, cudaStream_t st);
void launch_pull(void* dst, const void* src, size_t bytes, cudaStream_t st);
void launch_frame_setup(const Params& p, const TrackStore& ts, const Frame& f, const SceneReq* req, int n_scenes,
                        const int* d_n_tracks, int mstep, int cstep, bool dense, TcTile* tiles, FrameDyn* dyn, int* zero,
                        int n_zero, cudaStream_t st);
void note_launch(int n = 1);
unsigned long long launch_count();
void launch_pos_cost(const Params& p, const TrackStore& ts, const Frame& f, int n_scenes, int max_m, int max_n,
                     cudaStream_t st);
struct TcArgs {
  int max_init_done;
  int colmeta_done;
  bool use_tc;
  const TcTile* d_tiles;
  int n_tiles;
  const int* d_n_tiles;
  long long a_rows, b_rows;
  int num_sms;
  cudaEvent_t ev_screen0, ev_screen1, ev_refine1;
  VisColMeta* colmeta;
  VisColGeo* colgeo;
  float* colb;
  unsigned int* colvalid;
  VisRowMeta* rowmeta;
  int total_cols;
  int max_rows;
  bool dense;
  int cstep;
  int max_blocks;
  int n_slabs_ub;
  void* ws;
  unsigned int* d_rowb;
  unsigned int* d_colb;
  long long blk_ub;
  float* slab_ktf;
  DenseTrackMeta* tmeta;
  int2* rowinfo;
  float* slab_colc;
  float* slab_cmax;
  unsigned int* slab_vmask;
  unsigned int* slab_bmask;
  float* scene_l0;
  float* scene_cmax;
  VisPair* maxc;
  float* maxc_val;
  int* maxc_cnt;
  int* maxc_next;
  int* dense_bad;
  int* zeros;
  int* dbg_counts;
};
int launch_vis_cost(const Params& p, const TrackStore& ts, const Frame& f, int n_scenes, int max_m, int max_n,
                    const TcArgs& tc, cudaStream_t st);
int launch_vis_dense(const Params& p, const TrackStore& ts, const Frame& f, int n_scenes, int max_m, const TcArgs& tc,
                     cudaStream_t st);
int launch_vis_cost_a(const Params& p, const TrackStore& ts, const Frame& f, int n_scenes, int max_m, int max_n,
                      const TcArgs& tc, cudaStream_t st);
int launch_vis_cost_b(const Params& p, const TrackStore& ts, const Frame& f, int n_scenes, int max_m, int max_n,
                      const TcArgs& tc, cudaStream_t st);
void launch_pos_fill(const Params& p, const Frame& f, int n_scenes, int max_m, int max_n, cudaStream_t st);
void launch_pos_scan(const Params& p, const TrackStore& ts, const Frame& f, int n_scenes, int max_m, int max_n,
                     cudaStream_t st);
void launch_pos_scan_lazy(const Params& p, const TrackStore& ts, const Frame& f, int n_scenes, int max_m, int max_n,
                          int pass, cudaStream_t st);
int launch_vote_masks(const Params& p, const TrackStore& ts, const Frame& f, int n_scenes, int max_m, int max_n,
                      cudaStream_t st);
void launch_vis_colmeta(const Params& p, const TrackStore& ts, const Frame& f, int n_scenes, int max_n, const TcArgs& tc,
                        cudaStream_t st);
int vis_screen_ucols(int d8, int num_sms, int n_scenes, const int* m, const int* nb, int K);
int launch_vis_cost_tc(const Params& p, const TrackStore& ts, const Frame& f, int n_scenes, int max_n, const TcArgs& tc,
                       int phase, cudaStream_t st);
void launch_vis_densify(const Params& p, const Frame& f, int n_scenes, cudaStream_t st);
void launch_to_bf16(const float* src, int src_pitch, int d, int d8, long long rows, void* dst, cudaStream_t st);
void launch_scene_max(const Params& p, const Frame& f, int n_scenes, bool init_only, cudaStream_t st);
void launch_scene_mode(const Params& p, const Frame& f, int n_scenes, bool tc_used, cudaStream_t st);
void launch_vis_mode(const Params& p, const Frame& f, int n_scenes, bool tc_used, cudaStream_t st);
size_t voting_smem_need(int max_m, int max_n, int viscap = 0);
constexpr size_t kVotingSmemLimit = 220 * 1024;
int launch_voting(const Params& p, const TrackStore& ts, const Frame& f, int n_scenes, int max_m, int max_n,
                  cudaStream_t st);
void launch_apply(const Params& p, const TrackStore& ts, const Frame& f, int n_scenes, int max_m,
                  unsigned long long id_base, int* d_n_tracks, cudaStream_t st);
bool launch_feat_store(const Params& p, const TrackStore& ts, const Frame& f, cudaStream_t st);
struct WastedBuf {
  int cap;
  int* count;
  unsigned long long* id;
  unsigned long long* scene;
  unsigned int* epoch;
  unsigned int* length;
  float* pred;
  float* obs;
  float* hist_pred;
  float* hist_obs;
};
void launch_waste(const Params& p, const TrackStore& ts, int n_slots, const unsigned int* d_cur_epoch,
                  const unsigned long long* d_scene_ids, int* d_n_tracks, const WastedBuf& wb, int max_n,
                  cudaStream_t st);
void launch_frame_sweep(const Params& p, const TrackStore& ts, const Frame& f, int n_scenes, int* d_n_tracks,
                        const WastedBuf& wb, cudaStream_t st);

void launch_kalman_ops(int op, float pw, float vw, const float* in30, const float* boxes, int n, float* out30,
                       cudaStream_t st);

__device__ __forceinline__ bool compat_ok(const Params& p, unsigned int cand_epoch, unsigned int trk_epoch, float cx,
                                          float cy, float cr, float tx, float ty, float tr) {
  unsigned int delta = cand_epoch > trk_epoch ? cand_epoch - trk_epoch : trk_epoch - cand_epoch;
  if ((unsigned int)p.max_idle_epochs < delta) return false;
  for (int i = 0; i < p.n_constraints; ++i) {
    if ((unsigned int)p.constraint_epochs[i] >= delta) {
      float d = dist_in_2r(cx, cy, cr, tx, ty, tr);
      return d <= p.constraint_max_dist[i];
    }
  }
  return true;
}

}
```

Before: 53.37 billion.

## Split TC screen into scene waves overlapped with refine on a side stream

Plans the tensor-core screening pass as several waves of scenes, each launched with a limited cluster count. After each wave an event releases the vis-mode and refine kernels for that wave's scenes onto a separate low-priority stream. The refine kernel becomes persistent over a scene range and uses a warp-ballot scene picker, so refine work runs on the SMs the screen leaves idle instead of waiting for the whole screen to finish. The prep-after-cost default also flips so prep no longer waits for cost by default. The extra launches, events and SM partitioning may add overhead or starve the screen kernel.

```diff
diff --git a/similari_b200/csrc/engine.cu b/similari_b200/csrc/engine.cu
--- a/similari_b200/csrc/engine.cu
+++ b/similari_b200/csrc/engine.cu
@@ -198,6 +198,10 @@
   cudaStream_t pos_stream = nullptr;
   bool side_off = false;
   cudaEvent_t ev_fork[2]{}, ev_join = nullptr;
+  cudaStream_t refine_stream = nullptr;
+  std::vector<cudaEvent_t> ev_wave;
+  cudaEvent_t ev_refined = nullptr;
+  std::vector<int> wave_scene;
   float stage_ms[5]{};
   std::unordered_map<uint64_t, int> slot_of;
   std::vector<uint64_t> scene_of_slot;
@@ -233,7 +237,7 @@
   DBuf f_cbox2[2], f_cradius2[2], f_cconf2[2], f_cvert2[2], f_cflags2[2], f_cnorm22[2], f_cbf162[2], f_decided2[2];
   DBuf f_winner, f_cvt, f_pos, f_vis, f_scenes, f_newcount,
       f_status, f_featdst, f_apprank, f_appmeta, f_posgq, f_frameout, f_excl, f_prewin, f_own, f_ownovf, f_dyn, f_ws, f_tmeta, f_rowinfo, f_slabc, f_slabm, f_slabmask,
-      f_dscene, f_maxc, f_maxcval, f_drowb, f_dcolb, f_slabk, f_scene_max, f_tiles, f_pairs, f_colmeta, f_colgeo, f_colb, f_colvalid, f_rowmeta, f_poslist, f_counters, f_visval;
+      f_dscene, f_maxc, f_maxcval, f_drowb, f_dcolb, f_slabk, f_scene_max, f_tiles, f_pairs, f_colmeta, f_colgeo, f_colb, f_colvalid, f_rowmeta, f_poslist, f_counters, f_visval, f_waves;
   int num_sms = 132;
   DBuf o_ids, o_epochs, o_lengths, o_vt, o_pred, o_obs;
   HBuf h_small;
@@ -247,7 +251,7 @@
     cudaSetDevice(device);
     DBuf* all[] = {&b_id, &b_epoch, &b_length, &b_custom, &b_vt, &b_pred, &b_obs, &b_radius, &b_kst, &b_vert, &b_hpred, &b_hobs, &w_hpred, &w_hobs, &b_feat,
                    &b_feat_bf16, &f_scene_max, &f_tiles, &f_pairs, &f_colmeta, &f_colgeo, &f_colb, &f_colvalid, &f_rowmeta, &f_poslist, &f_counters, &f_visval, &b_fnorm2, &b_obs_phys, &b_obs_hasf, &b_obs_q, &b_obs_n, &b_feat_cnt, &b_ntracks, &b_cur_epoch,
-                   &b_fblk, &b_blk_owner, &b_blk_free, &b_nfree, &b_atop, &f_frameout, &f_excl, &f_prewin, &f_own, &f_ownovf, &f_dyn, &b_idc, &f_ws, &f_tmeta, &f_rowinfo, &f_slabc, &f_slabm, &f_slabmask, &f_dscene, &f_maxc, &f_maxcval, &f_drowb, &f_dcolb, &f_slabk,
+                   &b_fblk, &b_blk_owner, &b_blk_free, &b_nfree, &b_atop, &f_frameout, &f_excl, &f_prewin, &f_own, &f_ownovf, &f_dyn, &b_idc, &f_ws, &f_tmeta, &f_rowinfo, &f_slabc, &f_slabm, &f_slabmask, &f_dscene, &f_maxc, &f_maxcval, &f_drowb, &f_dcolb, &f_slabk, &f_waves,
                    &b_scene_ids, &w_count, &w_id, &w_scene, &w_epoch, &w_length, &w_pred, &w_obs, &f_winner, &f_cvt, &f_pos, &f_vis, &f_scenes, &f_newcount, &f_status,
                    &f_featdst, &f_apprank, &f_appmeta, &f_posgq, &o_ids, &o_epochs, &o_lengths, &o_vt, &o_pred, &o_obs};
     for (DBuf* b : all) b->release();
@@ -272,6 +276,9 @@
     }
     if (copy_stream) cudaStreamDestroy(copy_stream);
     if (pos_stream) cudaStreamDestroy(pos_stream);
+    if (refine_stream) cudaStreamDestroy(refine_stream);
+    for (cudaEvent_t e : ev_wave) cudaEventDestroy(e);
+    if (ev_refined) cudaEventDestroy(ev_refined);
     if (prep_stream) cudaStreamDestroy(prep_stream);
     for (cudaEvent_t e : {ev_user_in, ev_user_out, ev_prep_done, ev_set_free[0], ev_set_free[1], ev_inputs, ev_join_req, ev_cost_done}) if (e) cudaEventDestroy(e);
     for (auto& e : ev_fork) if (e) cudaEventDestroy(e);
@@ -765,6 +772,7 @@
     r.vis_lbase = (int)visl_total;
     r.vis_lcap = P.is_visual ? (int)std::min<long long>((long long)r.m * 64, (long long)vote_cap * 4) : 0;
     visl_total += r.vis_lcap;
+    r.wave = -1;
   }
   const long long hint_dets = (long long)std::max(opts.max_scenes_hint, n_scenes) * opts.max_dets_per_scene_hint;
   const size_t T = (size_t)std::max<long long>(std::max(total, 1), hint_dets);
@@ -811,6 +819,13 @@
       blk_ub += ct * (cstep / K);
     }
     tc.n_tiles = (int)tiles_ub;
+    if (!want_dense && tiles_ub > 0) {
+      int wc = 0, wr = 0;
+      if (const char* e = getenv("SB200_SCREEN_WAVES")) { if (sscanf(e, "%d,%d", &wc, &wr) != 2) wc = wr = 0; }
+      tc.n_waves = sb::plan_screen_waves(P.d8, num_sms, n_scenes, m_of.data(), nb_ub.data(), K, cstep, wc, wr, wave_scene,
+                                         &tc.wave_last_clusters);
+      tc.wave_clusters = wc;
+    }
     long long tiles_alloc = tiles_ub;
     {
       const long long hs = std::max(opts.max_scenes_hint, n_scenes), hd = std::max(opts.max_dets_per_scene_hint, max_m);
@@ -827,6 +842,26 @@
     tc.d_n_tiles = &f_dyn.as<sb::FrameDyn>()->n_tiles;
     tc.a_rows = total;
     tc.b_rows = (long long)scene_cap * track_cap * K;
+    if (tc.n_waves > 0) {
+      if ((rc = ENS(f_waves, sizeof(int) * ((size_t)tc.n_waves + 1)))) return rc;
+      if (!refine_stream) {
+        int lo = 0, hi = 0;
+        CU(cudaDeviceGetStreamPriorityRange(&lo, &hi));
+        CU(cudaStreamCreateWithPriority(&refine_stream, cudaStreamNonBlocking, lo));
+        CU(cudaEventCreateWithFlags(&ev_refined, cudaEventDisableTiming));
+      }
+      while ((int)ev_wave.size() < tc.n_waves) {
+        cudaEvent_t e = nullptr;
+        CU(cudaEventCreateWithFlags(&e, cudaEventDisableTiming));
+        ev_wave.push_back(e);
+      }
+      for (int w = 0; w < tc.n_waves; ++w) hreq[wave_scene[w]].wave = w;
+      tc.wave_scene = wave_scene.data();
+      tc.d_wave_unit = f_waves.as<int>();
+      tc.refine_stream = refine_stream;
+      tc.ev_wave = ev_wave.data();
+      tc.ev_refined = ev_refined;
+    }
     if (!want_dense) {
       if ((rc = ENS(f_colmeta, sizeof(sb::VisColMeta) * (size_t)(std::max(col_total, hint_cols) + 256))) ||
           (rc = ENS(f_colb, 4 * (size_t)(std::max(col_total, hint_cols) + 256))) ||
@@ -1059,7 +1094,8 @@
     s_setup = pos_stream;
   }
   sb::launch_frame_setup(P, ts, f, reinterpret_cast<const sb::SceneReq*>(q.h_req.dp), n_scenes, b_ntracks.as<int>(), mstep,
-                         cstep, tc.dense, f_tiles.as<sb::TcTile>(), f_dyn.as<sb::FrameDyn>(), f_counters.as<int>(), (int)n_counters, s_setup);
+                         cstep, tc.dense, f_tiles.as<sb::TcTile>(), f_dyn.as<sb::FrameDyn>(), f_counters.as<int>(), (int)n_counters,
+                         tc.n_waves > 0 ? f_waves.as<int>() : nullptr, tc.n_waves, s_setup);
   tc.max_init_done = 1;
   if (side_setup && Pf.is_visual && tc.use_tc && !tc.dense && tc.n_tiles > 0 && max_m > 0 && max_n > 0 && f.in_feat) {
     sb::launch_vis_colmeta(Pf, ts, f, n_scenes, max_n, tc, pos_stream);
@@ -1079,7 +1115,7 @@
       else { CU(cudaEventRecord(ev_inputs, stream)); CU(cudaStreamWaitEvent(prep_stream, ev_inputs, 0)); }
     }
     if (set_busy[cset]) CU(cudaStreamWaitEvent(prep_stream, ev_set_free[cset], 0));
-    static const bool after_cost = [] { const char* e = getenv("SB200_PREP_AFTER"); return !(e && !strcmp(e, "none")); }();
+    static const bool after_cost = [] { const char* e = getenv("SB200_PREP_AFTER"); return e && !strcmp(e, "cost"); }();
     if (after_cost && cost_done_valid) CU(cudaStreamWaitEvent(prep_stream, ev_cost_done, 0));
     sb::launch_prep(Pf, f, n_scenes, max_m, prep_stream);
     CU(cudaEventRecord(ev_prep_done, prep_stream));
diff --git a/similari_b200/csrc/kernels_assign.cu b/similari_b200/csrc/kernels_assign.cu
--- a/similari_b200/csrc/kernels_assign.cu
+++ b/similari_b200/csrc/kernels_assign.cu
@@ -918,9 +918,9 @@
   f.scene_mode[s] = mode;
   if (mode != 0 && f.dense_cnt) atomicAdd(f.dense_cnt, 1);
 }
-__global__ void vis_mode_kernel(Params p, Frame f, int n_scenes, int tc_used) {
-  int s = blockIdx.x * blockDim.x + threadIdx.x;
-  if (s >= n_scenes) return;
+__global__ void vis_mode_kernel(Params p, Frame f, int s0, int s1, int tc_used) {
+  int s = s0 + blockIdx.x * blockDim.x + threadIdx.x;
+  if (s >= s1) return;
   f.vis_mode[s] = vis_side_mode(p, f, f.scenes[s], s, tc_used);
 }
 
@@ -930,9 +930,9 @@
   note_launch();
 }
 
-void launch_vis_mode(const Params& p, const Frame& f, int n_scenes, bool tc_used, cudaStream_t st) {
-  if (n_scenes == 0 || !f.vis_mode) return;
-  vis_mode_kernel<<<(n_scenes + 127) / 128, 128, 0, st>>>(p, f, n_scenes, tc_used ? 1 : 0);
+void launch_vis_mode(const Params& p, const Frame& f, int s0, int s1, bool tc_used, cudaStream_t st) {
+  if (s1 <= s0 || !f.vis_mode) return;
+  vis_mode_kernel<<<(s1 - s0 + 127) / 128, 128, 0, st>>>(p, f, s0, s1, tc_used ? 1 : 0);
   note_launch();
 }
 
diff --git a/similari_b200/csrc/kernels_cost.cu b/similari_b200/csrc/kernels_cost.cu
--- a/similari_b200/csrc/kernels_cost.cu
+++ b/similari_b200/csrc/kernels_cost.cu
@@ -660,7 +660,7 @@
     int rc = launch_vis_cost_tc(p, ts, f, n_scenes, max_n, tc, 0, st);
     if (rc != 0) return rc;
   }
-  launch_vis_mode(p, f, n_scenes, use_tc, st);
+  if (!(use_tc && !tc.dense && tc.n_waves > 0)) launch_vis_mode(p, f, 0, n_scenes, use_tc, st);
   if (use_tc) {
     int rc = launch_vis_cost_tc(p, ts, f, n_scenes, max_n, tc, 1, st);
     if (rc != 0) return rc;
diff --git a/similari_b200/csrc/kernels_feat_dense.cu b/similari_b200/csrc/kernels_feat_dense.cu
--- a/similari_b200/csrc/kernels_feat_dense.cu
+++ b/similari_b200/csrc/kernels_feat_dense.cu
@@ -573,7 +573,6 @@
   return r == CUDA_SUCCESS ? 0 : -2;
 }
 
-int launch_vis_refine(const Params& p, const TrackStore& ts, const Frame& f, int n_scenes, int* nan_flag, cudaStream_t st);
 
 int launch_vis_dense(const Params& p, const TrackStore& ts, const Frame& f, int n_scenes, int max_m, const TcArgs& tc,
                      cudaStream_t st) {
@@ -650,7 +649,7 @@
     Frame fm = f;
     fm.vis_pairs = tc.maxc; fm.vis_val = tc.maxc_val; fm.vis_cnt = tc.maxc_cnt; fm.refine_next = tc.maxc_next;
     fm.vis_mode = tc.zeros;
-    int rc = launch_vis_refine(p, ts, fm, n_scenes, tc.dense_bad, st);
+    int rc = launch_vis_refine(p, ts, fm, 0, n_scenes, 0, tc.dense_bad, st);
     if (rc != 0) return rc;
   }
   {
diff --git a/similari_b200/csrc/kernels_feat_tc.cu b/similari_b200/csrc/kernels_feat_tc.cu
--- a/similari_b200/csrc/kernels_feat_tc.cu
+++ b/similari_b200/csrc/kernels_feat_tc.cu
@@ -232,10 +232,11 @@
 template <bool COSINE>
 __global__ void __launch_bounds__(TC_THREADS, 1)
 vis_screen_sa_kernel(const __grid_constant__ CUtensorMap mapA, const __grid_constant__ CUtensorMap mapB, Params p,
-                     TrackStore ts, Frame f, const TcTile* units, int n_units_host, const int* n_units_dev, int ucols,
-                     const VisColMeta* colmeta, const VisColGeo* colgeo, const VisRowMeta* rowmeta, const float* colb,
-                     const unsigned int* colvalid) {
-  const int n_units = n_units_dev ? *n_units_dev : n_units_host;
+                     TrackStore ts, Frame f, const TcTile* units, int n_units_host, const int* n_units_dev, const int* wave,
+                     int ucols, const VisColMeta* colmeta, const VisColGeo* colgeo, const VisRowMeta* rowmeta,
+                     const float* colb, const unsigned int* colvalid) {
+  const int unit_begin = wave ? wave[0] : 0;
+  const int unit_end = wave ? wave[1] : (n_units_dev ? *n_units_dev : n_units_host);
   extern __shared__ unsigned char smem_raw_[];
   SaSmem& S = *reinterpret_cast<SaSmem*>(smem_raw_ + ((1024u - (smem_u32(smem_raw_) & 1023u)) & 1023u));
   const int warp = threadIdx.x >> 5, lane = threadIdx.x & 31;
@@ -258,7 +259,7 @@
       asm volatile("prefetch.tensormap [%0];" ::"l"((uint64_t)&mapA) : "memory");
       asm volatile("prefetch.tensormap [%0];" ::"l"((uint64_t)&mapB) : "memory");
       int seq = 0, gk = 0, unit = 0;
-      for (int u = (int)(blockIdx.x >> 1); u < n_units; u += (int)(gridDim.x >> 1), ++unit) {
+      for (int u = unit_begin + (int)(blockIdx.x >> 1); u < unit_end; u += (int)(gridDim.x >> 1), ++unit) {
         const TcTile tl = units[u];
         const SceneDesc sc = f.scenes[tl.scene];
         const int m0 = tl.m0 + (int)crank * TC_BM;
@@ -502,77 +503,99 @@
   return reduce_add8_tc(t);
 }
 
+__device__ __forceinline__ int refine_next_scene(const Frame& f, int s_first, int n_sc, int gw, int lane, int& base) {
+  for (; base < n_sc; base += 32) {
+    const int c = base + lane;
+    int scene = -1;
+    bool open = false;
+    if (c < n_sc) {
+      scene = s_first + (gw + c) % n_sc;
+      open = f.vis_mode[scene] == 0 && __ldcg(f.refine_next + scene) < min(f.vis_cnt[scene], f.scenes[scene].vis_lcap);
+    }
+    const unsigned int ob = __ballot_sync(0xffffffffu, open);
+    if (ob != 0u) {
+      const int pick = __ffs(ob) - 1;
+      base += pick + 1;
+      return __shfl_sync(0xffffffffu, scene, pick);
+    }
+  }
+  return -1;
+}
+
 template <bool COSINE, bool TAIL, int RP>
-__global__ void __launch_bounds__(RF_WARPS * 32, RP == 32 ? 6 : 8) vis_refine_kernel(Params p, TrackStore ts, Frame f, int* nan_flag) {
+__global__ void __launch_bounds__(RF_WARPS * 32, RP == 32 ? 6 : 8)
+vis_refine_kernel(Params p, TrackStore ts, Frame f, int s0, int n_sc, int* nan_flag) {
   __shared__ float s_bs[RF_WARPS][RP][RF_PITCH];
-  const int scene = blockIdx.y;
-  if (f.vis_mode[scene] != 0) return;
-  const SceneDesc sc = f.scenes[scene];
   const int lane = threadIdx.x & 31, w = threadIdx.x >> 5;
-  const int n_pairs = min(f.vis_cnt[scene], sc.vis_lcap);
   const int nblk = p.d8 / 8;
   const int D = p.feature_dim;
   float (*bs)[RF_PITCH] = s_bs[w];
-  float vmax = nanf("");
-  for (;;) {
-    int i0 = 0;
-    if (lane == 0) i0 = atomicAdd(f.refine_next + scene, RP);
-    i0 = __shfl_sync(0xffffffffu, i0, 0);
-    if (i0 >= n_pairs) break;
-    const int npair = min(RP, n_pairs - i0);
-    VisPair mine;
-    mine.g = 0; mine.row = 0; mine.scene = 0; mine.outcol = 0;
-    if (lane < npair) mine = f.vis_pairs[sc.vis_lbase + i0 + lane];
-    float acc = 0.0f;
-    for (int seg0 = 0; seg0 < nblk; seg0 += RF_SEG) {
-      const int segn = min(RF_SEG, nblk - seg0);
-      int g_prev = -1;
-      float av[RF_SEG / 32][8];
+  const int gw = (int)blockIdx.x * RF_WARPS + w;
+  int base = 0;
+  for (int scene; (scene = refine_next_scene(f, s0 + (int)blockIdx.y, n_sc, gw, lane, base)) >= 0;) {
+    const SceneDesc sc = f.scenes[scene];
+    const int n_pairs = min(f.vis_cnt[scene], sc.vis_lcap);
+    float vmax = nanf("");
+    for (;;) {
+      int i0 = 0;
+      if (lane == 0) i0 = atomicAdd(f.refine_next + scene, RP);
+      i0 = __shfl_sync(0xffffffffu, i0, 0);
+      if (i0 >= n_pairs) break;
+      const int npair = min(RP, n_pairs - i0);
+      VisPair mine;
+      mine.g = 0; mine.row = 0; mine.scene = 0; mine.outcol = 0;
+      if (lane < npair) mine = f.vis_pairs[sc.vis_lbase + i0 + lane];
+      float acc = 0.0f;
+      for (int seg0 = 0; seg0 < nblk; seg0 += RF_SEG) {
+        const int segn = min(RF_SEG, nblk - seg0);
+        int g_prev = -1;
+        float av[RF_SEG / 32][8];
 #pragma unroll 4
-      for (int pp = 0; pp < npair; ++pp) {
-        const int g = __shfl_sync(0xffffffffu, mine.g, pp);
-        const int row = __shfl_sync(0xffffffffu, mine.row, pp);
-        const float* b = ts.feat + (size_t)row * p.d8;
-        if (g != g_prev) {
-          const float* a = f.in_feat + (size_t)g * D;
-#pragma unroll
-          for (int h = 0; h < RF_SEG / 32; ++h)
-            if (h * 32 + lane < segn) refine_load_a<TAIL>(a, seg0 + h * 32 + lane, D, av[h]);
-          g_prev = g;
-        }
-#pragma unroll
-        for (int h = 0; h < RF_SEG / 32; ++h) {
-          const int j = h * 32 + lane;
-          if (j < segn) bs[pp][j] = refine_block_sum<COSINE>(av[h], b, seg0 + j);
-        }
-      }
-      __syncwarp();
-      if (lane < npair)
-        for (int j = 0; j < segn; ++j) acc = acc + bs[lane][j];
-      __syncwarp();
-    }
-    if (lane < npair) {
-      float v = nanf("");
-      if (COSINE) {
-        const float d = acc / sqrtf(f.c_norm2[mine.g] * ts.fnorm2[mine.row]);
-        if (d >= p.visual_threshold) v = 1.0f - d;
-      } else {
-        const float d = sqrtf(acc);
-        if (d <= p.visual_threshold) v = d;
-      }
-      f.vis_val[sc.vis_lbase + i0 + lane] = v;
-      if (!is_nan(v) && !(v <= vmax)) vmax = v;
-      if (nan_flag && is_nan(v)) nan_flag[scene] = 1;
-    }
-  }
-  unsigned int u = 0u;
-  if (!is_nan(vmax)) {
-    u = __float_as_uint(vmax);
-    u = (u & 0x80000000u) ? ~u : (u | 0x80000000u);
-  }
-#pragma unroll
-  for (int o = 16; o > 0; o >>= 1) u = max(u, __shfl_xor_sync(0xffffffffu, u, o));
-  if (lane == 0 && u != 0u) atomicMax(f.scene_max + scene, u);
+        for (int pp = 0; pp < npair; ++pp) {
+          const int g = __shfl_sync(0xffffffffu, mine.g, pp);
+          const int row = __shfl_sync(0xffffffffu, mine.row, pp);
+          const float* b = ts.feat + (size_t)row * p.d8;
+          if (g != g_prev) {
+            const float* a = f.in_feat + (size_t)g * D;
+#pragma unroll
+            for (int h = 0; h < RF_SEG / 32; ++h)
+              if (h * 32 + lane < segn) refine_load_a<TAIL>(a, seg0 + h * 32 + lane, D, av[h]);
+            g_prev = g;
+          }
+#pragma unroll
+          for (int h = 0; h < RF_SEG / 32; ++h) {
+            const int j = h * 32 + lane;
+            if (j < segn) bs[pp][j] = refine_block_sum<COSINE>(av[h], b, seg0 + j);
+          }
+        }
+        __syncwarp();
+        if (lane < npair)
+          for (int j = 0; j < segn; ++j) acc = acc + bs[lane][j];
+        __syncwarp();
+      }
+      if (lane < npair) {
+        float v = nanf("");
+        if (COSINE) {
+          const float d = acc / sqrtf(f.c_norm2[mine.g] * ts.fnorm2[mine.row]);
+          if (d >= p.visual_threshold) v = 1.0f - d;
+        } else {
+          const float d = sqrtf(acc);
+          if (d <= p.visual_threshold) v = d;
+        }
+        f.vis_val[sc.vis_lbase + i0 + lane] = v;
+        if (!is_nan(v) && !(v <= vmax)) vmax = v;
+        if (nan_flag && is_nan(v)) nan_flag[scene] = 1;
+      }
+    }
+    unsigned int u = 0u;
+    if (!is_nan(vmax)) {
+      u = __float_as_uint(vmax);
+      u = (u & 0x80000000u) ? ~u : (u | 0x80000000u);
+    }
+#pragma unroll
+    for (int o = 16; o > 0; o >>= 1) u = max(u, __shfl_xor_sync(0xffffffffu, u, o));
+    if (lane == 0 && u != 0u) atomicMax(f.scene_max + scene, u);
+  }
 }
 
 constexpr int RA_WARPS = 6;
@@ -589,122 +612,125 @@
 __device__ __forceinline__ void cp_async_wait() { asm volatile("cp.async.wait_group %0;" ::"n"(N) : "memory"); }
 
 template <bool COSINE>
-__global__ void __launch_bounds__(RA_WARPS * 32) vis_refine_async_kernel(Params p, TrackStore ts, Frame f, int* nan_flag) {
+__global__ void __launch_bounds__(RA_WARPS * 32)
+vis_refine_async_kernel(Params p, TrackStore ts, Frame f, int s0, int n_sc, int* nan_flag) {
   extern __shared__ __align__(16) unsigned char ra_smem[];
-  const int scene = blockIdx.y;
-  if (f.vis_mode[scene] != 0) return;
-  const SceneDesc sc = f.scenes[scene];
   const int lane = threadIdx.x & 31, w = threadIdx.x >> 5;
   float* stage0 = reinterpret_cast<float*>(ra_smem) + (size_t)w * (RA_STAGES * RA_STAGE_FLOATS + 32 * RF_PITCH);
   float (*bs)[RF_PITCH] = reinterpret_cast<float (*)[RF_PITCH]>(stage0 + RA_STAGES * RA_STAGE_FLOATS);
-  const int n_pairs = min(f.vis_cnt[scene], sc.vis_lcap);
   const int nblk = p.d8 / 8;
   const int D = p.feature_dim;
-  float vmax = nanf("");
-  for (;;) {
-    int i0 = 0;
-    if (lane == 0) i0 = atomicAdd(f.refine_next + scene, 32);
-    i0 = __shfl_sync(0xffffffffu, i0, 0);
-    if (i0 >= n_pairs) break;
-    const int npair = min(32, n_pairs - i0);
-    VisPair mine;
-    mine.g = 0; mine.row = 0; mine.scene = 0; mine.outcol = 0;
-    if (lane < npair) mine = f.vis_pairs[sc.vis_lbase + i0 + lane];
-    float acc = 0.0f;
-    const int nst = (npair + RA_PAIRS - 1) / RA_PAIRS;
-    for (int seg0 = 0; seg0 < nblk; seg0 += RF_SEG) {
-      const int segn = min(RF_SEG, nblk - seg0);
-      const int nchunk = segn * 2;
-      auto issue = [&](int st) {
-        if (st < nst) {
-          float* dst = stage0 + (st % RA_STAGES) * RA_STAGE_FLOATS;
-#pragma unroll
-          for (int pi = 0; pi < RA_PAIRS; ++pi) {
-            const int pp = st * RA_PAIRS + pi;
-            const int g = __shfl_sync(0xffffffffu, mine.g, pp & 31);
-            const int row = __shfl_sync(0xffffffffu, mine.row, pp & 31);
-            if (pp < npair) {
-              const float* a = f.in_feat + (size_t)g * D + seg0 * 8;
-              const float* b = ts.feat + (size_t)row * p.d8 + seg0 * 8;
-              float* da = dst + (pi * 2) * RA_SEGF;
-              float* db = da + RA_SEGF;
-#pragma unroll
-              for (int c = 0; c < RA_SEGF / 4 / 32; ++c) {
-                const int q = c * 32 + lane;
-                if (q < nchunk) {
-                  const int pos = ((q & 1) * RF_SEG + (q >> 1)) * 4;
-                  cp_async16(da + pos, a + q * 4);
-                  cp_async16(db + pos, b + q * 4);
+  const int gw = (int)blockIdx.x * RA_WARPS + w;
+  int base = 0;
+  for (int scene; (scene = refine_next_scene(f, s0 + (int)blockIdx.y, n_sc, gw, lane, base)) >= 0;) {
+    const SceneDesc sc = f.scenes[scene];
+    const int n_pairs = min(f.vis_cnt[scene], sc.vis_lcap);
+    float vmax = nanf("");
+    for (;;) {
+      int i0 = 0;
+      if (lane == 0) i0 = atomicAdd(f.refine_next + scene, 32);
+      i0 = __shfl_sync(0xffffffffu, i0, 0);
+      if (i0 >= n_pairs) break;
+      const int npair = min(32, n_pairs - i0);
+      VisPair mine;
+      mine.g = 0; mine.row = 0; mine.scene = 0; mine.outcol = 0;
+      if (lane < npair) mine = f.vis_pairs[sc.vis_lbase + i0 + lane];
+      float acc = 0.0f;
+      const int nst = (npair + RA_PAIRS - 1) / RA_PAIRS;
+      for (int seg0 = 0; seg0 < nblk; seg0 += RF_SEG) {
+        const int segn = min(RF_SEG, nblk - seg0);
+        const int nchunk = segn * 2;
+        auto issue = [&](int st) {
+          if (st < nst) {
+            float* dst = stage0 + (st % RA_STAGES) * RA_STAGE_FLOATS;
+#pragma unroll
+            for (int pi = 0; pi < RA_PAIRS; ++pi) {
+              const int pp = st * RA_PAIRS + pi;
+              const int g = __shfl_sync(0xffffffffu, mine.g, pp & 31);
+              const int row = __shfl_sync(0xffffffffu, mine.row, pp & 31);
+              if (pp < npair) {
+                const float* a = f.in_feat + (size_t)g * D + seg0 * 8;
+                const float* b = ts.feat + (size_t)row * p.d8 + seg0 * 8;
+                float* da = dst + (pi * 2) * RA_SEGF;
+                float* db = da + RA_SEGF;
+#pragma unroll
+                for (int c = 0; c < RA_SEGF / 4 / 32; ++c) {
+                  const int q = c * 32 + lane;
+                  if (q < nchunk) {
+                    const int pos = ((q & 1) * RF_SEG + (q >> 1)) * 4;
+                    cp_async16(da + pos, a + q * 4);
+                    cp_async16(db + pos, b + q * 4);
+                  }
                 }
               }
             }
           }
-        }
-        cp_async_commit();
-      };
-      issue(0);
-      issue(1);
-      for (int st = 0; st < nst; ++st) {
-        issue(st + 2);
-        cp_async_wait<2>();
-        __syncwarp();
-        const float* src = stage0 + (st % RA_STAGES) * RA_STAGE_FLOATS;
-#pragma unroll
-        for (int pi = 0; pi < RA_PAIRS; ++pi) {
-          const int pp = st * RA_PAIRS + pi;
-          if (pp < npair) {
-            const float* sa = src + (pi * 2) * RA_SEGF;
-            const float* sb2 = sa + RA_SEGF;
-#pragma unroll
-            for (int h = 0; h < RF_SEG / 32; ++h) {
-              const int j = h * 32 + lane;
-              if (j < segn) {
-                const float4 a0 = *reinterpret_cast<const float4*>(sa + j * 4);
-                const float4 a1 = *reinterpret_cast<const float4*>(sa + (RF_SEG + j) * 4);
-                const float4 b0 = *reinterpret_cast<const float4*>(sb2 + j * 4);
-                const float4 b1 = *reinterpret_cast<const float4*>(sb2 + (RF_SEG + j) * 4);
-                const float av[8] = {a0.x, a0.y, a0.z, a0.w, a1.x, a1.y, a1.z, a1.w};
-                const float bv[8] = {b0.x, b0.y, b0.z, b0.w, b1.x, b1.y, b1.z, b1.w};
-                float t[8];
-#pragma unroll
-                for (int l = 0; l < 8; ++l) {
-                  if (COSINE) t[l] = av[l] * bv[l];
-                  else { const float df = av[l] - bv[l]; t[l] = df * df; }
+          cp_async_commit();
+        };
+        issue(0);
+        issue(1);
+        for (int st = 0; st < nst; ++st) {
+          issue(st + 2);
+          cp_async_wait<2>();
+          __syncwarp();
+          const float* src = stage0 + (st % RA_STAGES) * RA_STAGE_FLOATS;
+#pragma unroll
+          for (int pi = 0; pi < RA_PAIRS; ++pi) {
+            const int pp = st * RA_PAIRS + pi;
+            if (pp < npair) {
+              const float* sa = src + (pi * 2) * RA_SEGF;
+              const float* sb2 = sa + RA_SEGF;
+#pragma unroll
+              for (int h = 0; h < RF_SEG / 32; ++h) {
+                const int j = h * 32 + lane;
+                if (j < segn) {
+                  const float4 a0 = *reinterpret_cast<const float4*>(sa + j * 4);
+                  const float4 a1 = *reinterpret_cast<const float4*>(sa + (RF_SEG + j) * 4);
+                  const float4 b0 = *reinterpret_cast<const float4*>(sb2 + j * 4);
+                  const float4 b1 = *reinterpret_cast<const float4*>(sb2 + (RF_SEG + j) * 4);
+                  const float av[8] = {a0.x, a0.y, a0.z, a0.w, a1.x, a1.y, a1.z, a1.w};
+                  const float bv[8] = {b0.x, b0.y, b0.z, b0.w, b1.x, b1.y, b1.z, b1.w};
+                  float t[8];
+#pragma unroll
+                  for (int l = 0; l < 8; ++l) {
+                    if (COSINE) t[l] = av[l] * bv[l];
+                    else { const float df = av[l] - bv[l]; t[l] = df * df; }
+                  }
+                  bs[pp][j] = reduce_add8_tc(t);
                 }
-                bs[pp][j] = reduce_add8_tc(t);
               }
             }
           }
-        }
+          __syncwarp();
+        }
+        cp_async_wait<0>();
+        if (lane < npair)
+          for (int j = 0; j < segn; ++j) acc = acc + bs[lane][j];
         __syncwarp();
       }
-      cp_async_wait<0>();
-      if (lane < npair)
-        for (int j = 0; j < segn; ++j) acc = acc + bs[lane][j];
-      __syncwarp();
-    }
-    if (lane < npair) {
-      float v = nanf("");
-      if (COSINE) {
-        const float d = acc / sqrtf(f.c_norm2[mine.g] * ts.fnorm2[mine.row]);
-        if (d >= p.visual_threshold) v = 1.0f - d;
-      } else {
-        const float d = sqrtf(acc);
-        if (d <= p.visual_threshold) v = d;
-      }
-      f.vis_val[sc.vis_lbase + i0 + lane] = v;
-      if (!is_nan(v) && !(v <= vmax)) vmax = v;
-      if (nan_flag && is_nan(v)) nan_flag[scene] = 1;
-    }
-  }
-  unsigned int u = 0u;
-  if (!is_nan(vmax)) {
-    u = __float_as_uint(vmax);
-    u = (u & 0x80000000u) ? ~u : (u | 0x80000000u);
-  }
-#pragma unroll
-  for (int o = 16; o > 0; o >>= 1) u = max(u, __shfl_xor_sync(0xffffffffu, u, o));
-  if (lane == 0 && u != 0u) atomicMax(f.scene_max + scene, u);
+      if (lane < npair) {
+        float v = nanf("");
+        if (COSINE) {
+          const float d = acc / sqrtf(f.c_norm2[mine.g] * ts.fnorm2[mine.row]);
+          if (d >= p.visual_threshold) v = 1.0f - d;
+        } else {
+          const float d = sqrtf(acc);
+          if (d <= p.visual_threshold) v = d;
+        }
+        f.vis_val[sc.vis_lbase + i0 + lane] = v;
+        if (!is_nan(v) && !(v <= vmax)) vmax = v;
+        if (nan_flag && is_nan(v)) nan_flag[scene] = 1;
+      }
+    }
+    unsigned int u = 0u;
+    if (!is_nan(vmax)) {
+      u = __float_as_uint(vmax);
+      u = (u & 0x80000000u) ? ~u : (u | 0x80000000u);
+    }
+#pragma unroll
+    for (int o = 16; o > 0; o >>= 1) u = max(u, __shfl_xor_sync(0xffffffffu, u, o));
+    if (lane == 0 && u != 0u) atomicMax(f.scene_max + scene, u);
+  }
 }
 
 __global__ void vis_fill_none_kernel(Params p, Frame f) {
@@ -848,34 +874,39 @@
   rowmeta[g] = rm;
 }
 
-int launch_vis_refine(const Params& p, const TrackStore& ts, const Frame& f, int n_scenes, int* nan_flag, cudaStream_t st) {
-  if (n_scenes == 0) return 0;
-  dim3 grid(16, n_scenes);
+int launch_vis_refine(const Params& p, const TrackStore& ts, const Frame& f, int s0, int s1, int n_sms, int* nan_flag,
+                      cudaStream_t st) {
+  if (s1 <= s0) return 0;
   const bool tail = p.feature_dim != p.d8 || (reinterpret_cast<uintptr_t>(f.in_feat) & 15) != 0;
   static const bool async_copy = getenv("SB200_REFINE") != nullptr && !strcmp(getenv("SB200_REFINE"), "async");
-  if (!tail && async_copy) {
-    const size_t smem = (size_t)RA_WARPS * (RA_STAGES * RA_STAGE_FLOATS + 32 * RF_PITCH) * sizeof(float);
-    const void* fn = p.visual_kind == 1 ? (const void*)vis_refine_async_kernel<true> : (const void*)vis_refine_async_kernel<false>;
-    cudaError_t e = cudaFuncSetAttribute(fn, cudaFuncAttributeMaxDynamicSharedMemorySize, (int)smem);
+  static const bool rp16 = !(getenv("SB200_REFINE_PAIRS") != nullptr && atoi(getenv("SB200_REFINE_PAIRS")) == 32);
+  const bool cosine = p.visual_kind == 1;
+  const bool use_async = !tail && async_copy;
+  const size_t smem = use_async ? (size_t)RA_WARPS * (RA_STAGES * RA_STAGE_FLOATS + 32 * RF_PITCH) * sizeof(float) : 0;
+  const void* fn;
+  if (use_async) fn = cosine ? (const void*)vis_refine_async_kernel<true> : (const void*)vis_refine_async_kernel<false>;
+  else if (rp16) fn = cosine ? (tail ? (const void*)vis_refine_kernel<true, true, 16> : (const void*)vis_refine_kernel<true, false, 16>)
+                             : (tail ? (const void*)vis_refine_kernel<false, true, 16> : (const void*)vis_refine_kernel<false, false, 16>);
+  else fn = cosine ? (tail ? (const void*)vis_refine_kernel<true, true, 32> : (const void*)vis_refine_kernel<true, false, 32>)
+                   : (tail ? (const void*)vis_refine_kernel<false, true, 32> : (const void*)vis_refine_kernel<false, false, 32>);
+  const int threads = (use_async ? RA_WARPS : RF_WARPS) * 32;
+  cudaError_t e = cudaSuccess;
+  if (use_async) {
+    e = cudaFuncSetAttribute(fn, cudaFuncAttributeMaxDynamicSharedMemorySize, (int)smem);
     if (e != cudaSuccess) return (int)e;
-    dim3 grid2(8, n_scenes);
-    if (p.visual_kind == 1) vis_refine_async_kernel<true><<<grid2, RA_WARPS * 32, smem, st>>>(p, ts, f, nan_flag);
-    else vis_refine_async_kernel<false><<<grid2, RA_WARPS * 32, smem, st>>>(p, ts, f, nan_flag);
-    note_launch();
-    return 0;
-  }
-  static const bool rp16 = !(getenv("SB200_REFINE_PAIRS") != nullptr && atoi(getenv("SB200_REFINE_PAIRS")) == 32);
-#define SB_RF(C, T)                                                                        \
-  do {                                                                                     \
-    if (rp16) vis_refine_kernel<C, T, 16><<<grid, RF_WARPS * 32, 0, st>>>(p, ts, f, nan_flag); \
-    else vis_refine_kernel<C, T, 32><<<grid, RF_WARPS * 32, 0, st>>>(p, ts, f, nan_flag);      \
-  } while (0)
-  if (p.visual_kind == 1) {
-    if (tail) SB_RF(true, true); else SB_RF(true, false);
-  } else {
-    if (tail) SB_RF(false, true); else SB_RF(false, false);
-  }
-#undef SB_RF
+  }
+  dim3 grid(use_async ? 8 : 16, s1 - s0);
+  int n_sc = 1;
+  if (n_sms > 0) {
+    int per_sm = 0;
+    e = cudaOccupancyMaxActiveBlocksPerMultiprocessor(&per_sm, fn, threads, smem);
+    if (e != cudaSuccess) return (int)e;
+    grid = dim3(std::max(1, per_sm) * n_sms, 1);
+    n_sc = s1 - s0;
+  }
+  void* args[] = {(void*)&p, (void*)&ts, (void*)&f, (void*)&s0, (void*)&n_sc, (void*)&nan_flag};
+  e = cudaLaunchKernel(fn, grid, dim3(threads), args, smem, st);
+  if (e != cudaSuccess) return (int)e;
   note_launch();
   return 0;
 }
@@ -905,11 +936,64 @@
   return (int)std::max<long long>(2, std::min<long long>(per, max_ct)) * SA_BN;
 }
 
+int plan_screen_waves(int d8, int num_sms, int n_scenes, const int* m, const int* nb, int K, int cstep, int clusters,
+                      int rounds, std::vector<int>& wave_scene, int* last_clusters) {
+  wave_scene.clear();
+  if (d8 > kScreenStationaryMaxD8 || clusters < 1 || rounds < 1 || 2 * clusters >= num_sms) return 0;
+  const long long cap = (long long)clusters * rounds;
+  long long in_wave = 0;
+  for (int s = 0; s < n_scenes; ++s) {
+    const long long ub = (long long)((m[s] + 2 * TC_BM - 1) / (2 * TC_BM)) * (((long long)nb[s] * K + cstep - 1) / cstep);
+    if (wave_scene.empty() || (in_wave > 0 && in_wave + ub > cap)) { wave_scene.push_back(s); in_wave = 0; }
+    in_wave += ub;
+  }
+  const int n_waves = (int)wave_scene.size();
+  if (n_waves < 2) { wave_scene.clear(); return 0; }
+  wave_scene.push_back(n_scenes);
+  *last_clusters = (int)std::max<long long>(1, std::min<long long>(in_wave, num_sms / 2));
+  return n_waves;
+}
+
+static int launch_screen(const CUtensorMap& mA, const CUtensorMap& mB, const Params& p, const TrackStore& ts,
+                         const Frame& f, const TcArgs& tc, const void* fn, bool stationary, size_t smem, int clusters,
+                         const int* wave, cudaStream_t st) {
+  cudaLaunchConfig_t cfg;
+  memset(&cfg, 0, sizeof(cfg));
+  cfg.gridDim = dim3(2 * clusters);
+  cfg.blockDim = dim3(TC_THREADS);
+  cfg.dynamicSmemBytes = smem;
+  cfg.stream = st;
+  cudaLaunchAttribute attr[1];
+  attr[0].id = cudaLaunchAttributeClusterDimension;
+  attr[0].val.clusterDim.x = 2; attr[0].val.clusterDim.y = 1; attr[0].val.clusterDim.z = 1;
+  cfg.attrs = attr;
+  cfg.numAttrs = 1;
+  const TcTile* d_tiles = tc.d_tiles;
+  int n_tiles = tc.n_tiles;
+  const int* d_n_tiles = tc.d_n_tiles;
+  const VisColMeta* cmeta = tc.colmeta;
+  const VisColGeo* cgeo = tc.colgeo;
+  const VisRowMeta* rmeta = tc.rowmeta;
+  const float* cb = tc.colb;
+  const unsigned int* cv = tc.colvalid;
+  int ucols = tc.cstep;
+  void* args[] = {(void*)&mA, (void*)&mB, (void*)&p, (void*)&ts, (void*)&f, (void*)&d_tiles, (void*)&n_tiles,
+                  (void*)&d_n_tiles, (void*)&cmeta, (void*)&cgeo, (void*)&rmeta, (void*)&cb, (void*)&cv};
+  void* args_sa[] = {(void*)&mA, (void*)&mB, (void*)&p, (void*)&ts, (void*)&f, (void*)&d_tiles, (void*)&n_tiles,
+                     (void*)&d_n_tiles, (void*)&wave, (void*)&ucols, (void*)&cmeta, (void*)&cgeo, (void*)&rmeta,
+                     (void*)&cb, (void*)&cv};
+  cudaError_t e = cudaLaunchKernelExC(&cfg, fn, stationary ? args_sa : args);
+  if (e != cudaSuccess) return (int)e;
+  note_launch();
+  return 0;
+}
+
 int launch_vis_cost_tc(const Params& p, const TrackStore& ts, const Frame& f, int n_scenes, int max_n, const TcArgs& tc,
                        int phase, cudaStream_t st) {
   if (tc.n_tiles == 0) return 0;
   if (phase == 1) {
-    int rc = launch_vis_refine(p, ts, f, n_scenes, nullptr, st);
+    if (tc.n_waves > 0) return 0;
+    int rc = launch_vis_refine(p, ts, f, 0, n_scenes, 0, nullptr, st);
     if (tc.ev_refine1) cudaEventRecord(tc.ev_refine1, st);
     return rc;
   }
@@ -929,37 +1013,29 @@
   vis_rowmeta_kernel<<<(f.total + 255) / 256, 256, 0, st>>>(p, f, tc.rowmeta);
   note_launch();
   if (tc.ev_screen0) cudaEventRecord(tc.ev_screen0, st);
-  {
-    const int ncta = 2 * std::min(tc.n_tiles, tc.num_sms / 2);
-    cudaLaunchConfig_t cfg;
-    memset(&cfg, 0, sizeof(cfg));
-    cfg.gridDim = dim3(ncta);
-    cfg.blockDim = dim3(TC_THREADS);
-    cfg.dynamicSmemBytes = smem;
-    cfg.stream = st;
-    cudaLaunchAttribute attr[1];
-    attr[0].id = cudaLaunchAttributeClusterDimension;
-    attr[0].val.clusterDim.x = 2; attr[0].val.clusterDim.y = 1; attr[0].val.clusterDim.z = 1;
-    cfg.attrs = attr;
-    cfg.numAttrs = 1;
-    const TcTile* d_tiles = tc.d_tiles;
-    int n_tiles = tc.n_tiles;
-    const int* d_n_tiles = tc.d_n_tiles;
-    const VisColMeta* cmeta = tc.colmeta;
-    const VisColGeo* cgeo = tc.colgeo;
-    const VisRowMeta* rmeta = tc.rowmeta;
-    const float* cb = tc.colb;
-    const unsigned int* cv = tc.colvalid;
-    int ucols = tc.cstep;
-    void* args[] = {(void*)&mA, (void*)&mB, (void*)&p, (void*)&ts, (void*)&f, (void*)&d_tiles, (void*)&n_tiles,
-                    (void*)&d_n_tiles, (void*)&cmeta, (void*)&cgeo, (void*)&rmeta, (void*)&cb, (void*)&cv};
-    void* args_sa[] = {(void*)&mA, (void*)&mB, (void*)&p, (void*)&ts, (void*)&f, (void*)&d_tiles, (void*)&n_tiles,
-                       (void*)&d_n_tiles, (void*)&ucols, (void*)&cmeta, (void*)&cgeo, (void*)&rmeta, (void*)&cb, (void*)&cv};
-    e = cudaLaunchKernelExC(&cfg, fn, stationary ? args_sa : args);
-    if (e != cudaSuccess) return (int)e;
-    note_launch();
+  if (tc.n_waves == 0) {
+    int rc = launch_screen(mA, mB, p, ts, f, tc, fn, stationary, smem, std::min(tc.n_tiles, tc.num_sms / 2), nullptr, st);
+    if (rc != 0) return rc;
+    if (tc.ev_screen1) cudaEventRecord(tc.ev_screen1, st);
+    return 0;
+  }
+  for (int w = 0; w < tc.n_waves; ++w) {
+    const bool last = w + 1 == tc.n_waves;
+    int rc = launch_screen(mA, mB, p, ts, f, tc, fn, true, smem, last ? tc.wave_last_clusters : tc.wave_clusters,
+                           tc.d_wave_unit + w, st);
+    if (rc != 0) return rc;
+    if ((e = cudaEventRecord(tc.ev_wave[w], st)) != cudaSuccess) return (int)e;
+    if ((e = cudaStreamWaitEvent(tc.refine_stream, tc.ev_wave[w], 0)) != cudaSuccess) return (int)e;
+    const int s0 = tc.wave_scene[w], s1 = tc.wave_scene[w + 1];
+    launch_vis_mode(p, f, s0, s1, true, tc.refine_stream);
+    rc = launch_vis_refine(p, ts, f, s0, s1, last ? tc.num_sms : tc.num_sms - 2 * tc.wave_clusters, nullptr,
+                           tc.refine_stream);
+    if (rc != 0) return rc;
   }
   if (tc.ev_screen1) cudaEventRecord(tc.ev_screen1, st);
+  if ((e = cudaEventRecord(tc.ev_refined, tc.refine_stream)) != cudaSuccess) return (int)e;
+  if ((e = cudaStreamWaitEvent(st, tc.ev_refined, 0)) != cudaSuccess) return (int)e;
+  if (tc.ev_refine1) cudaEventRecord(tc.ev_refine1, st);
   return 0;
 }
 
diff --git a/similari_b200/csrc/kernels_state.cu b/similari_b200/csrc/kernels_state.cu
--- a/similari_b200/csrc/kernels_state.cu
+++ b/similari_b200/csrc/kernels_state.cu
@@ -555,7 +555,8 @@
 
 __global__ void __launch_bounds__(FS_T) frame_setup_kernel(Params p, TrackStore ts, Frame f, const SceneReq* req, int n_scenes,
                                                            const int* n_tracks, int mstep, int cstep, int dense_i,
-                                                           TcTile* tiles, FrameDyn* dyn, int* zero, int n_zero) {
+                                                           TcTile* tiles, FrameDyn* dyn, int* zero, int n_zero,
+                                                           int* wave_unit, int n_waves) {
   constexpr int NQ = 6;
   __shared__ long long s_w[NQ][FS_T / 32];
   __shared__ long long s_carry[NQ];
@@ -574,6 +575,7 @@
     const int s = base + tid;
     SceneReq r;
     r.slot = 0; r.m = 0; r.det_base = 0; r.epoch = 0; r.scene_id = 0; r.pos_lbase = r.pos_lcap = r.vis_lbase = r.vis_lcap = 0;
+    r.wave = -1;
     int n = 0, nb = 0, rows = 0;
     long long v[NQ] = {0, 0, 0, 0, 0, 0};
     int ctiles = 0;
@@ -634,6 +636,7 @@
         for (int m0 = 0; m0 < r.m; m0 += mstep)
           for (int j = 0; j < ctiles; ++j) { TcTile t; t.scene = s; t.m0 = m0; t.c0 = j * cstep; t.pad = j; tiles[k++] = t; }
       }
+      if (r.wave >= 0 && r.wave < n_waves) wave_unit[r.wave] = (int)ex[3];
     }
     __syncthreads();
   }
@@ -654,14 +657,15 @@
     d.units_mn = a; d.units_rows = b; d.live_total = (long long)c;
     d.ws_total = s_carry[4]; d.blk_total = (int)s_carry[5]; d.dense_scenes = 0;
     *dyn = d;
+    if (n_waves > 0) wave_unit[n_waves] = d.n_tiles;
   }
 }
 
 void launch_frame_setup(const Params& p, const TrackStore& ts, const Frame& f, const SceneReq* req, int n_scenes,
                         const int* d_n_tracks, int mstep, int cstep, bool dense, TcTile* tiles, FrameDyn* dyn, int* zero,
-                        int n_zero, cudaStream_t st) {
+                        int n_zero, int* wave_unit, int n_waves, cudaStream_t st) {
   frame_setup_kernel<<<1, FS_T, 0, st>>>(p, ts, f, req, n_scenes, d_n_tracks, mstep, cstep > 0 ? cstep : 256, dense ? 1 : 0, tiles,
-                                         dyn, zero, n_zero);
+                                         dyn, zero, n_zero, wave_unit, n_waves);
   note_launch();
 }
 
diff --git a/similari_b200/csrc/sb_engine.cuh b/similari_b200/csrc/sb_engine.cuh
--- a/similari_b200/csrc/sb_engine.cuh
+++ b/similari_b200/csrc/sb_engine.cuh
@@ -1,6 +1,8 @@
 #pragma once
 #include <cuda_runtime.h>
 #include <stdint.h>
+
+#include <vector>
 
 #include "sb_math.cuh"
 
@@ -50,6 +52,7 @@
   unsigned int epoch;
   unsigned long long scene_id;
   int pos_lbase, pos_lcap, vis_lbase, vis_lcap;
+  int wave;
 };
 struct FrameDyn {
   int n_tiles;
@@ -183,7 +186,7 @@
 void launch_pull(void* dst, const void* src, size_t bytes, cudaStream_t st);
 void launch_frame_setup(const Params& p, const TrackStore& ts, const Frame& f, const SceneReq* req, int n_scenes,
                         const int* d_n_tracks, int mstep, int cstep, bool dense, TcTile* tiles, FrameDyn* dyn, int* zero,
-                        int n_zero, cudaStream_t st);
+                        int n_zero, int* wave_unit, int n_waves, cudaStream_t st);
 void note_launch(int n = 1);
 unsigned long long launch_count();
 void launch_pos_cost(const Params& p, const TrackStore& ts, const Frame& f, int n_scenes, int max_m, int max_n,
@@ -229,6 +232,14 @@
   int* dense_bad;
   int* zeros;
   int* dbg_counts;
+  int n_waves;
+  int wave_clusters;
+  int wave_last_clusters;
+  const int* wave_scene;
+  const int* d_wave_unit;
+  cudaStream_t refine_stream;
+  cudaEvent_t* ev_wave;
+  cudaEvent_t ev_refined;
 };
 int launch_vis_cost(const Params& p, const TrackStore& ts, const Frame& f, int n_scenes, int max_m, int max_n,
                     const TcArgs& tc, cudaStream_t st);
@@ -248,13 +259,17 @@
 void launch_vis_colmeta(const Params& p, const TrackStore& ts, const Frame& f, int n_scenes, int max_n, const TcArgs& tc,
                         cudaStream_t st);
 int vis_screen_ucols(int d8, int num_sms, int n_scenes, const int* m, const int* nb, int K);
+int plan_screen_waves(int d8, int num_sms, int n_scenes, const int* m, const int* nb, int K, int cstep, int clusters,
+                      int rounds, std::vector<int>& wave_scene, int* last_clusters);
+int launch_vis_refine(const Params& p, const TrackStore& ts, const Frame& f, int s0, int s1, int n_sms, int* nan_flag,
+                      cudaStream_t st);
 int launch_vis_cost_tc(const Params& p, const TrackStore& ts, const Frame& f, int n_scenes, int max_n, const TcArgs& tc,
                        int phase, cudaStream_t st);
 void launch_vis_densify(const Params& p, const Frame& f, int n_scenes, cudaStream_t st);
 void launch_to_bf16(const float* src, int src_pitch, int d, int d8, long long rows, void* dst, cudaStream_t st);
 void launch_scene_max(const Params& p, const Frame& f, int n_scenes, bool init_only, cudaStream_t st);
 void launch_scene_mode(const Params& p, const Frame& f, int n_scenes, bool tc_used, cudaStream_t st);
-void launch_vis_mode(const Params& p, const Frame& f, int n_scenes, bool tc_used, cudaStream_t st);
+void launch_vis_mode(const Params& p, const Frame& f, int s0, int s1, bool tc_used, cudaStream_t st);
 size_t voting_smem_need(int max_m, int max_n, int viscap = 0);
 constexpr size_t kVotingSmemLimit = 220 * 1024;
 int launch_voting(const Params& p, const TrackStore& ts, const Frame& f, int n_scenes, int max_m, int max_n,
```

Result: faster. 54.53 billion, median of 6 (+2.2%).
